# mkshing/e4t-diffusion

Hardware: AMD Instinct MI355X
Metric: E4T pretrain images/sec @512px bf16 (higher is better)
Workload: dtype bf16; 1 GPU; SD-1.4 UNet + ViT-H-14 E4T encoder pretrain step, 512px; per_gpu_batch=16, global_batch=16, parallelism=dp1, trainable=weight offsets + E4T head (ViT frozen), next_batch_prefetch=vit+vae

## Files before the change

e4t-diffusion_amd/csrc/attention.hip:

```cpp
#include "common.h"
#include "../../include/e4t_hip.h"
#include <math.h>
#include <type_traits>

namespace {

struct AttnArgs {
  const bf16_t *Q, *K, *V, *dO;
  const bf16_t* O;
  bf16_t *Out, *dQ, *dK, *dV;
  float* L;
  float* Delta;
  float* LD;
  int T, S, H;
  int ldq, ldk, ldv, ldo;
  long long bq, bk, bv, bo;
  float scale2;
  float scale;
  int causal;
  int xcd_raster;
  float* part;
  int tsplit, tchunk;
};

struct Blk { int x, h, b; };
__device__ __forceinline__ Blk xcd_block(int on) {
  Blk o{(int)blockIdx.x, (int)blockIdx.y, (int)blockIdx.z};
  if (!on) return o;
  const int gx = gridDim.x, gy = gridDim.y, nwg = gx * gy * gridDim.z;
  const int lin = (blockIdx.z * gy + blockIdx.y) * gx + blockIdx.x;
  const int q = nwg >> 3, r = nwg & 7, v = lin & 7;
  const int lin2 = (v < r ? v * (q + 1) : r * (q + 1) + (v - r) * q) + (lin >> 3);
  const int t = lin2 / gx;
  o.x = lin2 - t * gx; o.b = t / gy; o.h = t - o.b * gy;
  return o;
}

template <int DH>
struct Cfg {
  static constexpr int DK = (DH + 15) / 16 * 16;
  static constexpr int DV = (DH + 31) / 32 * 32;
  static constexpr int NKS = DK / 16;
  static constexpr int NDT = DV / 32;
  static constexpr int LDE = DH <= 128 ? 128 : 256;
  static constexpr int NCH = DH / 8;
  static constexpr int NIT = (32 * NCH + 255) / 256;
};

union Frag {
  bf16x8 v;
  uint4 q;
  uint2 h[2];
  uint32_t w[4];
};

__device__ __forceinline__ float xhalf_max(float v) {
  float a = v, b = v;
  asm volatile("s_nop 1\n\tv_permlane32_swap_b32 %0, %1\n\ts_nop 1\n\tv_max_f32 %0, %0, %1" : "+v"(a), "+v"(b));
  return a;
}
__device__ __forceinline__ float xhalf_sum(float v) {
  float a = v, b = v;
  asm volatile("s_nop 1\n\tv_permlane32_swap_b32 %0, %1\n\ts_nop 1\n\tv_add_f32 %0, %0, %1" : "+v"(a), "+v"(b));
  return a;
}

__device__ __forceinline__ f32x16 mfma32(bf16x8 a, bf16x8 b, f32x16 c) { return __builtin_amdgcn_mfma_f32_32x32x16_bf16(a, b, c, 0, 0, 0); }

__device__ __forceinline__ float fast_exp2(float x) { return __builtin_amdgcn_exp2f(x); }

typedef float f32x2 __attribute__((ext_vector_type(2)));
constexpr bool PK_REG = true;
constexpr bool PK_DMA = false;
template <bool PK>
__device__ __forceinline__ f32x2 pk_fma(f32x2 a, f32x2 b, f32x2 c) {
  if constexpr (PK) return __builtin_elementwise_fma(a, b, c);
  else return f32x2{__builtin_fmaf(a.x, b.x, c.x), __builtin_fmaf(a.y, b.y, c.y)};
}
template <bool PK>
__device__ __forceinline__ f32x2 pk_mul(f32x2 a, f32x2 b) {
  if constexpr (PK) return a * b;
  else return f32x2{a.x * b.x, a.y * b.y};
}


template <int LDE>
__device__ __forceinline__ int img_off(int r, int L) {
  return r * LDE + (((((L >> 2) ^ (r & 3)) << 2) | ((L & 3) ^ ((r >> 2) & 3))) << 3);
}

template <int DH>
struct TileRegs {
  using C = Cfg<DH>;
  uint4 v[C::NIT][2];
  unsigned vo[C::NIT];
  int ldb;
  __device__ __forceinline__ void init(int ld) {
    ldb = ld * 2;
#pragma unroll
    for (int it = 0; it < C::NIT; ++it) {
      const int item = threadIdx.x + it * 256;
      const int ch = item >> 5, kp = item & 31;
      vo[it] = item < 32 * C::NCH ? (unsigned)((2 * kp * ld + ch * 8) * 2) : 0xFFFF0000u;
    }
  }
  __device__ __forceinline__ void load(__amdgpu_buffer_rsrc_t rs, int r0) {
    const int soff = r0 * ldb;
#pragma unroll
    for (int it = 0; it < C::NIT; ++it) {
      v[it][0] = buf_load16(rs, vo[it], soff);
      v[it][1] = buf_load16(rs, vo[it], soff + ldb);
    }
  }
  __device__ __forceinline__ void store_rows(bf16_t* lds) const {
#pragma unroll
    for (int it = 0; it < C::NIT; ++it) {
      const int item = threadIdx.x + it * 256;
      const int ch = item >> 5, kp = item & 31;
      if (item < 32 * C::NCH) {
        *(uint4*)(lds + img_off<C::LDE>(2 * kp, ch)) = v[it][0];
        *(uint4*)(lds + img_off<C::LDE>(2 * kp + 1, ch)) = v[it][1];
      }
    }
  }
};

template <int DH>
__device__ __forceinline__ void zero_pad_cols(bf16_t* lds) {
  constexpr int PADC = (Cfg<DH>::DK - DH) / 8;
  if (PADC > 0)
    for (int i = threadIdx.x; i < 64 * PADC; i += 256)
      *(uint4*)(lds + img_off<Cfg<DH>::LDE>(i / PADC, Cfg<DH>::NCH + i % PADC)) = make_uint4(0, 0, 0, 0);
}

template <int DH>
__device__ __forceinline__ void load_row_frags(const bf16_t* g, int ld, int row, int R, int hi, bf16x8* f) {
#pragma unroll
  for (int ks = 0; ks < Cfg<DH>::NKS; ++ks) {
    Frag t;
    t.q = make_uint4(0, 0, 0, 0);
    const int d0 = ks * 16 + hi * 8;
    if (row < R && d0 < DH) t.q = *(const uint4*)(g + (long long)row * ld + d0);
    f[ks] = t.v;
  }
}

template <int DH>
struct FragOff {
  using C = Cfg<DH>;
  int row[C::NKS], tr_lo[C::NDT], tr_hi[C::NDT];
  __device__ __forceinline__ FragOff() {
    const int lane = threadIdx.x & 63, li = lane & 31, hi = lane >> 5, il = lane & 15, d16 = (lane >> 4) & 1;
#pragma unroll
    for (int ks = 0; ks < C::NKS; ++ks) row[ks] = img_off<C::LDE>(li, ks * 2 + hi);
#pragma unroll
    for (int dt = 0; dt < C::NDT; ++dt) {
      const int L = dt * 4 + 2 * d16 + ((il & 3) >> 1), r = 4 * hi + (il >> 2);
      tr_lo[dt] = img_off<C::LDE>(r, L) + 4 * (il & 1);
      tr_hi[dt] = img_off<C::LDE>(r + 8, L) + 4 * (il & 1);
    }
  }
};
template <int DH>
__device__ __forceinline__ bf16x8 load_row_frag(const bf16_t* img, const FragOff<DH>& f, int sub, int ks) {
  return *(const bf16x8*)(img + sub * 32 * Cfg<DH>::LDE + f.row[ks]);
}
template <int DH>
__device__ __forceinline__ bf16x8 load_T_frag(const bf16_t* img, const FragOff<DH>& f, int dt, int sub, int k2) {
  const bf16_t* b = img + (sub * 32 + k2 * 16) * Cfg<DH>::LDE;
  return tr_frag(b + f.tr_lo[dt], b + f.tr_hi[dt]);
}
__device__ __forceinline__ bf16x8 pack_acc(const float* p, int k2) {
  Frag t;
#pragma unroll
  for (int j = 0; j < 4; ++j) t.w[j] = pack2bf(p[8 * k2 + 2 * j], p[8 * k2 + 2 * j + 1]);
  return t.v;
}
__device__ __forceinline__ int acc_row(int r, int hi) { return (r & 3) + 8 * (r >> 2) + 4 * hi; }

template <int DH>
__device__ __forceinline__ void store_T_acc(const f32x16* acc, float mul, bf16_t* g, int ld, int row, int R, int hi) {
  if (row >= R) return;
#pragma unroll
  for (int dt = 0; dt < Cfg<DH>::NDT; ++dt)
#pragma unroll
    for (int rg = 0; rg < 4; ++rg) {
      const int d = dt * 32 + 8 * rg + 4 * hi;
      if (d < DH) {
        float f[4];
#pragma unroll
        for (int j = 0; j < 4; ++j) f[j] = acc[dt][rg * 4 + j] * mul;
        *(uint2*)(g + (long long)row * ld + d) = pack4(f);
      }
    }
}

template <int DH>
__device__ __forceinline__ void store_T_acc_f32(const f32x16* acc, float* g, int row, int R, int hi) {
  if (row >= R) return;
#pragma unroll
  for (int dt = 0; dt < Cfg<DH>::NDT; ++dt)
#pragma unroll
    for (int rg = 0; rg < 4; ++rg) {
      const int d = dt * 32 + 8 * rg + 4 * hi;
      if (d < DH) *(float4*)(g + (size_t)row * DH + d) = make_float4(acc[dt][rg * 4], acc[dt][rg * 4 + 1], acc[dt][rg * 4 + 2], acc[dt][rg * 4 + 3]);
    }
}

template <int DH>
__global__ __launch_bounds__(256, (DH <= 64 ? 4 : DH <= 80 ? 2 : 1)) void attn_fwd_kernel(AttnArgs p) {
  using C = Cfg<DH>;
  __shared__ __attribute__((aligned(16))) bf16_t Ks[64 * C::LDE];
  __shared__ __attribute__((aligned(16))) bf16_t Vs[64 * C::LDE];
  const FragOff<DH> fo;
  const Blk blk = xcd_block(p.xcd_raster);
  const int b = blk.b, h = blk.h;
  const int lane = threadIdx.x & 63, wave = threadIdx.x >> 6;
  const int li = lane & 31, hi = lane >> 5;
  const int q = blk.x * 128 + wave * 32 + li;
  const bf16_t* Qb = p.Q + b * p.bq + h * DH;
  const bf16_t* Kb = p.K + b * p.bk + h * DH;
  const bf16_t* Vb = p.V + b * p.bv + h * DH;

  bf16x8 qf[C::NKS];
  load_row_frags<DH>(Qb, p.ldq, q, p.T, hi, qf);

  f32x16 o[C::NDT];
#pragma unroll
  for (int dt = 0; dt < C::NDT; ++dt)
#pragma unroll
    for (int r = 0; r < 16; ++r) o[dt][r] = 0.f;
  float m = -INFINITY, l = 0.f;
  constexpr bool SUM_BY_MFMA = C::DV > DH && DH % 8 == 0;

  TileRegs<DH> kr, vr;
  const __amdgpu_buffer_rsrc_t rsK = make_rsrc(Kb, (unsigned)(((long long)(p.S - 1) * p.ldk + DH) * 2));
  const __amdgpu_buffer_rsrc_t rsV = make_rsrc(Vb, (unsigned)(((long long)(p.S - 1) * p.ldv + DH) * 2));
  kr.init(p.ldk); vr.init(p.ldv);
  kr.load(rsK, 0);
  vr.load(rsV, 0);
  zero_pad_cols<DH>(Ks);
  if (SUM_BY_MFMA) {
    if (threadIdx.x < 64) *(uint4*)(Vs + img_off<C::LDE>(threadIdx.x, C::NCH)) = make_uint4(0x3F80u, 0, 0, 0);
  }
  for (int kv0 = 0; kv0 < p.S; kv0 += 64) {
    __syncthreads();
    kr.store_rows(Ks);
    vr.store_rows(Vs);
    __syncthreads();
    if (kv0 + 64 < p.S) {
      kr.load(rsK, kv0 + 64);
      vr.load(rsV, kv0 + 64);
    }
    const int nsub = (p.S - kv0 > 32) ? 2 : 1;
#pragma unroll
    for (int sub = 0; sub < 2; ++sub) {
      if (sub >= nsub) break;
      f32x16 s;
#pragma unroll
      for (int r = 0; r < 16; ++r) s[r] = 0.f;
#pragma unroll
      for (int ks = 0; ks < C::NKS; ++ks) {
        s = mfma32(load_row_frag<DH>(Ks, fo, sub, ks), qf[ks], s);
      }
      float pr[16];
      float mx = -INFINITY;
      const bool tail = kv0 + 64 > p.S;
      if (tail || p.causal) {
#pragma unroll
        for (int r = 0; r < 16; ++r) {
          const int key = kv0 + sub * 32 + acc_row(r, hi);
          s[r] = (key < p.S && (!p.causal || key <= q)) ? s[r] : -INFINITY;
        }
      }
#pragma unroll
      for (int r = 0; r < 16; ++r) mx = fmaxf(mx, s[r]);
      mx = xhalf_max(mx) * p.scale2;
      if (__builtin_amdgcn_ballot_w64(mx > m + 8.f) != 0) {
        const float mn = fmaxf(m, mx);
        const float alpha = fast_exp2(m - mn);
        m = mn;
        if (!SUM_BY_MFMA) l *= alpha;
#pragma unroll
        for (int dt = 0; dt < C::NDT; ++dt)
#pragma unroll
          for (int r = 0; r < 16; ++r) o[dt][r] *= alpha;
      }
#pragma unroll
      for (int r = 0; r < 16; r += 2) {
        const f32x2 t = pk_fma<PK_REG>(f32x2{s[r], s[r + 1]}, f32x2{p.scale2, p.scale2}, f32x2{-m, -m});
        pr[r] = fast_exp2(t.x); pr[r + 1] = fast_exp2(t.y);
      }
      if (!SUM_BY_MFMA) {
        float rs = 0.f;
#pragma unroll
        for (int r = 0; r < 16; ++r) rs += pr[r];
        l += xhalf_sum(rs);
      }
      const bf16x8 pf0 = pack_acc(pr, 0), pf1 = pack_acc(pr, 1);
#pragma unroll
      for (int dt = 0; dt < C::NDT; ++dt) {
        o[dt] = mfma32(load_T_frag<DH>(Vs, fo, dt, sub, 0), pf0, o[dt]);
        o[dt] = mfma32(load_T_frag<DH>(Vs, fo, dt, sub, 1), pf1, o[dt]);
      }
    }
  }
  if (SUM_BY_MFMA) {
    constexpr int blk = DH / 32, reg = (DH % 32) / 8 * 4;
    static_assert((DH % 32) % 8 == 0 && ((DH % 32) / 8) * 8 + 0 == DH % 32, "spare row must be row 8k of its block");
    l = o[blk][reg];
    l = __shfl(l, li, 64);
  }
  const float inv = 1.f / l;
  store_T_acc<DH>(o, inv, p.Out + b * p.bo + h * DH, p.ldo, q, p.T, hi);
  if (p.L && hi == 0 && q < p.T) p.L[((long long)b * p.H + h) * p.T + q] = m + log2f(l);
}

constexpr int FWD64_OCC = 2, FWD64_MIN_S = 512;
__device__ __forceinline__ void a64_fence() { __builtin_amdgcn_sched_barrier(0); }

__device__ __forceinline__ f32x2 pk_fms(f32x2 s, f32x2 sc, f32x2 mm) {
  f32x2 d;
  asm("v_fma_f32 %0, %1, %2, -%3" : "=v"(d.x) : "v"(s.x), "s"(sc.x), "v"(mm.x));
  asm("v_fma_f32 %0, %1, %2, -%3" : "=v"(d.y) : "v"(s.y), "s"(sc.x), "v"(mm.x));
  return d;
}

__device__ __forceinline__ int img64_slot(int r, int L) { return ((((L >> 2) ^ ((r >> 1) & 1)) << 2) | ((L & 3) ^ ((r >> 2) & 3))); }
__device__ __forceinline__ int img64_off(int r, int L) { return r * 64 + img64_slot(r, L) * 8; }
template <int DH>
struct FragOff64 {
  using C = Cfg<DH>;
  static_assert(C::DV <= 64, "128-byte image rows hold 64 columns");
  int row[C::NKS], tr_lo[C::NDT], tr_hi[C::NDT];
  __device__ __forceinline__ FragOff64() {
    const int lane = threadIdx.x & 63, li = lane & 31, hi = lane >> 5, il = lane & 15, d16 = (lane >> 4) & 1;
#pragma unroll
    for (int ks = 0; ks < C::NKS; ++ks) row[ks] = img64_off(li, ks * 2 + hi);
#pragma unroll
    for (int dt = 0; dt < C::NDT; ++dt) {
      const int L = dt * 4 + 2 * d16 + ((il & 3) >> 1), r = 4 * hi + (il >> 2);
      tr_lo[dt] = img64_off(r, L) + 4 * (il & 1);
      tr_hi[dt] = img64_off(r + 8, L) + 4 * (il & 1);
    }
  }
};
typedef int i32x4_native __attribute__((ext_vector_type(4)));
struct DmaRsrc { i32x4_native w; };
__device__ __forceinline__ DmaRsrc make_dma_rsrc(const void* base, unsigned bytes) {
  const unsigned long long a = (unsigned long long)base;
  DmaRsrc r;
  r.w = i32x4_native{__builtin_amdgcn_readfirstlane((int)(unsigned)a), __builtin_amdgcn_readfirstlane((int)(unsigned)(a >> 32)),
                     __builtin_amdgcn_readfirstlane((int)bytes), 0x00020000};
  return r;
}
__device__ __forceinline__ unsigned lds_addr(const bf16_t* p) {
  return (unsigned)(unsigned long long)(__attribute__((address_space(3))) const void*)p;
}
__device__ __forceinline__ void dma16(const DmaRsrc& rs, unsigned voff, unsigned lds_wave_base_bytes) {
  asm volatile("s_mov_b32 m0, %0\n\ts_nop 0\n\tbuffer_load_dwordx4 %1, %2, 0 offen lds" ::"s"(lds_wave_base_bytes), "v"(voff), "s"(rs.w) : "memory");
}
__device__ __forceinline__ void dma4(const DmaRsrc& rs, unsigned voff, unsigned lds_wave_base_bytes) {
  asm volatile("s_mov_b32 m0, %0\n\ts_nop 0\n\tbuffer_load_dword %1, %2, 0 offen lds" ::"s"(lds_wave_base_bytes), "v"(voff), "s"(rs.w) : "memory");
}
template <int N>
__device__ __forceinline__ void attn_wait_vmcnt() { asm volatile("s_waitcnt vmcnt(%0)" ::"n"(N) : "memory"); }
template <int DH, int ROWS = 64>
struct TileDma {
  static constexpr int NP = ROWS / 32;
  unsigned vo[NP], step[NP];
  __device__ __forceinline__ void init(int ld) {
    const int lane = threadIdx.x & 63, wave = threadIdx.x >> 6;
#pragma unroll
    for (int i = 0; i < NP; ++i) {
      const int r = 8 * (NP * wave + i) + (lane >> 3), L = img64_slot(r, lane & 7);
      const bool on = L < Cfg<DH>::NCH;
      vo[i] = on ? (unsigned)((r * ld + L * 8) * 2) : 0x80000000u;
      step[i] = on ? (unsigned)(ROWS * ld * 2) : 0u;
    }
  }
  __device__ __forceinline__ void issue(const DmaRsrc& rs, bf16_t* img) {
    const unsigned base = __builtin_amdgcn_readfirstlane(lds_addr(img) + (threadIdx.x >> 6) * (NP * 1024));
#pragma unroll
    for (int i = 0; i < NP; ++i) {
      dma16(rs, vo[i], base + i * 1024);
      vo[i] += step[i];
    }
  }
};

template <int DH>
__device__ __forceinline__ void fwd64_write_pads(bf16_t* tile, int row0, int S) {
  constexpr int ROWS = 128, IMG = ROWS * 64, PER = ROWS / 4;
  const int lane = threadIdx.x & 63, wave = threadIdx.x >> 6;
  const int img = lane / PER, r = PER * wave + lane % PER;
  if (img < 2) {
    const unsigned w0 = img ? 0x3F80u : (row0 + r < S ? 0u : 0xC6EAu);
    *(uint4*)(tile + img * IMG + img64_off(r, Cfg<DH>::NCH)) = make_uint4(w0, 0u, 0u, 0u);
  }
}

template <int DH, bool LOADS, int VOFF, int KOFF, int PADS, int STAGE>
__device__ __forceinline__ void fwd64_phase(const f32x2 sc, const FragOff64<DH>& fo, bf16_t* lds,
                                            const f32x16& sx, f32x2& mm, Frag (&px)[2], f32x16 (&ox)[Cfg<DH>::NDT],
                                            f32x16& sy, const Frag (&py)[2], f32x16 (&oy)[Cfg<DH>::NDT], const bf16x8 (&qfy)[Cfg<DH>::NKS],
                                            bf16x8 (&vfr)[Cfg<DH>::NDT][2], bf16x8 (&kfr)[Cfg<DH>::NKS],
                                            TileDma<DH, 128>& kd, TileDma<DH, 128>& vd, const DmaRsrc& rsK, const DmaRsrc& rsV, const int pad_row0,
                                            const int S) {
  using C = Cfg<DH>;
  constexpr int NPV = 2 * C::NDT, NM = NPV + C::NKS, IMG = 128 * 64;
  f32x2 t = pk_fms(f32x2{sx[0], sx[1]}, sc, mm);
  float pe0 = 0.f, pe1 = 0.f;
#pragma unroll
  for (int c = 0; c < 8; ++c) {
#pragma unroll
    for (int i = (c * NM + 7) / 8; i < ((c + 1) * NM + 7) / 8; ++i) {
      if (i < NPV) {
        const int k2 = i / C::NDT, dt = i % C::NDT;
        oy[dt] = mfma32(vfr[dt][k2], py[k2].v, oy[dt]);
      } else {
        const int ks = i - NPV;
        f32x16 z;
#pragma unroll
        for (int r = 0; r < 16; ++r) z[r] = 0.f;
        sy = mfma32(kfr[ks], qfy[ks], ks == 0 ? z : sy);
      }
      a64_fence();
      if (LOADS && i == NPV - 1) {
#pragma unroll
        for (int k2 = 0; k2 < 2; ++k2)
#pragma unroll
          for (int dt = 0; dt < C::NDT; ++dt) {
            const bf16_t* vb = lds + VOFF + k2 * 16 * 64;
            vfr[dt][k2] = tr_frag(vb + fo.tr_lo[dt], vb + fo.tr_hi[dt]);
          }
        a64_fence();
      }
      if (LOADS && i == NM - 1 && PADS >= 0) {
        attn_wait_vmcnt<0>();
        fwd64_write_pads<DH>(lds + PADS, pad_row0, S);
        __syncthreads();
      }
      if (LOADS && i == NM - 1) {
#pragma unroll
        for (int ks = 0; ks < C::NKS; ++ks) kfr[ks] = *(const bf16x8*)(lds + KOFF + fo.row[ks]);
        a64_fence();
      }
    }
    const float e0 = fast_exp2(t.x), e1 = fast_exp2(t.y);
    if (c < 7) t = pk_fms(f32x2{sx[2 * c + 2], sx[2 * c + 3]}, sc, mm);
    if (c > 0) px[(c - 1) >> 2].w[(c - 1) & 3] = pack2bf(pe0, pe1);
    pe0 = e0; pe1 = e1;
    a64_fence();
    if (STAGE >= 0) {
      if (c == 0) { kd.issue(rsK, lds + STAGE); a64_fence(); }
      if (c == 1) { vd.issue(rsV, lds + STAGE + IMG); a64_fence(); }
    }
  }
  px[1].w[3] = pack2bf(pe0, pe1);
  const uint32_t orv = (px[0].w[0] | px[0].w[1] | px[0].w[2]) | (px[0].w[3] | px[1].w[0] | px[1].w[1]) | (px[1].w[2] | px[1].w[3]);
  if (__builtin_amdgcn_ballot_w64((orv & 0x40004000u) != 0u) != 0) {
    float mv = sx[0];
#pragma unroll
    for (int r = 1; r < 16; ++r) mv = fmaxf(mv, sx[r]);
    mv = xhalf_max(mv) * sc.x;
    const float mn = fmaxf(mm.x, mv);
    const float alpha = fast_exp2(mm.x - mn);
    mm = f32x2{mn, mn};
#pragma unroll
    for (int dt = 0; dt < C::NDT; ++dt)
#pragma unroll
      for (int r = 0; r < 16; ++r) ox[dt][r] *= alpha;
#pragma unroll
    for (int c = 0; c < 8; ++c) {
      const f32x2 u = pk_fma<PK_DMA>(f32x2{sx[2 * c], sx[2 * c + 1]}, sc, -mm);
      px[c >> 2].w[c & 3] = pack2bf(fast_exp2(u.x), fast_exp2(u.y));
    }
  }
}

template <int DH>
__global__ __launch_bounds__(256, FWD64_OCC) void attn_fwd64_kernel(AttnArgs p) {
  using C = Cfg<DH>;
  static_assert(DH % 16 == 8 && C::DV > DH && C::DV <= 64, "needs a spare contraction slot (key mask), a spare O^T row (row sum), 128-byte image rows");
  constexpr int ROWS = 128, IMG = ROWS * 64, TILE = 2 * IMG, NBUF = 2;
  __shared__ __attribute__((aligned(1024))) bf16_t lds[NBUF * TILE];
  const FragOff64<DH> fo;
  const Blk blk = xcd_block(p.xcd_raster);
  const int b = blk.b, h = blk.h;
  const int lane = threadIdx.x & 63, wave = threadIdx.x >> 6;
  const int li = lane & 31, hi = lane >> 5;
  const int q0 = blk.x * 256 + wave * 64 + li;
  const bf16_t* Qb = p.Q + b * p.bq + h * DH;
  const bf16_t* Kb = p.K + b * p.bk + h * DH;
  const bf16_t* Vb = p.V + b * p.bv + h * DH;
  const f32x2 sc = {p.scale2, p.scale2};

  TileDma<DH, ROWS> kd, vd;
  const DmaRsrc rsK = make_dma_rsrc(Kb, (unsigned)(((long long)(p.S - 1) * p.ldk + DH) * 2));
  const DmaRsrc rsV = make_dma_rsrc(Vb, (unsigned)(((long long)(p.S - 1) * p.ldv + DH) * 2));
  kd.init(p.ldk); vd.init(p.ldv);
#pragma unroll
  for (int tb = 0; tb < NBUF; ++tb) { kd.issue(rsK, lds + tb * TILE); vd.issue(rsV, lds + tb * TILE + IMG); }

  bf16x8 qf[2][C::NKS];
  load_row_frags<DH>(Qb, p.ldq, q0, p.T, hi, qf[0]);
  load_row_frags<DH>(Qb, p.ldq, q0 + 32, p.T, hi, qf[1]);
  if (hi == 1) {
    Frag t;
    t.q = make_uint4(0x3F80u, 0u, 0u, 0u);
    qf[0][DH / 16] = t.v; qf[1][DH / 16] = t.v;
  }

  f32x16 oa[C::NDT], ob[C::NDT], sa, sb;
  Frag pa[2], pb[2];
  bf16x8 vfr[C::NDT][2], kfr[C::NKS];
#pragma unroll
  for (int dt = 0; dt < C::NDT; ++dt)
#pragma unroll
    for (int r = 0; r < 16; ++r) { oa[dt][r] = 0.f; ob[dt][r] = 0.f; }
  {
    Frag z;
    z.q = make_uint4(0u, 0u, 0u, 0u);
    pa[0] = z; pa[1] = z; pb[0] = z; pb[1] = z;
#pragma unroll
    for (int dt = 0; dt < C::NDT; ++dt) { vfr[dt][0] = z.v; vfr[dt][1] = z.v; }
  }
  f32x2 ma = {-1e30f, -1e30f}, mb = ma;
  attn_wait_vmcnt<0>();
  fwd64_write_pads<DH>(lds, 0, p.S);
  __syncthreads();
#pragma unroll
  for (int ks = 0; ks < C::NKS; ++ks) kfr[ks] = *(const bf16x8*)(lds + fo.row[ks]);
#pragma unroll
  for (int r = 0; r < 16; ++r) sa[r] = 0.f;
#pragma unroll
  for (int ks = 0; ks < C::NKS; ++ks) sa = mfma32(kfr[ks], qf[0][ks], sa);

  const int ntiles = (p.S + ROWS - 1) / ROWS;
  auto tile = [&](auto tb_, int t) __attribute__((always_inline)) {
    constexpr int TB = decltype(tb_)::value;
    constexpr int KI = TB * TILE, VI = KI + IMG, KN = ((TB + 1) % NBUF) * TILE;
#define F64_Y sa, ma, pa, oa, sb, pb, ob, qf[1], vfr, kfr, kd, vd, rsK, rsV
#define F64_X sb, mb, pb, ob, sa, pa, oa, qf[0], vfr, kfr, kd, vd, rsK, rsV
    fwd64_phase<DH, true, VI, KI + 32 * 64, -1, -1>(sc, fo, lds, F64_Y, 0, p.S);
    fwd64_phase<DH, false, 0, 0, -1, -1>(sc, fo, lds, F64_X, 0, p.S);
    fwd64_phase<DH, true, VI + 32 * 64, KI + 64 * 64, -1, -1>(sc, fo, lds, F64_Y, 0, p.S);
    fwd64_phase<DH, false, 0, 0, -1, -1>(sc, fo, lds, F64_X, 0, p.S);
    fwd64_phase<DH, true, VI + 64 * 64, KI + 96 * 64, -1, -1>(sc, fo, lds, F64_Y, 0, p.S);
    fwd64_phase<DH, false, 0, 0, -1, -1>(sc, fo, lds, F64_X, 0, p.S);
    fwd64_phase<DH, true, VI + 96 * 64, KN, KN, -1>(sc, fo, lds, F64_Y, (t + 1) * ROWS, p.S);
    fwd64_phase<DH, false, 0, 0, -1, KI>(sc, fo, lds, F64_X, 0, p.S);
#undef F64_Y
#undef F64_X
  };
  for (int t = 0; t < ntiles; t += NBUF) {
    tile(std::integral_constant<int, 0>{}, t);
    if (t + 1 < ntiles) tile(std::integral_constant<int, 1>{}, t + 1);
  }
  attn_wait_vmcnt<0>();
#pragma unroll
  for (int k2 = 0; k2 < 2; ++k2)
#pragma unroll
    for (int dt = 0; dt < C::NDT; ++dt) ob[dt] = mfma32(vfr[dt][k2], pb[k2].v, ob[dt]);

  constexpr int sblk = DH / 32, sreg = (DH % 32) / 8 * 4;
  float la = __shfl(oa[sblk][sreg], li, 64), lb = __shfl(ob[sblk][sreg], li, 64);
  bf16_t* Ob = p.Out + b * p.bo + h * DH;
  int qrow = q0;
  asm volatile("" : "+v"(qrow));
  store_T_acc<DH>(oa, 1.f / la, Ob, p.ldo, qrow, p.T, hi);
  store_T_acc<DH>(ob, 1.f / lb, Ob, p.ldo, qrow + 32, p.T, hi);
  if (p.L && hi == 0) {
    float* Lb = p.L + ((long long)b * p.H + h) * p.T;
    if (qrow < p.T) Lb[qrow] = ma.x + log2f(la);
    if (qrow + 32 < p.T) Lb[qrow + 32] = mb.x + log2f(lb);
  }
}

template <int DH>
__device__ __forceinline__ float row_delta(const bf16_t* o_base, int ldo, int row, int R, int hi, const bf16x8* dof) {
  bf16x8 of[Cfg<DH>::NKS];
  load_row_frags<DH>(o_base, ldo, row, R, hi, of);
  float s = 0.f;
#pragma unroll
  for (int ks = 0; ks < Cfg<DH>::NKS; ++ks) {
    Frag a, g;
    a.v = of[ks]; g.v = dof[ks];
    float x[8], y[8];
    unpack8(a.q, x);
    unpack8(g.q, y);
#pragma unroll
    for (int k = 0; k < 8; ++k) s = fmaf(x[k], y[k], s);
  }
  return s + __shfl_xor(s, 32, 64);
}

template <int DH>
__global__ __launch_bounds__(256, (DH <= 64 ? 3 : DH <= 80 ? 2 : 1)) void attn_bwd_dq_kernel(AttnArgs p) {
  using C = Cfg<DH>;
  __shared__ __attribute__((aligned(16))) bf16_t Ks[64 * C::LDE];
  __shared__ __attribute__((aligned(16))) bf16_t Vs[64 * C::LDE];
  const FragOff<DH> fo;
  const Blk blk = xcd_block(p.xcd_raster);
  const int b = blk.b, h = blk.h;
  const int lane = threadIdx.x & 63, wave = threadIdx.x >> 6;
  const int li = lane & 31, hi = lane >> 5;
  const int q = blk.x * 128 + wave * 32 + li;
  const bf16_t* Kb = p.K + b * p.bk + h * DH;
  const bf16_t* Vb = p.V + b * p.bv + h * DH;

  bf16x8 qf[C::NKS], dof[C::NKS];
  load_row_frags<DH>(p.Q + b * p.bq + h * DH, p.ldq, q, p.T, hi, qf);
  load_row_frags<DH>(p.dO + b * p.bo + h * DH, p.ldo, q, p.T, hi, dof);
  float Lq = 0.f;
  const float Dq = row_delta<DH>(p.O + b * p.bo + h * DH, p.ldo, q, p.T, hi, dof);
  if (q < p.T) {
    Lq = p.L[((long long)b * p.H + h) * p.T + q];
    if (hi == 0) {
      p.Delta[((long long)b * p.H + h) * p.T + q] = Dq;
      if (p.LD) *(float2*)(p.LD + 2 * (((long long)b * p.H + h) * p.T + q)) = make_float2(Lq, Dq);
    }
  }

  f32x16 acc[C::NDT];
#pragma unroll
  for (int dt = 0; dt < C::NDT; ++dt)
#pragma unroll
    for (int r = 0; r < 16; ++r) acc[dt][r] = 0.f;

  TileRegs<DH> kr, vr;
  const __amdgpu_buffer_rsrc_t rsK = make_rsrc(Kb, (unsigned)(((long long)(p.S - 1) * p.ldk + DH) * 2));
  const __amdgpu_buffer_rsrc_t rsV = make_rsrc(Vb, (unsigned)(((long long)(p.S - 1) * p.ldv + DH) * 2));
  kr.init(p.ldk); vr.init(p.ldv);
  kr.load(rsK, 0);
  vr.load(rsV, 0);
  zero_pad_cols<DH>(Ks);
  zero_pad_cols<DH>(Vs);
  for (int kv0 = 0; kv0 < p.S; kv0 += 64) {
    __syncthreads();
    kr.store_rows(Ks);
    vr.store_rows(Vs);
    __syncthreads();
    if (kv0 + 64 < p.S) {
      kr.load(rsK, kv0 + 64);
      vr.load(rsV, kv0 + 64);
    }
    const int nsub = (p.S - kv0 > 32) ? 2 : 1;
    auto sub_tile = [&](auto sub_) __attribute__((always_inline)) {
      const int sub = sub_;
      f32x16 s, dp;
#pragma unroll
      for (int r = 0; r < 16; ++r) { s[r] = 0.f; dp[r] = 0.f; }
#pragma unroll
      for (int ks = 0; ks < C::NKS; ++ks) {
        s = mfma32(load_row_frag<DH>(Ks, fo, sub, ks), qf[ks], s);
        dp = mfma32(load_row_frag<DH>(Vs, fo, sub, ks), dof[ks], dp);
      }
      float ds[16];
      if (kv0 + 64 > p.S || p.causal) {
#pragma unroll
        for (int r = 0; r < 16; ++r) {
          const int key = kv0 + sub * 32 + acc_row(r, hi);
          const float pv = (key < p.S && (!p.causal || key <= q)) ? fast_exp2(s[r] * p.scale2 - Lq) : 0.f;
          ds[r] = pv * (dp[r] - Dq);
        }
      } else {
#pragma unroll
        for (int r = 0; r < 16; r += 2) {
          if (DH <= 48) {
            const f32x2 t = pk_fma<PK_REG>(f32x2{s[r], s[r + 1]}, f32x2{p.scale2, p.scale2}, f32x2{-Lq, -Lq});
            const f32x2 d = pk_fma<PK_REG>(f32x2{Dq, Dq}, f32x2{-1.f, -1.f}, f32x2{dp[r], dp[r + 1]});
            const f32x2 o2 = pk_mul<PK_REG>(f32x2{fast_exp2(t.x), fast_exp2(t.y)}, d);
            ds[r] = o2.x; ds[r + 1] = o2.y;
          } else {
            ds[r] = fast_exp2(s[r] * p.scale2 - Lq) * (dp[r] - Dq);
            ds[r + 1] = fast_exp2(s[r + 1] * p.scale2 - Lq) * (dp[r + 1] - Dq);
          }
        }
      }
      const bf16x8 f0 = pack_acc(ds, 0), f1 = pack_acc(ds, 1);
#pragma unroll
      for (int dt = 0; dt < C::NDT; ++dt) {
        acc[dt] = mfma32(load_T_frag<DH>(Ks, fo, dt, sub, 0), f0, acc[dt]);
        acc[dt] = mfma32(load_T_frag<DH>(Ks, fo, dt, sub, 1), f1, acc[dt]);
      }
    };
    if constexpr (DH <= 48) {
      sub_tile(std::integral_constant<int, 0>{});
      if (nsub > 1) sub_tile(std::integral_constant<int, 1>{});
    } else {
#pragma unroll 1
      for (int sub = 0; sub < nsub; ++sub) sub_tile(sub);
    }
  }
  int qrow = q;
  asm volatile("" : "+v"(qrow));
  store_T_acc<DH>(acc, p.scale, p.dQ + b * p.bq + h * DH, p.ldq, qrow, p.T, hi);
}

template <int DH>
__global__ __launch_bounds__(256, 3) void attn_bwd_dq_dma_kernel(AttnArgs p) {
  using C = Cfg<DH>;
  static_assert(C::DV <= 64, "compact images hold 64 columns");
  constexpr int IMG = 64 * 64, TILE = 2 * IMG, NB = 3;
  __shared__ __attribute__((aligned(1024))) bf16_t lds[NB * TILE];
  const FragOff64<DH> fo;
  const Blk blk = xcd_block(p.xcd_raster);
  const int b = blk.b, h = blk.h;
  const int lane = threadIdx.x & 63, wave = threadIdx.x >> 6;
  const int li = lane & 31, hi = lane >> 5;
  const int q = blk.x * 128 + wave * 32 + li;
  const bf16_t* Kb = p.K + b * p.bk + h * DH;
  const bf16_t* Vb = p.V + b * p.bv + h * DH;

  TileDma<DH> kd, vd;
  const DmaRsrc rsK = make_dma_rsrc(Kb, (unsigned)(((long long)(p.S - 1) * p.ldk + DH) * 2));
  const DmaRsrc rsV = make_dma_rsrc(Vb, (unsigned)(((long long)(p.S - 1) * p.ldv + DH) * 2));
  kd.init(p.ldk); vd.init(p.ldv);
  kd.issue(rsK, lds); vd.issue(rsV, lds + IMG);
  kd.issue(rsK, lds + TILE); vd.issue(rsV, lds + TILE + IMG);

  bf16x8 qf[C::NKS], dof[C::NKS];
  load_row_frags<DH>(p.Q + b * p.bq + h * DH, p.ldq, q, p.T, hi, qf);
  load_row_frags<DH>(p.dO + b * p.bo + h * DH, p.ldo, q, p.T, hi, dof);
  float Lq = 0.f;
  const float Dq = row_delta<DH>(p.O + b * p.bo + h * DH, p.ldo, q, p.T, hi, dof);
  if (q < p.T) {
    Lq = p.L[((long long)b * p.H + h) * p.T + q];
    if (hi == 0) {
      p.Delta[((long long)b * p.H + h) * p.T + q] = Dq;
      if (p.LD) *(float2*)(p.LD + 2 * (((long long)b * p.H + h) * p.T + q)) = make_float2(Lq, Dq);
    }
  }
  f32x16 acc[C::NDT];
#pragma unroll
  for (int dt = 0; dt < C::NDT; ++dt)
#pragma unroll
    for (int r = 0; r < 16; ++r) acc[dt][r] = 0.f;
  const int ntiles = (p.S + 63) >> 6;

  auto tile = [&](auto tb_, int t) __attribute__((always_inline)) {
    constexpr int TB = decltype(tb_)::value;
    constexpr int KI = TB * TILE, VI = KI + IMG, NXT = ((TB + 2) % NB) * TILE;
    attn_wait_vmcnt<4>();
    __syncthreads();
    kd.issue(rsK, lds + NXT); vd.issue(rsV, lds + NXT + IMG);
    const int kv0 = t * 64;
    auto sub_tile = [&](auto sub_) __attribute__((always_inline)) {
      constexpr int sub = decltype(sub_)::value, SO = sub * 32 * 64;
      f32x16 s, dp;
#pragma unroll
      for (int r = 0; r < 16; ++r) { s[r] = 0.f; dp[r] = 0.f; }
#pragma unroll
      for (int ks = 0; ks < C::NKS; ++ks) {
        s = mfma32(*(const bf16x8*)(lds + KI + SO + fo.row[ks]), qf[ks], s);
        dp = mfma32(*(const bf16x8*)(lds + VI + SO + fo.row[ks]), dof[ks], dp);
      }
      float ds[16];
      if (kv0 + 64 > p.S) {
#pragma unroll
        for (int r = 0; r < 16; ++r) {
          const int key = kv0 + sub * 32 + acc_row(r, hi);
          const float pv = key < p.S ? fast_exp2(s[r] * p.scale2 - Lq) : 0.f;
          ds[r] = pv * (dp[r] - Dq);
        }
      } else {
#pragma unroll
        for (int r = 0; r < 16; r += 2) {
          const f32x2 t2 = pk_fma<PK_DMA>(f32x2{s[r], s[r + 1]}, f32x2{p.scale2, p.scale2}, f32x2{-Lq, -Lq});
          const f32x2 d = pk_fma<PK_DMA>(f32x2{Dq, Dq}, f32x2{-1.f, -1.f}, f32x2{dp[r], dp[r + 1]});
          const f32x2 o2 = pk_mul<PK_DMA>(f32x2{fast_exp2(t2.x), fast_exp2(t2.y)}, d);
          ds[r] = o2.x; ds[r + 1] = o2.y;
        }
      }
      const bf16x8 f0 = pack_acc(ds, 0), f1 = pack_acc(ds, 1);
#pragma unroll
      for (int dt = 0; dt < C::NDT; ++dt) {
        const bf16_t* k0 = lds + KI + SO, *k1 = k0 + 16 * 64;
        acc[dt] = mfma32(tr_frag(k0 + fo.tr_lo[dt], k0 + fo.tr_hi[dt]), f0, acc[dt]);
        acc[dt] = mfma32(tr_frag(k1 + fo.tr_lo[dt], k1 + fo.tr_hi[dt]), f1, acc[dt]);
      }
    };
    sub_tile(std::integral_constant<int, 0>{});
    if (p.S - kv0 > 32) sub_tile(std::integral_constant<int, 1>{});
  };
  for (int t = 0; t < ntiles; t += 3) {
    tile(std::integral_constant<int, 0>{}, t);
    if (t + 1 < ntiles) tile(std::integral_constant<int, 1>{}, t + 1);
    if (t + 2 < ntiles) tile(std::integral_constant<int, 2>{}, t + 2);
  }
  attn_wait_vmcnt<0>();
  int qrow = q;
  asm volatile("" : "+v"(qrow));
  store_T_acc<DH>(acc, p.scale, p.dQ + b * p.bq + h * DH, p.ldq, qrow, p.T, hi);
}

__device__ __forceinline__ uint4 split3_bf16(float x) {
  const bf16_t h0 = f2bf(x);
  const float r1 = x - bf2f(h0);
  const bf16_t h1 = f2bf(r1);
  const bf16_t h2 = f2bf(r1 - bf2f(h1));
  return make_uint4((uint32_t)h0 | ((uint32_t)h1 << 16), (uint32_t)h2, 0u, 0u);
}

template <int DH, int OCC>
__global__ __launch_bounds__(256, OCC) void attn_bwd_dkv_kernel(AttnArgs p) {
  using C = Cfg<DH>;
  __shared__ __attribute__((aligned(16))) bf16_t Qs[64 * C::LDE];
  __shared__ __attribute__((aligned(16))) bf16_t dOs[64 * C::LDE];
  const FragOff<DH> fo;
  __shared__ __attribute__((aligned(16))) float Ls[64], Dls[64];
  const Blk blk = xcd_block(p.xcd_raster);
  const int b = blk.b, h = blk.h;
  const int lane = threadIdx.x & 63, wave = threadIdx.x >> 6;
  const int li = lane & 31, hi = lane >> 5;
  const int nkb = (p.S + 127) >> 7;
  const int ts = p.tsplit > 1 ? blk.x / nkb : 0;
  const int key = (blk.x - ts * nkb) * 128 + wave * 32 + li;
  const int t_begin = ts * p.tchunk, t_end = p.tsplit > 1 ? min(p.T, t_begin + p.tchunk) : p.T;
  const bf16_t* Qb = p.Q + b * p.bq + h * DH;
  const bf16_t* dOb = p.dO + b * p.bo + h * DH;

  bf16x8 kf[C::NKS], vf[C::NKS];
  load_row_frags<DH>(p.K + b * p.bk + h * DH, p.ldk, key, p.S, hi, kf);
  load_row_frags<DH>(p.V + b * p.bv + h * DH, p.ldv, key, p.S, hi, vf);
  constexpr bool FOLD = C::DK - DH >= 3 && DH % 8 == 0;
  if (FOLD && hi == (DH % 16) / 8) {
    Frag t;
    t.v = kf[DH / 16]; t.w[0] = 0x3F803F80u; t.w[1] = 0x00003F80u; kf[DH / 16] = t.v;
    t.v = vf[DH / 16]; t.w[0] = 0x3F803F80u; t.w[1] = 0x00003F80u; vf[DH / 16] = t.v;
  }

  f32x16 dvt[C::NDT], dkt[C::NDT];
#pragma unroll
  for (int dt = 0; dt < C::NDT; ++dt)
#pragma unroll
    for (int r = 0; r < 16; ++r) { dvt[dt][r] = 0.f; dkt[dt][r] = 0.f; }

  TileRegs<DH> qr, dor;
  float l_next = 0.f, d_next = 0.f;
  auto load_stats = [&](int q0) {
    if (threadIdx.x < 64) {
      const int qq = q0 + threadIdx.x;
      l_next = qq < p.T ? p.L[((long long)b * p.H + h) * p.T + qq] : INFINITY;
      d_next = qq < p.T ? p.Delta[((long long)b * p.H + h) * p.T + qq] : 0.f;
    }
  };
  constexpr bool PF = DH <= 80 && OCC < 3;
  const __amdgpu_buffer_rsrc_t rsQ = make_rsrc(Qb, (unsigned)(((long long)(p.T - 1) * p.ldq + DH) * 2));
  const __amdgpu_buffer_rsrc_t rsdO = make_rsrc(dOb, (unsigned)(((long long)(p.T - 1) * p.ldo + DH) * 2));
  qr.init(p.ldq); dor.init(p.ldo);
  if (PF) {
    qr.load(rsQ, t_begin);
    dor.load(rsdO, t_begin);
    load_stats(t_begin);
  }
  zero_pad_cols<DH>(Qs);
  zero_pad_cols<DH>(dOs);
  const float inv_scale2 = 1.f / p.scale2;
  for (int q0 = t_begin; q0 < t_end; q0 += 64) {
    if (!PF) {
      qr.load(rsQ, q0);
      dor.load(rsdO, q0);
      load_stats(q0);
    }
    __syncthreads();
    qr.store_rows(Qs);
    dor.store_rows(dOs);
    if (threadIdx.x < 64) {
      if (FOLD) {
        *(uint4*)(Qs + img_off<C::LDE>(threadIdx.x, C::NCH)) = split3_bf16(fmaxf(-l_next * inv_scale2, -1e30f));
        *(uint4*)(dOs + img_off<C::LDE>(threadIdx.x, C::NCH)) = split3_bf16(-d_next);
      } else {
        Ls[threadIdx.x] = l_next; Dls[threadIdx.x] = d_next;
      }
    }
    __syncthreads();
    if (PF && q0 + 64 < t_end) {
      qr.load(rsQ, q0 + 64);
      dor.load(rsdO, q0 + 64);
      load_stats(q0 + 64);
    }
    const int nsub = (t_end - q0 > 32) ? 2 : 1;
    auto sub_tile = [&](auto sub_) __attribute__((always_inline)) {
      const int sub = sub_;
      f32x16 s, dp;
#pragma unroll
      for (int r = 0; r < 16; ++r) { s[r] = 0.f; dp[r] = 0.f; }
#pragma unroll
      for (int ks = 0; ks < C::NKS; ++ks) {
        s = mfma32(load_row_frag<DH>(Qs, fo, sub, ks), kf[ks], s);
        dp = mfma32(load_row_frag<DH>(dOs, fo, sub, ks), vf[ks], dp);
      }
      float pr[16], ds[16];
      if (FOLD) {
#pragma unroll
        for (int r = 0; r < 16; r += 2) {
          const f32x2 t = pk_mul<PK_REG>(f32x2{s[r], s[r + 1]}, f32x2{p.scale2, p.scale2});
          const f32x2 e2 = f32x2{fast_exp2(t.x), fast_exp2(t.y)};
          const f32x2 o2 = pk_mul<PK_REG>(e2, f32x2{dp[r], dp[r + 1]});
          pr[r] = e2.x; pr[r + 1] = e2.y; ds[r] = o2.x; ds[r + 1] = o2.y;
        }
      } else
#pragma unroll
      for (int g = 0; g < 4; ++g) {
        const float4 l4 = *(const float4*)(Ls + sub * 32 + 8 * g + 4 * hi);
        const float4 d4 = *(const float4*)(Dls + sub * 32 + 8 * g + 4 * hi);
        const float lq[4] = {l4.x, l4.y, l4.z, l4.w}, dq[4] = {d4.x, d4.y, d4.z, d4.w};
#pragma unroll
        for (int j = 0; j < 4; j += 2) {
          const int r = 4 * g + j;
          const f32x2 t = pk_fma<PK_REG>(f32x2{s[r], s[r + 1]}, f32x2{p.scale2, p.scale2}, f32x2{-lq[j], -lq[j + 1]});
          const f32x2 d = pk_fma<PK_REG>(f32x2{dq[j], dq[j + 1]}, f32x2{-1.f, -1.f}, f32x2{dp[r], dp[r + 1]});
          const f32x2 e2 = f32x2{fast_exp2(t.x), fast_exp2(t.y)};
          const f32x2 o2 = pk_mul<PK_REG>(e2, d);
          pr[r] = e2.x; pr[r + 1] = e2.y; ds[r] = o2.x; ds[r + 1] = o2.y;
        }
      }
      if (p.causal) {
#pragma unroll
        for (int r = 0; r < 16; ++r)
          if (q0 + sub * 32 + acc_row(r, hi) < key) { pr[r] = 0.f; ds[r] = 0.f; }
      }
      const bf16x8 pf0 = pack_acc(pr, 0), pf1 = pack_acc(pr, 1);
      const bf16x8 sf0 = pack_acc(ds, 0), sf1 = pack_acc(ds, 1);
#pragma unroll
      for (int dt = 0; dt < C::NDT; ++dt) {
        dvt[dt] = mfma32(load_T_frag<DH>(dOs, fo, dt, sub, 0), pf0, dvt[dt]);
        dvt[dt] = mfma32(load_T_frag<DH>(dOs, fo, dt, sub, 1), pf1, dvt[dt]);
        dkt[dt] = mfma32(load_T_frag<DH>(Qs, fo, dt, sub, 0), sf0, dkt[dt]);
        dkt[dt] = mfma32(load_T_frag<DH>(Qs, fo, dt, sub, 1), sf1, dkt[dt]);
      }
    };
    if constexpr (DH <= 48) {
      sub_tile(std::integral_constant<int, 0>{});
      if (nsub > 1) sub_tile(std::integral_constant<int, 1>{});
    } else {
#pragma unroll 1
      for (int sub = 0; sub < nsub; ++sub) sub_tile(sub);
    }
  }
  int krow = key;
  asm volatile("" : "+v"(krow));
  if (p.tsplit > 1) {
    float* base = p.part + ((((size_t)ts * gridDim.z + b) * p.H + h) * 2) * (size_t)p.S * DH;
    store_T_acc_f32<DH>(dvt, base, krow, p.S, hi);
    store_T_acc_f32<DH>(dkt, base + (size_t)p.S * DH, krow, p.S, hi);
    return;
  }
  store_T_acc<DH>(dvt, 1.f, p.dV + b * p.bv + h * DH, p.ldv, krow, p.S, hi);
  store_T_acc<DH>(dkt, p.scale, p.dK + b * p.bk + h * DH, p.ldk, krow, p.S, hi);
}

template <int DH>
__global__ __launch_bounds__(256, 3) void attn_bwd_dkv_dma_kernel(AttnArgs p) {
  using C = Cfg<DH>;
  static_assert(DH % 16 == 8 && C::DK - DH >= 3 && C::DV <= 64, "folded statistics need three spare contraction slots; compact images 64 columns");
  constexpr int IMG = 64 * 64, STAT = 512, TILE = 2 * IMG + STAT, NB = 3;
  __shared__ __attribute__((aligned(1024))) bf16_t lds[NB * TILE];
  const FragOff64<DH> fo;
  const Blk blk = xcd_block(p.xcd_raster);
  const int b = blk.b, h = blk.h;
  const int lane = threadIdx.x & 63, wave = __builtin_amdgcn_readfirstlane(threadIdx.x >> 6);
  const int li = lane & 31, hi = lane >> 5;
  const int key = blk.x * 128 + wave * 32 + li;
  const bf16_t* Qb = p.Q + b * p.bq + h * DH;
  const bf16_t* dOb = p.dO + b * p.bo + h * DH;
  const float* LDb = p.LD + 2 * ((long long)b * p.H + h) * p.T;

  bf16x8 kf[C::NKS], vf[C::NKS];
  load_row_frags<DH>(p.K + b * p.bk + h * DH, p.ldk, key, p.S, hi, kf);
  load_row_frags<DH>(p.V + b * p.bv + h * DH, p.ldv, key, p.S, hi, vf);
  if (hi == 1) {
    Frag t;
    t.q = make_uint4(0x3F803F80u, 0x00003F80u, 0u, 0u);
    kf[DH / 16] = t.v; vf[DH / 16] = t.v;
  }
  f32x16 dvt[C::NDT], dkt[C::NDT];
#pragma unroll
  for (int dt = 0; dt < C::NDT; ++dt)
#pragma unroll
    for (int r = 0; r < 16; ++r) { dvt[dt][r] = 0.f; dkt[dt][r] = 0.f; }

  TileDma<DH> qd, dod;
  const DmaRsrc rsQ = make_dma_rsrc(Qb, (unsigned)(((long long)(p.T - 1) * p.ldq + DH) * 2));
  const DmaRsrc rsdO = make_dma_rsrc(dOb, (unsigned)(((long long)(p.T - 1) * p.ldo + DH) * 2));
  const DmaRsrc rsLD = make_dma_rsrc(LDb, (unsigned)(p.T * 8));
  qd.init(p.ldq); dod.init(p.ldo);
  unsigned svo = lane < 32 ? (unsigned)((32 * wave + lane) * 4) : 0x80000000u;
  const unsigned sstep = lane < 32 ? 512u : 0u;
  auto issue_tile = [&](bf16_t* slot) {
    qd.issue(rsQ, slot); dod.issue(rsdO, slot + IMG);
    dma4(rsLD, svo, __builtin_amdgcn_readfirstlane(lds_addr(slot + 2 * IMG) + wave * 256));
    svo += sstep;
  };
  issue_tile(lds);
  issue_tile(lds + TILE);
  const float inv_scale2 = 1.f / p.scale2;
  const int ntiles = (p.T + 63) >> 6;

  auto tile = [&](auto tb_, int t) __attribute__((always_inline)) {
    constexpr int TB = decltype(tb_)::value;
    constexpr int QI = TB * TILE, DI = QI + IMG, SI = QI + 2 * IMG, NXT = ((TB + 2) % NB) * TILE;
    attn_wait_vmcnt<5>();
    if (lane < 32) {
      const int r = 16 * wave + (lane & 15);
      const float2 ld = *(const float2*)((const float*)(lds + SI) + 64 * wave + 2 * (lane & 15));
      const int q = t * 64 + r;
      const float x = lane < 16 ? fmaxf(-(q < p.T ? ld.x : INFINITY) * inv_scale2, -1e30f) : (q < p.T ? -ld.y : 0.f);
      *(uint4*)(lds + (lane < 16 ? QI : DI) + img64_off(r, C::NCH)) = split3_bf16(x);
    }
    __syncthreads();
    issue_tile(lds + NXT);
    auto sub_tile = [&](auto sub_) __attribute__((always_inline)) {
      constexpr int SO = decltype(sub_)::value * 32 * 64;
      f32x16 s, dp;
#pragma unroll
      for (int r = 0; r < 16; ++r) { s[r] = 0.f; dp[r] = 0.f; }
#pragma unroll
      for (int ks = 0; ks < C::NKS; ++ks) {
        s = mfma32(*(const bf16x8*)(lds + QI + SO + fo.row[ks]), kf[ks], s);
        dp = mfma32(*(const bf16x8*)(lds + DI + SO + fo.row[ks]), vf[ks], dp);
      }
      float pr[16], ds[16];
#pragma unroll
      for (int r = 0; r < 16; r += 2) {
        const f32x2 t2 = pk_mul<PK_DMA>(f32x2{s[r], s[r + 1]}, f32x2{p.scale2, p.scale2});
        const f32x2 e2 = f32x2{fast_exp2(t2.x), fast_exp2(t2.y)};
        const f32x2 o2 = pk_mul<PK_DMA>(e2, f32x2{dp[r], dp[r + 1]});
        pr[r] = e2.x; pr[r + 1] = e2.y; ds[r] = o2.x; ds[r + 1] = o2.y;
      }
      const bf16x8 pf0 = pack_acc(pr, 0), pf1 = pack_acc(pr, 1);
      const bf16x8 sf0 = pack_acc(ds, 0), sf1 = pack_acc(ds, 1);
#pragma unroll
      for (int dt = 0; dt < C::NDT; ++dt) {
        const bf16_t* q0 = lds + QI + SO, *q1 = q0 + 16 * 64, *o0 = lds + DI + SO, *o1 = o0 + 16 * 64;
        dvt[dt] = mfma32(tr_frag(o0 + fo.tr_lo[dt], o0 + fo.tr_hi[dt]), pf0, dvt[dt]);
        dvt[dt] = mfma32(tr_frag(o1 + fo.tr_lo[dt], o1 + fo.tr_hi[dt]), pf1, dvt[dt]);
        dkt[dt] = mfma32(tr_frag(q0 + fo.tr_lo[dt], q0 + fo.tr_hi[dt]), sf0, dkt[dt]);
        dkt[dt] = mfma32(tr_frag(q1 + fo.tr_lo[dt], q1 + fo.tr_hi[dt]), sf1, dkt[dt]);
      }
    };
    sub_tile(std::integral_constant<int, 0>{});
    if (p.T - t * 64 > 32) sub_tile(std::integral_constant<int, 1>{});
  };
  for (int t = 0; t < ntiles; t += 3) {
    tile(std::integral_constant<int, 0>{}, t);
    if (t + 1 < ntiles) tile(std::integral_constant<int, 1>{}, t + 1);
    if (t + 2 < ntiles) tile(std::integral_constant<int, 2>{}, t + 2);
  }
  attn_wait_vmcnt<0>();
  int krow = key;
  asm volatile("" : "+v"(krow));
  store_T_acc<DH>(dvt, 1.f, p.dV + b * p.bv + h * DH, p.ldv, krow, p.S, hi);
  store_T_acc<DH>(dkt, p.scale, p.dK + b * p.bk + h * DH, p.ldk, krow, p.S, hi);
}

template <int DH>
__global__ __launch_bounds__(256) void attn_dkv_reduce_kernel(AttnArgs p, int Bn) {
  constexpr int D4 = DH / 4;
  const long long per = (long long)p.S * D4, total = (long long)Bn * p.H * 2 * per;
  const size_t slab = (size_t)Bn * p.H * 2 * p.S * DH;
  for (long long i = (long long)blockIdx.x * 256 + threadIdx.x; i < total; i += (long long)gridDim.x * 256) {
    const long long bh2 = i / per;
    const int rem = (int)(i - bh2 * per), key = rem / D4, d = (rem - key * D4) * 4;
    const int which = (int)(bh2 & 1), h = (int)((bh2 >> 1) % p.H), b = (int)((bh2 >> 1) / p.H);
    const float* src = p.part + (size_t)bh2 * p.S * DH + (size_t)key * DH + d;
    float4 a = *(const float4*)src;
    for (int t = 1; t < p.tsplit; ++t) {
      const float4 v = *(const float4*)(src + (size_t)t * slab);
      a.x += v.x; a.y += v.y; a.z += v.z; a.w += v.w;
    }
    const float mul = which ? p.scale : 1.f;
    const float f[4] = {a.x * mul, a.y * mul, a.z * mul, a.w * mul};
    bf16_t* dst = which ? p.dK + b * p.bk + (long long)key * p.ldk + h * DH + d : p.dV + b * p.bv + (long long)key * p.ldv + h * DH + d;
    *(uint2*)dst = pack4(f);
  }
}

struct AttnKernel { void (*fn)(AttnArgs); const char* text; int rows; };
#define ATTN_KERNEL(rows, name, ...) {&name<__VA_ARGS__>, #name "<" #__VA_ARGS__ ">", rows}
#define NO_KERNEL {nullptr, nullptr, 0}
struct AttnKernels {
  int dh;
  AttnKernel fwd, fwd64;
  AttnKernel dq, dq_dma;
  AttnKernel dkv, dkv3, dkv_dma;
  void (*reduce)(AttnArgs, int);
};
const AttnKernels kKernels[] = {
    {32, ATTN_KERNEL(128, attn_fwd_kernel, 32), NO_KERNEL, ATTN_KERNEL(128, attn_bwd_dq_kernel, 32), ATTN_KERNEL(128, attn_bwd_dq_dma_kernel, 32),
     ATTN_KERNEL(128, attn_bwd_dkv_kernel, 32, 2), ATTN_KERNEL(128, attn_bwd_dkv_kernel, 32, 3), NO_KERNEL, &attn_dkv_reduce_kernel<32>},
    {40, ATTN_KERNEL(128, attn_fwd_kernel, 40), ATTN_KERNEL(256, attn_fwd64_kernel, 40), ATTN_KERNEL(128, attn_bwd_dq_kernel, 40),
     ATTN_KERNEL(128, attn_bwd_dq_dma_kernel, 40), ATTN_KERNEL(128, attn_bwd_dkv_kernel, 40, 2), ATTN_KERNEL(128, attn_bwd_dkv_kernel, 40, 3),
     ATTN_KERNEL(128, attn_bwd_dkv_dma_kernel, 40), &attn_dkv_reduce_kernel<40>},
    {64, ATTN_KERNEL(128, attn_fwd_kernel, 64), NO_KERNEL, ATTN_KERNEL(128, attn_bwd_dq_kernel, 64), ATTN_KERNEL(128, attn_bwd_dq_dma_kernel, 64),
     ATTN_KERNEL(128, attn_bwd_dkv_kernel, 64, 2), NO_KERNEL, NO_KERNEL, &attn_dkv_reduce_kernel<64>},
    {80, ATTN_KERNEL(128, attn_fwd_kernel, 80), NO_KERNEL, ATTN_KERNEL(128, attn_bwd_dq_kernel, 80), NO_KERNEL,
     ATTN_KERNEL(128, attn_bwd_dkv_kernel, 80, 1), NO_KERNEL, NO_KERNEL, &attn_dkv_reduce_kernel<80>},
    {160, ATTN_KERNEL(128, attn_fwd_kernel, 160), NO_KERNEL, ATTN_KERNEL(128, attn_bwd_dq_kernel, 160), NO_KERNEL,
     ATTN_KERNEL(128, attn_bwd_dkv_kernel, 160, 1), NO_KERNEL, NO_KERNEL, &attn_dkv_reduce_kernel<160>},
};
#undef ATTN_KERNEL
#undef NO_KERNEL
const AttnKernels* kernels_for(int DH) {
  for (const AttnKernels& k : kKernels)
    if (k.dh == DH) return &k;
  return nullptr;
}

inline void dkv_tsplit(int Bn, int H, int T, int S, int* tsplit, int* tchunk) {
  const long long wgs = (long long)cdiv(S, 128) * H * Bn;
  int n = 1;
  if (wgs < 512 && T >= 512) {
    n = (int)((1024 + wgs - 1) / wgs);
    if (n > T / 256) n = T / 256;
    if (n < 1) n = 1;
  }
  const int chunk = cdiv(cdiv(T, n), 64) * 64;
  *tchunk = chunk;
  *tsplit = cdiv(T, chunk);
}

struct BwdWorkspace {
  int tsplit, tchunk;
  size_t ld, part;
  size_t total;
};
BwdWorkspace plan_workspace(int Bn, int H, int T, int S, int DH, size_t ws_floats) {
  BwdWorkspace w{};
  dkv_tsplit(Bn, H, T, S, &w.tsplit, &w.tchunk);
  const size_t delta = (size_t)Bn * H * T, behind = (delta + 3) & ~(size_t)3;
  if (w.tsplit > 1) {
    const size_t partials = (size_t)w.tsplit * Bn * H * 2 * S * DH;
    w.total = delta + 4 + partials;
    if (ws_floats >= delta + 3 + partials) w.part = behind;
    else w.tsplit = 1;
  } else {
    w.total = 3 * delta + 4;
    if (ws_floats >= w.total) w.ld = behind;
  }
  return w;
}

const AttnKernel& plan_fwd(const AttnKernels& k, int S, int causal) {
  return k.dh == 40 && !causal && S >= FWD64_MIN_S ? k.fwd64 : k.fwd;
}

struct BwdPlan {
  BwdWorkspace ws;
  const AttnKernel *dq, *dkv;
  int dkv_occ;
  bool reduce;
};
BwdPlan plan_bwd(const AttnKernels& k, int Bn, int H, int T, int S, int causal, size_t ws_floats) {
  const int DH = k.dh;
  BwdPlan pl;
  pl.ws = plan_workspace(Bn, H, T, S, DH, ws_floats);
  const bool dq_dma = DH <= 64 && !causal && S >= 192;
  const bool dkv_dma = DH == 40 && !causal && pl.ws.tsplit == 1 && T >= 192 && pl.ws.ld != 0 && (long long)T * 8 < 0x7fffffffLL;
  pl.dkv_occ = dkv_dma ? 3 : DH > 64 ? 1 : (S >= 2048 && DH < 64) ? 3 : 2;
  pl.dq = dq_dma ? &k.dq_dma : &k.dq;
  pl.dkv = dkv_dma ? &k.dkv_dma : pl.dkv_occ == 3 ? &k.dkv3 : &k.dkv;
  pl.reduce = pl.ws.tsplit > 1;
  return pl;
}

int launch(const AttnKernel& k, dim3 grid, const AttnArgs& p, hipStream_t st) {
  E4T_REQUIRE(k.fn, "attention: the planned kernel is not built for this head dim");
  hipLaunchKernelGGL(k.fn, grid, dim3(256), 0, st, p);
  E4T_CHECK_LAUNCH(k.text);
  return 0;
}

int launch_fwd(const AttnKernels& k, const AttnArgs& p, int Bn, hipStream_t st) {
  const int DH = k.dh;
  const AttnKernel& f = plan_fwd(k, p.S, p.causal);
  E4T_LOG_LAUNCH("%s|B%d H%d T%d S%d causal%d|%.0f|%.0f", f.text, Bn, p.H, p.T, p.S, p.causal,
                 2.0 * Bn * p.H * DH * (2.0 * p.T + 2.0 * p.S) + 4.0 * Bn * p.H * p.T, 4.0 * Bn * p.H * (double)p.T * p.S * DH);
  return launch(f, dim3(cdiv(p.T, f.rows), p.H, Bn), p, st);
}

int launch_bwd(const AttnKernels& k, AttnArgs p, int Bn, size_t ws_floats, hipStream_t st) {
  const int DH = k.dh;
  const BwdPlan pl = plan_bwd(k, Bn, p.H, p.T, p.S, p.causal, ws_floats);
  p.tsplit = pl.ws.tsplit; p.tchunk = pl.ws.tchunk;
  if (pl.ws.ld) p.LD = p.Delta + pl.ws.ld;
  if (pl.ws.part) p.part = p.Delta + pl.ws.part;
  if (e4t_launch_log_enabled()) {
    const double el = (double)Bn * p.H * DH;
    E4T_LOG_LAUNCH("%s|B%d H%d T%d S%d causal%d|%.0f|%.0f", pl.dq->text, Bn, p.H, p.T, p.S, p.causal,
                   2.0 * el * (4.0 * p.T + 2.0 * p.S) + 8.0 * Bn * p.H * p.T, 6.0 * Bn * p.H * (double)p.T * p.S * DH);
    E4T_LOG_LAUNCH("%s|B%d H%d T%d S%d causal%d|%.0f|%.0f", pl.dkv->text, Bn, p.H, p.T, p.S, p.causal,
                   2.0 * el * (2.0 * p.T + 4.0 * p.S) + 8.0 * Bn * p.H * p.T, 8.0 * Bn * p.H * (double)p.T * p.S * DH);
  }
  if (int e = launch(*pl.dq, dim3(cdiv(p.T, pl.dq->rows), p.H, Bn), p, st)) return e;
  if (int e = launch(*pl.dkv, dim3(cdiv(p.S, pl.dkv->rows) * p.tsplit, p.H, Bn), p, st)) return e;
  if (pl.reduce) {
    const long long items = (long long)Bn * p.H * 2 * p.S * (DH / 4);
    int rb = (int)((items + 255) / 256);
    if (rb > 2048) rb = 2048;
    hipLaunchKernelGGL(k.reduce, dim3(rb), dim3(256), 0, st, p, Bn);
    E4T_CHECK_LAUNCH("attn_dkv_reduce_kernel");
  }
  return 0;
}

int check_common(int Bn, int H, int T, int S, int DH, int ldq, int ldk, int ldv, int ldo) {
  E4T_REQUIRE(Bn > 0 && H > 0 && T > 0 && S > 0, "attention: bad shape B=%d H=%d T=%d S=%d", Bn, H, T, S);
  E4T_REQUIRE(kernels_for(DH), "attention: head dim %d not built (32/40/64/80/160)", DH);
  E4T_REQUIRE(ldq % 8 == 0 && ldk % 8 == 0 && ldv % 8 == 0 && ldo % 8 == 0, "attention: row strides must be multiples of 8");
  return 0;
}

AttnArgs common_args(const void* Q, const void* K, const void* V, int H, int T, int S, int ldq, int ldk, int ldv, int ldo, long long bq, long long bk,
                     long long bv, long long bo, float scale, int causal) {
  AttnArgs p;
  memset(&p, 0, sizeof(p));
  p.Q = (const bf16_t*)Q; p.K = (const bf16_t*)K; p.V = (const bf16_t*)V;
  p.T = T; p.S = S; p.H = H; p.ldq = ldq; p.ldk = ldk; p.ldv = ldv; p.ldo = ldo; p.bq = bq; p.bk = bk; p.bv = bv; p.bo = bo;
  p.scale = scale; p.scale2 = scale * 1.4426950408889634f; p.causal = causal;
  p.xcd_raster = 1;
  return p;
}

}

extern "C" int e4t_attention_fwd(const void* Q, const void* K, const void* V, void* O, float* lse, int Bn, int H, int T, int S,
                                 int DH, int ldq, int ldk, int ldv, int ldo, long long bq, long long bk, long long bv,
                                 long long bo, float scale, int causal, e4t_stream stream) {
  if (int e = check_common(Bn, H, T, S, DH, ldq, ldk, ldv, ldo)) return e;
  E4T_REQUIRE(Q && K && V && O, "attention_fwd: null operand");
  AttnArgs p = common_args(Q, K, V, H, T, S, ldq, ldk, ldv, ldo, bq, bk, bv, bo, scale, causal);
  p.Out = (bf16_t*)O; p.L = lse;
  return launch_fwd(*kernels_for(DH), p, Bn, (hipStream_t)stream);
}

extern "C" size_t e4t_attention_bwd_workspace_floats(int Bn, int H, int T, int S, int DH) {
  if (Bn <= 0 || H <= 0 || T <= 0 || S <= 0 || DH <= 0) return 0;
  return plan_workspace(Bn, H, T, S, DH, 0).total;
}

extern "C" int e4t_attention_plan(int Bn, int H, int T, int S, int DH, int causal, size_t ws_floats, e4t_attention_plan_t* out) {
  if (int e = check_common(Bn, H, T, S, DH, 0, 0, 0, 0)) return e;
  E4T_REQUIRE(out, "attention_plan: null output");
  const AttnKernels& k = *kernels_for(DH);
  const BwdPlan pl = plan_bwd(k, Bn, H, T, S, causal, ws_floats);
  out->fwd = plan_fwd(k, S, causal).text; out->dq = pl.dq->text; out->dkv = pl.dkv->text;
  out->tsplit = pl.ws.tsplit; out->tchunk = pl.ws.tchunk; out->dkv_occ = pl.dkv_occ;
  out->workspace_floats = pl.ws.total;
  return 0;
}

extern "C" int e4t_attention_bwd(const void* Q, const void* K, const void* V, const void* O, const void* dO, const float* lse,
                                 float* delta_ws, void* dQ, void* dK, void* dV, int Bn, int H, int T, int S, int DH, int ldq,
                                 int ldk, int ldv, int ldo, long long bq, long long bk, long long bv, long long bo, float scale,
                                 int causal, e4t_stream stream) {
  return e4t_attention_bwd_ws(Q, K, V, O, dO, lse, delta_ws, (size_t)(Bn > 0 && H > 0 && T > 0 ? (size_t)Bn * H * T : 0), dQ, dK, dV, Bn, H, T, S, DH,
                              ldq, ldk, ldv, ldo, bq, bk, bv, bo, scale, causal, stream);
}

extern "C" int e4t_attention_bwd_ws(const void* Q, const void* K, const void* V, const void* O, const void* dO, const float* lse,
                                    float* delta_ws, size_t ws_floats, void* dQ, void* dK, void* dV, int Bn, int H, int T, int S, int DH,
                                    int ldq, int ldk, int ldv, int ldo, long long bq, long long bk, long long bv, long long bo, float scale,
                                    int causal, e4t_stream stream) {
  if (int e = check_common(Bn, H, T, S, DH, ldq, ldk, ldv, ldo)) return e;
  E4T_REQUIRE(Q && K && V && O && dO && lse && delta_ws && dQ && dK && dV, "attention_bwd: null operand");
  E4T_REQUIRE(ws_floats >= (size_t)Bn * H * T, "attention_bwd: workspace of %zu floats is smaller than B*H*T", ws_floats);
  E4T_REQUIRE(((uintptr_t)delta_ws & 15) == 0, "attention_bwd: workspace must be 16-byte aligned");
  AttnArgs p = common_args(Q, K, V, H, T, S, ldq, ldk, ldv, ldo, bq, bk, bv, bo, scale, causal);
  p.O = (const bf16_t*)O; p.dO = (const bf16_t*)dO; p.L = (float*)lse; p.Delta = delta_ws;
  p.dQ = (bf16_t*)dQ; p.dK = (bf16_t*)dK; p.dV = (bf16_t*)dV;
  return launch_bwd(*kernels_for(DH), p, Bn, ws_floats, (hipStream_t)stream);
}
```

e4t-diffusion_amd/e4t/_C.py:

```python
from __future__ import annotations

import ctypes as C
import os

_HERE = os.path.dirname(os.path.abspath(__file__))
LIB_PATH = os.environ.get("E4T_LIB") or os.path.join(_HERE, "libe4t_hip.so")

vp, i32, i64, f32, sz = C.c_void_p, C.c_int, C.c_longlong, C.c_float, C.c_size_t


class GemmDesc(C.Structure):
    _fields_ = [
        ("A", vp), ("A2", vp), ("B", vp), ("C", vp), ("bias", vp), ("residual", vp), ("rowbias", vp),
        ("workspace", vp), ("workspace_bytes", sz),
        ("M", i32), ("N", i32), ("K", i32), ("K1", i32),
        ("lda", i32), ("lda2", i32), ("ldb", i32), ("ldc", i32), ("ldr", i32),
        ("rows_per_batch", i32), ("flags", i32), ("tile", i32), ("splitk", i32), ("batch", i32),
        ("strideA", i64), ("strideB", i64), ("strideC", i64), ("strideBias", i64),
        ("alpha", f32), ("ldrb", i32), ("colstats", vp),
        ("panel_rows", i32), ("panel_stride", i32), ("panel_off", i32),
        ("aux", vp), ("ldaux", i32),
    ]


class ConvDesc(C.Structure):
    _fields_ = [
        ("X", vp), ("W", vp), ("Y", vp), ("bias", vp), ("residual", vp), ("rowbias", vp),
        ("workspace", vp), ("workspace_bytes", sz),
        ("B", i32), ("Hin", i32), ("Win", i32), ("Cin", i32), ("Hout", i32), ("Wout", i32), ("Cout", i32),
        ("mode", i32), ("flags", i32), ("tile", i32), ("splitk", i32), ("ldrb", i32), ("colstats", vp),
    ]


class GemmPlan(C.Structure):
    _fields_ = [("tile", i32), ("tile_m", i32), ("tile_n", i32), ("splitk", i32), ("workspace_bytes", sz), ("tail_rows", i32), ("stages", i32)]


class GemmKernel(C.Structure):
    _fields_ = [("symbol", C.c_char_p), ("reduce", C.c_char_p), ("splitk", i32), ("tail_rows", i32), ("store", i32), ("colstats", i32)]


class AttentionPlan(C.Structure):
    _fields_ = [("fwd", C.c_char_p), ("dq", C.c_char_p), ("dkv", C.c_char_p), ("tsplit", i32), ("tchunk", i32), ("dkv_occ", i32), ("workspace_floats", sz)]


class WODesc(C.Structure):
    _fields_ = (
        [(n, vp) for n in ("v", "w1", "b1", "w2", "b2", "wc", "bc", "wr", "br", "W", "vecs", "partial", "weff", "weffT", "dweff")]
        + [(n, vp) for n in ("g_v", "g_w1", "g_b1", "g_w2", "g_b2", "g_wc", "g_bc", "g_wr", "g_br", "g_W")]
        + [(n, i32) for n in ("row", "col", "ld_weff", "ld_weffT", "ld_dweff", "mode")]
    )


SIGNATURES = {
    "e4t_version": (i32, []),
    "e4t_last_error": (C.c_char_p, []),
    "e4t_device_info": (i32, [C.c_char_p, i32, C.POINTER(i32)]),
    "e4t_set_launch_log": (i32, [C.c_char_p]),
    "e4t_gemm_nt": (i32, [C.POINTER(GemmDesc), vp]),
    "e4t_gemm_tn": (i32, [C.POINTER(GemmDesc), vp]),
    "e4t_conv3x3": (i32, [C.POINTER(ConvDesc), vp]),
    "e4t_gemm_plan": (i32, [C.POINTER(GemmDesc), C.POINTER(GemmPlan)]),
    "e4t_gemm_tn_plan": (i32, [C.POINTER(GemmDesc), C.POINTER(GemmPlan)]),
    "e4t_conv3x3_plan": (i32, [C.POINTER(ConvDesc), C.POINTER(GemmPlan)]),
    "e4t_conv3x3_kernel": (i32, [C.POINTER(ConvDesc), C.POINTER(C.c_char_p), C.POINTER(i32)]),
    "e4t_gemm_kernel": (i32, [C.POINTER(GemmDesc), C.POINTER(GemmKernel)]),
    "e4t_gemm_tn_kernel": (i32, [C.POINTER(GemmDesc), C.POINTER(GemmKernel)]),
    "e4t_attention_fwd": (i32, [vp, vp, vp, vp, vp, i32, i32, i32, i32, i32, i32, i32, i32, i32, i64, i64, i64, i64, f32, i32, vp]),
    "e4t_attention_bwd": (i32, [vp] * 10 + [i32] * 9 + [i64] * 4 + [f32, i32, vp]),
    "e4t_attention_bwd_workspace_floats": (sz, [i32] * 5),
    "e4t_attention_bwd_ws": (i32, [vp] * 7 + [sz] + [vp] * 3 + [i32] * 9 + [i64] * 4 + [f32, i32, vp]),
    "e4t_attention_plan": (i32, [i32] * 6 + [sz, C.POINTER(AttentionPlan)]),
    "e4t_groupnorm_num_chunks": (i32, [i32, i32]),
    "e4t_groupnorm_workspace_bytes": (sz, [i32, i32, i32, i32, i32]),
    "e4t_groupnorm_stats": (i32, [vp, i32, vp, i32, i32, i32, i32, f32, vp, vp, sz, vp]),
    "e4t_groupnorm_apply": (i32, [vp, i32, vp, i32, vp, vp, vp, vp, i32, i32, i32, i32, vp]),
    "e4t_groupnorm_fwd": (i32, [vp, i32, vp, i32, vp, vp, vp, vp, i32, i32, i32, f32, i32, vp, sz, vp]),
    "e4t_groupnorm_fwd_cs": (i32, [vp, i32, vp, vp, i32, vp, vp, vp, vp, vp, i32, i32, i32, f32, i32, vp, sz, vp]),
    "e4t_groupnorm_bwd": (i32, [vp, i32, vp, i32, vp, vp, vp, vp, vp, vp, vp, vp, vp, i32, i32, i32, i32, vp, sz, vp]),
    "e4t_layernorm_fwd": (i32, [vp, vp, vp, vp, vp, i32, i32, f32, vp]),
    "e4t_layernorm_fwd_f32": (i32, [vp, vp, vp, vp, vp, i32, i32, f32, vp]),
    "e4t_layernorm_bwd": (i32, [vp, vp, vp, vp, vp, vp, i32, i32, vp]),
    "e4t_colreduce_splits": (i32, [i32]),
    "e4t_colsum": (i32, [vp, i32, i32, i32, vp, i32, vp, sz, vp]),
    "e4t_layernorm_param_grad": (i32, [vp, vp, vp, i32, i32, vp, vp, i32, vp, sz, vp]),
    "e4t_wo_vecs_floats": (sz, [i32, i32]),
    "e4t_wo_partial_floats": (sz, [i32, i32]),
    "e4t_wo_forward": (i32, [vp, i32, i32, i32, vp]),
    "e4t_wo_backward": (i32, [vp, i32, i32, i32, i32, vp]),
    "e4t_weight_prepare": (i32, [vp, i32, i32, i32, vp]),
    "e4t_conv_weight_prepare": (i32, [vp, vp, vp, i32, i32, i32, i32, vp]),
    "e4t_geglu_fwd": (i32, [vp, vp, i64, i32, vp]),
    "e4t_geglu_bwd": (i32, [vp, vp, vp, i64, i32, vp]),
    "e4t_unary": (i32, [vp, vp, vp, i64, i32, vp]),
    "e4t_add": (i32, [vp, vp, vp, i64, vp]),
    "e4t_transpose": (i32, [vp, vp, i32, i32, i32, i32, i32, i64, i64, vp]),
    "e4t_sumpool2": (i32, [vp, vp, i32, i32, i32, i32, vp]),
    "e4t_spatial_mean": (i32, [vp, vp, i32, i32, i32, i32, i32, vp]),
    "e4t_spatial_mean_bwd": (i32, [vp, vp, vp, i32, i32, i32, i32, i32, vp]),
    "e4t_timestep_embedding": (i32, [vp, vp, i32, i32, vp]),
    "e4t_clip_preprocess": (i32, [vp, vp, i32, i32, i32, i32, i32, i32, vp]),
    "e4t_guided_step": (i32, [vp, vp, vp, vp, vp, i32, i32, i32, i32, i32, vp]),
    "e4t_sampler_step": (i32, [vp, vp, vp, vp, vp, vp, vp, vp, i32, i32, i32, i32, i32, i32, i32, vp]),
    "e4t_sampler_step_edit": (i32, [vp, vp, vp, vp, vp, vp, vp, vp, vp, vp, vp, i32, i32, i32, i32, i32, i32, i32, i32, i32, vp]),
    "e4t_image_prep": (i32, [vp, vp, vp, i32, i32, vp]),
    "e4t_mask_prep": (i32, [vp, vp, vp, vp, i32, i32, vp]),
    "e4t_masked_mse_fwd": (i32, [vp, vp, vp, vp, vp, i32, i32, i32, i32, vp]),
    "e4t_masked_mse_bwd": (i32, [vp, vp, vp, vp, i64, vp]),
    "e4t_weighted_mse_fwd": (i32, [vp, vp, vp, vp, vp, vp, i32, i32, i32, i32, vp]),
    "e4t_robust_loss_fwd": (i32, [vp, vp, vp, vp, vp, vp, vp, vp, i32, i32, i32, i32, i32, i32, vp]),
    "e4t_diffuse": (i32, [vp, vp, vp, vp, vp, vp, vp, vp, i32, i32, i32, i32, f32, i32, vp]),
    "e4t_softmax_rows": (i32, [vp, i64, i32, i32, vp]),
    "e4t_im2col3_rgb": (i32, [vp, vp, i32, i32, i32, vp]),
    "e4t_im2col_T": (i32, [vp, vp, i32, i32, i32, i32, i32, i32, i32, i32, vp]),
    "e4t_im2col": (i32, [vp, vp, i32, i32, i32, i32, i32, i32, i32, vp]),
    "e4t_adamw": (i32, [vp, vp, vp, vp, i64, f32, f32, f32, f32, f32, i32, f32, vp]),
    "e4t_adamw_hyper": (i32, [vp, vp, vp, vp, i64, vp, f32, f32, f32, f32, vp]),
    "e4t_adamw_rank": (i32, [vp, vp, vp, vp, vp, i32, i32, i32, i32, i32, i64, f32, f32, f32, f32, f32, i32, f32, vp, vp]),
    "e4t_adamw_ema": (i32, [vp, vp, vp, vp, vp, i64, f32, f32, f32, f32, f32, i32, f32, f32, vp, vp]),
    "e4t_adamw_rank_ema": (i32, [vp, vp, vp, vp, vp, vp, i32, i32, i32, i32, i32, i64, f32, f32, f32, f32, f32, i32, f32, f32, vp, vp]),
    "e4t_ema_update": (i32, [vp, vp, i64, f32, vp, vp]),
    "e4t_adamw8": (i32, [vp, vp, vp, vp, vp, vp, vp, i64, vp, vp, f32, f32, f32, f32, f32, i32, f32, f32, vp, vp]),
    "e4t_sumsq_partial": (i32, [vp, i64, vp, i32, vp]),
    "e4t_tome_plan_ints": (sz, [i32, i32]),
    "e4t_tome_match": (i32, [vp, i32, i32, i32, i32, i32, i32, vp, vp, vp]),
    "e4t_tome_merge": (i32, [vp, i32, vp, vp, i32, i32, i32, i32, i32, i32, vp]),
    "e4t_tome_unmerge": (i32, [vp, i32, vp, vp, vp, i32, i32, i32, i32, i32, i32, vp]),
    "e4t_probe_mfma_layout": (i32, [vp, vp, vp]),
    "e4t_comm_unique_id": (i32, [vp]),
    "e4t_comm_init": (i32, [C.POINTER(vp), vp, i32, i32]),
    "e4t_comm_allreduce": (i32, [vp, vp, i64, i32, i32, vp]),
    "e4t_comm_allgather": (i32, [vp, vp, vp, i64, i32, vp]),
    "e4t_comm_wait": (i32, [vp, vp]),
    "e4t_comm_info": (i32, [vp, C.POINTER(i32), C.POINTER(i32), C.POINTER(vp)]),
    "e4t_comm_destroy": (i32, [vp]),
}

OUT_F32, RES_F32, ACT_GELU, ACCUM, REDUCE_BATCH = 1, 2, 4, 8, 16
EPI_GEGLU, EPI_GEGLU_BWD = 32, 64
ERR_NO_FUSED = -95
STORE_NAMES = ("bf16-staged", "f32-direct", "scalar", "splitk-partial")
CONV_S1, CONV_S2, CONV_UP2, CONV_S2T, CONV_S2A = 1, 2, 3, 4, 5
WO_STORE_F32, WO_OFFSETS_ONLY = 1, 2
SAMPLER_MAX_HIST, SAMPLER_ROW = 4, 16
MASKED_MSE_STATS = 2050
LOSS_HUBER, LOSS_SMOOTH_L1 = 1, 2
COMM_F32, COMM_BF16 = 0, 1
COMM_SUM, COMM_AVG, COMM_MIN, COMM_MAX = 0, 1, 2, 3
OP_SILU, OP_SILU_BWD, OP_GELU, OP_GELU_BWD, OP_LRELU, OP_LRELU_BWD, OP_QGELU, OP_QGELU_BWD = range(8)

_lib = None


class E4TError(RuntimeError):
    pass


def load():
    global _lib
    if _lib is not None:
        return _lib
    if not os.path.exists(LIB_PATH):
        raise E4TError(
            f"{LIB_PATH} not found: build the HIP extension first (python -c 'import __graft_entry__ as g; g.build()'). "
            "There is no CPU / PyTorch fallback for the E4T hot path."
        )
    lib = C.CDLL(LIB_PATH)
    for name, (res, args) in SIGNATURES.items():
        fn = getattr(lib, name)
        fn.restype = res
        fn.argtypes = args
    _lib = lib
    return lib


def check(code: int, what: str) -> int:
    if code >= 0:
        return code
    msg = load().e4t_last_error()
    raise E4TError(f"{what} failed ({code}): {msg.decode() if msg else '?'}")
```

e4t-diffusion_amd/e4t/functional.py:

```python
from __future__ import annotations


import torch

from . import _C, ops

f32 = torch.float32


def act_dtype():
    return ops.ACT


class PreparedLinear:

    def __init__(self, weight: torch.nn.Parameter, colstats: bool = False):
        self.weight = weight
        self.key = None
        self.w = self.wT = None
        self._table = None
        self.colstats = colstats

    def get(self):
        wt = self.weight
# ... 140 lines not shown
    if ctx_needs_w:
        N, kw = weight.shape[0], weight[0].numel()
        g = _grad_slot(weight)
        if g is not None and x.shape[1] == kw:
            _weight_grad(dyb, x, out=g.view(N, kw))
        else:
            dw = _weight_grad(dyb, x)
            if dw.shape[1] != kw:
                dw = dw[:, :kw].contiguous()
            dw = dw.reshape(weight.shape)
    if ctx_needs_b:
        g = _grad_slot(bias) if (bias.requires_grad and bias.is_leaf) else None
        if g is not None:
            ops.backend().colsum(dyb, out=g, accumulate=True)
        else:
            db = ops.backend().colsum(dyb)
    return dw, db


class FeedForwardFn(torch.autograd.Function):

    @staticmethod
    def forward(ctx, x, w1, b1, w2, b2, residual, prep1: PreparedLinear, prep2: PreparedLinear):
        be = ops.backend()
        w1c, _ = prep1.get()
        w2c, _ = prep2.get()
        K, H = x.shape[1], w2.shape[1]
        w1v = w1c[:, :K] if w1c.shape[1] != K else w1c
        w2v = w2c[:, :H] if w2c.shape[1] != H else w2c
        uh = be.gemm_geglu(x, w1v, b1) if hasattr(be, "gemm_geglu") and not prep1.colstats else None
        if uh is None:
            u = be.gemm(x, w1v, bias=b1, out_dtype=act_dtype(), colstats=prep1.colstats)
            uh = (u, be.geglu_fwd(u))
        u, h = uh
        y = be.gemm(h, w2v, bias=b2, residual=residual, out_dtype=act_dtype(), colstats=prep2.colstats)
        ctx.prep1, ctx.prep2 = prep1, prep2
        ctx.params = (w1, b1, w2, b2)
        ctx.res_dtype = residual.dtype if residual is not None else None
        ctx.save_for_backward(x if w1.requires_grad else None, u, h if w2.requires_grad else None)
        return y

    @staticmethod
    def backward(ctx, dy):
        be = ops.backend()
        x, u, h = ctx.saved_tensors
        w1, b1, w2, b2 = ctx.params
        need = ctx.needs_input_grad
        dyb = (dy if dy.dtype == act_dtype() else dy.to(act_dtype())).contiguous()
        dx = dw1 = db1 = dw2 = db2 = dres = None
        if need[0] or need[1] or (b1 is not None and need[2]):
            _, w2T = ctx.prep2.get()
            N2, H = w2.shape
            w2Tn = w2T[:, :N2] if w2T.shape[1] != N2 else w2T
            du = be.gemm_geglu_bwd(dyb, w2Tn, u) if hasattr(be, "gemm_geglu_bwd") else None
            if du is None:
                du = be.geglu_bwd(u, be.gemm(dyb, w2Tn))
            if need[0]:
                _, w1T = ctx.prep1.get()
                N1 = w1.shape[0]
                dx = be.gemm(du, w1T[:, :N1] if w1T.shape[1] != N1 else w1T)
            dw1, db1 = _linear_param_grads(need[1], b1 is not None and need[2], w1, b1, du, x)
        dw2, db2 = _linear_param_grads(need[3], b2 is not None and need[4], w2, b2, dyb, h)
        if ctx.res_dtype is not None and need[5]:
            dres = dy if dy.dtype == ctx.res_dtype else dy.to(ctx.res_dtype)
        return dx, dw1, db1, dw2, db2, dres, None, None


def feed_forward(x, w1, b1, prep1, w2, b2, prep2, residual=None):
    return FeedForwardFn.apply(x, w1, b1, w2, b2, residual, prep1, prep2)


class WOSlot:

    def __init__(self, weff, weffT, dweff):
        self.weff, self.weffT, self.dweff = weff, weffT, dweff
        self.dweff_valid = False


class WOLinearFn(torch.autograd.Function):

    @staticmethod
    def forward(ctx, x, token, slot: WOSlot):
        y = ops.backend().gemm(x, slot.weff)
        ctx.slot = slot
        ctx.save_for_backward(x)
        return y

    @staticmethod
    def backward(ctx, dy):
        be = ops.backend()
        (x,) = ctx.saved_tensors
        slot = ctx.slot
        dy = dy.contiguous()
        dx = be.gemm(dy, slot.weffT) if ctx.needs_input_grad[0] else None
        be.gemm_tn(dy, x, out=slot.dweff, accum=slot.dweff_valid)
        slot.dweff_valid = True
        return dx, None, None


class WOBankFn(torch.autograd.Function):

    @staticmethod
    def forward(ctx, root, bank):
        bank._run_forward()
        ctx.bank = bank
        ctx.set_materialize_grads(False)
        tok = getattr(bank, "_token_value", None)
        if tok is None or tok.device != root.device:
            tok = bank._token_value = torch.zeros(1, dtype=f32, device=root.device)
        return tok.view_as(tok)

    @staticmethod
    def backward(ctx, g):
        ctx.bank._run_backward()
        return None, None


class ConvFn(torch.autograd.Function):
    @staticmethod
    def forward(ctx, x, weight, bias, rowbias, residual, prep: PreparedConv, geom, mode: int, out_f32: bool):
        B, Hin, Win, Hout, Wout = geom
        wf, _ = prep.get()
        y = ops.backend().conv3x3(x, wf, B, Hin, Win, Hout, Wout, mode, bias=bias, rowbias=rowbias, residual=residual,
                                  out_dtype=f32 if out_f32 else act_dtype(), colstats=not out_f32)
        ctx.prep, ctx.geom, ctx.mode = prep, geom, mode
        ctx.cin = x.shape[1]
        ctx.has = (bias is not None, rowbias is not None, residual is not None)
        ctx.bias_param = bias if (bias is not None and bias.requires_grad and bias.is_leaf) else None
        ctx.res_dtype = residual.dtype if residual is not None else None
        ctx.save_for_backward(x if weight.requires_grad else None)
        return y

    @staticmethod
    def backward(ctx, dy):
        be = ops.backend()
        B, Hin, Win, Hout, Wout = ctx.geom
        has_bias, has_rb, has_res = ctx.has
        dyb = dy if dy.dtype == act_dtype() else dy.to(act_dtype())
        dyb = dyb.contiguous()
        cout = dyb.shape[1]
        dx = db = drb = dres = None
        if ctx.needs_input_grad[0]:
            _, wd = ctx.prep.get()
            opad = wd.shape[1] // 9
            if opad != cout:
                t = torch.zeros((dyb.shape[0], opad), dtype=dyb.dtype, device=dyb.device)
                t[:, :cout] = dyb
                dyb_p = t
            else:
                dyb_p = dyb
            if ctx.mode == _C.CONV_S1:
                dx = be.conv3x3(dyb_p, wd, B, Hout, Wout, Hin, Win, _C.CONV_S1)
            elif ctx.mode == _C.CONV_S2:
                dx = be.conv3x3(dyb_p, wd, B, Hout, Wout, Hin, Win, _C.CONV_S2T)
            else:
                up = be.conv3x3(dyb_p, wd, B, Hout, Wout, Hout, Wout, _C.CONV_S1)
                dx = be.sumpool2(up, B, Hin, Win)
            if dx.shape[1] != ctx.cin:
                dx = dx[:, : ctx.cin].contiguous()
        dw = None
        if ctx.needs_input_grad[1]:
            (x,) = ctx.saved_tensors
            wshape = ctx.prep.weight.shape
            if cout % 8 == 0 and x.shape[1] % 8 == 0:
                dwk = be.gemm_tn(dyb, be.im2col(x, B, Hin, Win, Hout, Wout, ctx.mode), out_dtype=f32)
            else:
                xcolT = be.im2col_T(x, B, Hin, Win, Hout, Wout, ctx.mode)
                dwk = be.gemm(be.transpose(dyb, pad_to=xcolT.shape[1]), xcolT, out_dtype=f32)
            dw = dwk.view(wshape[0], 9, ctx.cin)[:, :, : wshape[1]].permute(0, 2, 1).reshape(wshape).contiguous()
        if has_bias and ctx.needs_input_grad[2]:
            g = _grad_slot(ctx.bias_param) if ctx.bias_param is not None else None
            if g is not None:
                ops.backend().colsum(dyb, out=g, accumulate=True)
            else:
                db = ops.backend().colsum(dyb)
        if has_rb and ctx.needs_input_grad[3]:
            drb = torch.zeros((B, cout), dtype=f32, device=dy.device)
            be.spatial_mean(dyb, B, Hout * Wout, drb, 0)
            drb = drb * float(Hout * Wout)
        if has_res and ctx.needs_input_grad[4]:
            dres = dy if dy.dtype == ctx.res_dtype else dy.to(ctx.res_dtype)
        return dx, dw, db, drb, dres, None, None, None, None


def conv3x3(x, weight, bias, prep, geom, mode=_C.CONV_S1, rowbias=None, residual=None, out_f32=False):
    return ConvFn.apply(x, weight, bias, rowbias, residual, prep, geom, mode, out_f32)


class TimeEmbProjAllFn(torch.autograd.Function):

    @staticmethod
    def forward(ctx, temb_act, wcat, wcat_t, bcat, splits):
        y = ops.backend().gemm(temb_act, wcat, bias=bcat, out_dtype=f32)
        ctx.save_for_backward(wcat_t)
        ctx.splits, ctx.act = splits, temb_act.dtype
        return tuple(y[:, o:o + c] for o, c in splits)

    @staticmethod
    def backward(ctx, *grads):
        (wcat_t,) = ctx.saved_tensors
        ref = next(g for g in grads if g is not None)
        parts = [g if g is not None else ref.new_zeros((ref.shape[0], c)) for g, (o, c) in zip(grads, ctx.splits)]
        dy = torch.cat(parts, dim=1).to(ctx.act)
        return ops.backend().gemm(dy, wcat_t), None, None, None, None


class GroupNormFn(torch.autograd.Function):
    @staticmethod
    def forward(ctx, x1, x2, gamma, beta, B, HW, G, eps, silu):
        y, stats = ops.backend().groupnorm_fwd(x1, x2, gamma, beta, B, HW, G, eps, silu)
        ctx.save_for_backward(x1, x2, stats, gamma, beta)
        ctx.cfg = (B, HW, G, silu)
        return y

    @staticmethod
    def backward(ctx, dy):
        x1, x2, stats, gamma, beta = ctx.saved_tensors
        B, HW, G, silu = ctx.cfg
        wp = ctx.needs_input_grad[2] or ctx.needs_input_grad[3]
        dx1, dx2, dg, db = ops.backend().groupnorm_bwd(x1, x2, dy.contiguous(), stats, gamma, beta, None, B, HW, G, silu, want_param_grads=wp)
        return dx1, dx2, dg, db, None, None, None, None, None


def group_norm(x1, x2, gamma, beta, B, HW, G, eps, silu):
    return GroupNormFn.apply(x1, x2, gamma, beta, B, HW, G, eps, silu)


class GroupNormSkipFn(torch.autograd.Function):

    @staticmethod
    def forward(ctx, x1, x2, gamma, beta, B, HW, G, eps, silu):
        y, stats = ops.backend().groupnorm_fwd(x1, x2, gamma, beta, B, HW, G, eps, silu)
        ctx.save_for_backward(x1, x2, stats, gamma, beta)
        ctx.cfg = (B, HW, G, silu)
        if x2 is None:
            return y, x1.view_as(x1)
        return y, x1.view_as(x1), x2.view_as(x2)

    @staticmethod
    def backward(ctx, dy, d1, d2=None):
        x1, x2, stats, gamma, beta = ctx.saved_tensors
        B, HW, G, silu = ctx.cfg
        wp = ctx.needs_input_grad[2] or ctx.needs_input_grad[3]
        if dy is None:
            return d1, d2, None, None, None, None, None, None, None
        a1 = None if d1 is None else d1.to(x1.dtype).contiguous()
        a2 = None if d2 is None else d2.to(x2.dtype).contiguous()
        dx1, dx2, dg, db = ops.backend().groupnorm_bwd(x1, x2, dy.contiguous(), stats, gamma, beta, a1, B, HW, G, silu,
                                                       want_param_grads=wp, add2=a2)
        return dx1, dx2, dg, db, None, None, None, None, None


def group_norm_skip(x1, x2, gamma, beta, B, HW, G, eps, silu):
    if not (torch.is_grad_enabled() and (x1.requires_grad or (x2 is not None and x2.requires_grad))):
        return GroupNormFn.apply(x1, x2, gamma, beta, B, HW, G, eps, silu), x1, x2
    out = GroupNormSkipFn.apply(x1, x2, gamma, beta, B, HW, G, eps, silu)
    return (out[0], out[1], None) if x2 is None else out


class LayerNormFn(torch.autograd.Function):
    @staticmethod
    def forward(ctx, x, gamma, beta, eps):
        y, stats = ops.backend().layernorm_fwd(x, gamma, beta, eps)
        ctx.save_for_backward(x, stats, gamma)
        return y

    @staticmethod
    def backward(ctx, dy):
        x, stats, gamma = ctx.saved_tensors
        wp = ctx.needs_input_grad[1] or ctx.needs_input_grad[2]
        dx, dg, db = ops.backend().layernorm_bwd(x, dy.contiguous(), gamma, stats, want_param_grads=wp)
        return dx, dg, db, None


def layer_norm(x, gamma, beta, eps=1e-5):
    return LayerNormFn.apply(x, gamma, beta, eps)


class LayerNormSkipFn(torch.autograd.Function):

    @staticmethod
    def forward(ctx, x, gamma, beta, eps):
        y, stats = ops.backend().layernorm_fwd(x, gamma, beta, eps)
        ctx.save_for_backward(x, stats, gamma)
        return y, x.view_as(x)

    @staticmethod
    def backward(ctx, dy, dskip):
        x, stats, gamma = ctx.saved_tensors
        wp = ctx.needs_input_grad[1] or ctx.needs_input_grad[2]
        if dy is None:
            return dskip, None, None, None
        add = None if dskip is None else dskip.to(x.dtype).contiguous()
        dx, dg, db = ops.backend().layernorm_bwd(x, dy.contiguous(), gamma, stats, want_param_grads=wp, add=add)
        return dx, dg, db, None


def layer_norm_skip(x, gamma, beta, eps=1e-5):
    if not (torch.is_grad_enabled() and x.requires_grad):
        return LayerNormFn.apply(x, gamma, beta, eps), x
    return LayerNormSkipFn.apply(x, gamma, beta, eps)


class AttentionFn(torch.autograd.Function):

    @staticmethod
    def forward(ctx, qkv, kv, B, H, T, S, DH, scale, causal=False):
        d = H * DH
        if kv is None:
            q, k, v = qkv[:, :d], qkv[:, d:2 * d], qkv[:, 2 * d:]
        else:
            q, k, v = qkv, kv[:, :d], kv[:, d:]
        o, lse = ops.backend().attention_fwd(q, k, v, B, H, T, S, DH, scale, causal=causal)
        ctx.save_for_backward(qkv, kv, o, lse)
        ctx.cfg = (B, H, T, S, DH, scale, causal)
        return o

    @staticmethod
    def backward(ctx, do):
        qkv, kv, o, lse = ctx.saved_tensors
        B, H, T, S, DH, scale, causal = ctx.cfg
        d = H * DH
        dqkv = torch.empty_like(qkv)
        dkv = torch.empty_like(kv) if kv is not None else None
        if kv is None:
            q, k, v = qkv[:, :d], qkv[:, d:2 * d], qkv[:, 2 * d:]
            dq, dk, dv = dqkv[:, :d], dqkv[:, d:2 * d], dqkv[:, 2 * d:]
        else:
            q, k, v = qkv, kv[:, :d], kv[:, d:]
            dq, dk, dv = dqkv, dkv[:, :d], dkv[:, d:]
        ops.backend().attention_bwd(q, k, v, o, do.contiguous(), lse, dq, dk, dv, B, H, T, S, DH, scale, causal=causal)
        return dqkv, dkv, None, None, None, None, None, None, None


def attention(qkv, kv, B, H, T, S, DH, scale, causal=False):
    return AttentionFn.apply(qkv, kv, B, H, T, S, DH, scale, causal)


class TomeMergeFn(torch.autograd.Function):

    @staticmethod
    def forward(ctx, x, plan):
        ctx.plan = plan
        return ops.backend().tome_merge(x, plan, mean=True)

    @staticmethod
    def backward(ctx, dy):
        return ops.backend().tome_unmerge(dy.contiguous(), ctx.plan, scale=True), None


class TomeUnmergeFn(torch.autograd.Function):

    @staticmethod
    def forward(ctx, y, residual, plan):
        ctx.plan = plan
        ctx.res_dtype = residual.dtype if residual is not None else None
        return ops.backend().tome_unmerge(y, plan, residual=residual)

    @staticmethod
    def backward(ctx, dout):
        dy = ops.backend().tome_merge(dout.contiguous(), ctx.plan, mean=False) if ctx.needs_input_grad[0] else None
        dres = None
        if ctx.res_dtype is not None and ctx.needs_input_grad[1]:
            dres = dout if dout.dtype == ctx.res_dtype else dout.to(ctx.res_dtype)
        return dy, dres, None


def tome_merge(x, plan):
    return TomeMergeFn.apply(x, plan)


def tome_unmerge(y, plan, residual=None):
    return TomeUnmergeFn.apply(y, residual, plan)


class GegluFn(torch.autograd.Function):
    @staticmethod
    def forward(ctx, u):
        ctx.save_for_backward(u)
        return ops.backend().geglu_fwd(u)

    @staticmethod
    def backward(ctx, dh):
        (u,) = ctx.saved_tensors
        return ops.backend().geglu_bwd(u, dh.contiguous())


def geglu(u):
    return GegluFn.apply(u)


class UnaryFn(torch.autograd.Function):
    @staticmethod
    def forward(ctx, x, op):
        ctx.save_for_backward(x)
        ctx.op = op
        return ops.backend().unary(x, op)

    @staticmethod
    def backward(ctx, dy):
        (x,) = ctx.saved_tensors
        return ops.backend().unary(x, ctx.op + 1, dy.contiguous()), None


def silu(x):
    return UnaryFn.apply(x, _C.OP_SILU)


def leaky_relu(x):
    return UnaryFn.apply(x, _C.OP_LRELU)


def gelu(x):
    return UnaryFn.apply(x, _C.OP_GELU)


def quick_gelu(x):
    return UnaryFn.apply(x, _C.OP_QGELU)


class MaskedMSEFn(torch.autograd.Function):

    @staticmethod
    def forward(ctx, pred, target, w):
        loss, wd, stats = ops.backend().masked_mse(pred, target, w, save=ctx.needs_input_grad[0])
        ctx.save_for_backward(wd, stats)
        return loss

    @staticmethod
    def backward(ctx, g):
        wd, stats = ctx.saved_tensors
        return ops.backend().masked_mse_bwd(wd, stats, g.contiguous().float()), None, None


def masked_mse(pred, target, w):
    be = ops.backend()
    if hasattr(be, "masked_mse"):
        return MaskedMSEFn.apply(pred.float(), target.float(), w.float())
    d = pred.float() - target.float()
    w = w.float()
    den = pred.shape[1] * torch.clamp(w.sum(), min=1.0)
    return (w.unsqueeze(1) * d * d).sum() / den


class WeightedMSEFn(torch.autograd.Function):

    @staticmethod
    def forward(ctx, pred, target, lam, w):
        loss, wd, stats = ops.backend().weighted_mse(pred, target, lam, w, save=ctx.needs_input_grad[0])
        ctx.save_for_backward(wd, stats)
        return loss

    @staticmethod
    def backward(ctx, g):
        wd, stats = ctx.saved_tensors
        return ops.backend().weighted_mse_bwd(wd, stats, g.contiguous().float()), None, None, None


def weighted_mse(pred, target, lam=None, w=None):
    be = ops.backend()
    if hasattr(be, "weighted_mse"):
        return WeightedMSEFn.apply(pred.float(), target.float(), None if lam is None else lam.detach().float(), None if w is None else w.float())
    d = pred.float() - target.float()
    B, C = pred.shape[0], pred.shape[1]
    if w is None:
        den = float(pred.numel())
        wl = torch.ones((B, 1, 1, 1), dtype=f32, device=pred.device) if lam is None else lam.detach().float().view(B, 1, 1, 1)
    else:
        w = w.float()
        den = C * torch.clamp(w.sum(), min=1.0)
        wl = w.unsqueeze(1) if lam is None else lam.detach().float().view(B, 1, 1, 1) * w.unsqueeze(1)
    return (wl * d * d).sum() / den


class RobustLossFn(torch.autograd.Function):

    @staticmethod
    def forward(ctx, pred, target, ctab, timesteps, kind, lam, w):
        loss, wd, stats = ops.backend().robust_loss(pred, target, ctab, timesteps, kind, lam, w, save=ctx.needs_input_grad[0])
        ctx.save_for_backward(wd, stats)
        return loss

    @staticmethod
    def backward(ctx, g):
        wd, stats = ctx.saved_tensors
        return ops.backend().robust_loss_bwd(wd, stats, g.contiguous().float()), None, None, None, None, None, None


ROBUST_KINDS = ("huber", "smooth_l1")


def robust_loss(pred, target, ctab, timesteps, kind="huber", lam=None, w=None):
    if kind not in ROBUST_KINDS:
        raise ValueError(f"robust_loss: kind={kind!r} must be one of {ROBUST_KINDS}")
    be = ops.backend()
    if hasattr(be, "robust_loss"):
        return RobustLossFn.apply(pred.float(), target.float(), ctab.float(), timesteps, kind, None if lam is None else lam.detach().float(),
                                  None if w is None else w.float())
    d = pred.float() - target.float()
    B, C = pred.shape[0], pred.shape[1]
    ctab = ctab.detach().float()
    c = (ctab[:1].expand(B) if timesteps is None else ctab[timesteps.clamp(0, ctab.shape[0] - 1)]).view(B, 1, 1, 1)
    d2 = d * d
    h = d2 / (torch.sqrt(d2 + c * c) + c)
    wl = 2.0 * c if kind == "huber" else torch.full_like(c, 2.0)
    if lam is not None:
        wl = lam.detach().float().view(B, 1, 1, 1) * wl
    if w is None:
        den = float(pred.numel())
    else:
        w = w.float()
        den = C * torch.clamp(w.sum(), min=1.0)
        wl = w.unsqueeze(1) * wl
    return (wl * h).sum() / den


def diffusion_objective(x0, noise, timesteps, coef, z=None, offset=0.0, v_prediction=False):
    if offset and z is None:
        raise ValueError("diffusion_objective: a noise offset needs its draw z [B, C]")
    if offset < 0:
        raise ValueError(f"diffusion_objective: offset={offset!r} must be >= 0")
    be = ops.backend()
    if hasattr(be, "diffuse"):
        return be.diffuse(x0.float(), noise.float(), timesteps, coef, z=None if not offset else z.float(), offset=float(offset),
                          v_prediction=v_prediction)
    x0, noise = x0.float(), noise.float()
    B = x0.shape[0]
    c = coef[timesteps.clamp(0, coef.shape[0] - 1)]
    a, s, lam = c[:, 0].view(B, 1, 1, 1), c[:, 1].view(B, 1, 1, 1), c[:, 2].contiguous()
    n1 = noise + (offset * z.float()).view(B, -1, 1, 1) if offset else noise
    noisy = a * x0 + s * n1
    target = a * n1 - s * x0 if v_prediction else n1
    return noisy, target, lam


class SpatialMeanFn(torch.autograd.Function):

    @staticmethod
    def forward(ctx, B, *maps):
        be = ops.backend()
        total = sum(m.shape[1] for m in maps)
        out = torch.empty((B, total), dtype=f32, device=maps[0].device)
        off, meta = 0, []
        for m in maps:
            hw = m.shape[0] // B
            be.spatial_mean(m, B, hw, out, off)
            meta.append((hw, m.shape[1], off))
            off += m.shape[1]
        ctx.meta, ctx.B = meta, B
        return out

    @staticmethod
    def backward(ctx, g):
        be = ops.backend()
        g = g.contiguous().float()
        outs = []
        for i, (hw, c, off) in enumerate(ctx.meta):
            outs.append(be.spatial_mean_bwd(g, None, ctx.B, hw, c, off) if ctx.needs_input_grad[1 + i] else None)
        return (None, *outs)


def spatial_mean_cat(B, maps):
    return SpatialMeanFn.apply(B, *maps)
```

e4t-diffusion_amd/e4t/ops.py:

```python
from __future__ import annotations

import contextlib
import ctypes as C
import gc
import os
import threading
from dataclasses import dataclass, field
from typing import List, Optional

import torch

from . import _C

bf16 = torch.bfloat16
f32 = torch.float32

ACT = bf16

_WEIGHTS_EPOCH = 0

capture_lock = threading.RLock()


@contextlib.contextmanager
def capture_guard():
    was_on = gc.isenabled()
    gc.collect()
    gc.disable()
    try:
        with capture_lock:
            yield
    finally:
        if was_on:
            gc.enable()


def weights_epoch() -> int:
    return _WEIGHTS_EPOCH


def bump_weights_epoch():
    global _WEIGHTS_EPOCH
    _WEIGHTS_EPOCH += 1


def _ptr(t: Optional[torch.Tensor]):
    return None if t is None else t.data_ptr()


_DEV_INDEX = None


def _stream():
    global _DEV_INDEX
    if _DEV_INDEX is None:
        _DEV_INDEX = torch.cuda.current_device()
    return torch._C._cuda_getCurrentRawStream(_DEV_INDEX)


def _rowmajor(t: torch.Tensor, name: str):
    if t.dim() < 2 or t.stride(-1) != 1:
        raise ValueError(f"{name}: expected a row-major matrix with unit inner stride, got strides {t.stride()}")



@dataclass
class WOEntry:
    row: int
    col: int
    W: torch.Tensor
    params: Optional[dict] = None
    weff: Optional[torch.Tensor] = None
    weffT: Optional[torch.Tensor] = None
    dweff: Optional[torch.Tensor] = None
    grads: Optional[dict] = None
    g_W: Optional[torch.Tensor] = None
    vecs: Optional[torch.Tensor] = None
    partial: Optional[torch.Tensor] = None
    mode: int = 0


@dataclass
class WOTable:
    entries: List[WOEntry]
    dev: Optional[torch.Tensor] = None
    _sig: tuple = field(default_factory=tuple)

    @property
    def max_row(self):
        return max(e.row for e in self.entries)

    @property
    def max_col(self):
        return max(e.col for e in self.entries)


class TomePlan:

    def __init__(self, buf: torch.Tensor, B: int, T: int, r: int):
        assert buf.dtype == torch.int32 and buf.dim() == 1 and buf.is_contiguous()
        assert T % 4 == 0 and 1 <= r <= T - T // 4 and buf.numel() >= B * (2 * T + T // 4 + 1)
        self.buf, self.B, self.T, self.r = buf, B, T, r
        self.nd, self.Tm = T // 4, T - r

    def _field(self, off, rows):
        return self.buf[off:off + self.B * rows].view(self.B, rows)

    @property
    def map(self):
        return self._field(0, self.T)

    @property
    def row_tok(self):
        return self._field(self.B * self.T, self.Tm)

    @property
    def seg_off(self):
        return self._field(self.B * (self.T + self.Tm), self.nd + 1)

    @property
    def seg_src(self):
        return self._field(self.B * (self.T + self.Tm + self.nd + 1), self.r)

    def fields(self):
        return {"map": self.map, "row_tok": self.row_tok, "seg_off": self.seg_off, "seg_src": self.seg_src}

    @classmethod
    def from_fields(cls, map, row_tok, seg_off, seg_src):
        B, T = map.shape
        r = seg_src.shape[1]
        buf = torch.cat([t.reshape(-1).to(torch.int32) for t in (map, row_tok, seg_off, seg_src)]).contiguous()
        return cls(buf, B, T, r)

    def to(self, device):
        n = self.B * (2 * self.T + self.nd + 1)
        return TomePlan(self.buf[:n].to(device), self.B, self.T, self.r)


class HipBackend:

    name = "hip"

    def __init__(self):
        self.lib = _C.load()
        self._ws = {}
        self.prof = None

    def _timed(self, key, flops, fn, nbytes=0.0):
        if self.prof is None:
            return fn()
        e0, e1 = torch.cuda.Event(enable_timing=True), torch.cuda.Event(enable_timing=True)
        e0.record()
        r = fn()
        e1.record()
        self.prof.append((key, flops, float(nbytes() if callable(nbytes) else nbytes), e0, e1))
        return r

    def _plan(self, fn, d, what):
        pl = _C.GemmPlan()
        _C.check(fn(C.byref(d), C.byref(pl)), what)
        return pl

    def workspace(self, nbytes: int, device) -> torch.Tensor:
        key = (device.type, device.index, _stream() if device.type == "cuda" else 0)
        ws = self._ws.get(key)
        if ws is None or ws.numel() < nbytes:
            ws = torch.empty(max(nbytes, 64 << 20), dtype=torch.uint8, device=device)
            self._ws[key] = ws
        return ws

    @staticmethod
    def _colstats_buf(out, M, N, wanted):
        if not wanted or out.dtype != bf16 or M % 32 or not out.is_contiguous():
            return None
        return torch.empty((M // 32, N, 2), dtype=f32, device=out.device)

    def gemm(self, a, b, *, a2=None, bias=None, residual=None, rowbias=None, rows_per_batch=0, out=None,
             out_dtype=bf16, gelu=False, accum=False, alpha=1.0, reduce_batch=False, tile=0, splitk=0, colstats=False, panels=None):
        batched = a.dim() == 3
        _rowmajor(a, "gemm A"); _rowmajor(b, "gemm B")
        if batched:
            nb, M, K = a.shape
            N = b.shape[1]
            sA, sB = a.stride(0), b.stride(0)
        else:
            nb, (M, K), N, sA, sB = 1, a.shape, b.shape[0], 0, 0
        if panels is not None:
            pr, ps, po, pc = panels
            assert not batched and out is not None and a.shape[0] >= (pc - 1) * ps + po + pr and out.shape[0] == a.shape[0], "gemm: bad row panels"
            assert residual is None or residual.shape[0] == a.shape[0]
            M = pr * pc
        K1 = K
        if a2 is not None:
            _rowmajor(a2, "gemm A2")
            K = K1 + a2.shape[-1]
        assert b.shape[-1] == K, f"gemm: B has K={b.shape[-1]}, A has K={K}"
        if out is None:
            shape = (M, N) if (not batched or reduce_batch) else (nb, M, N)
            out = torch.empty(shape, dtype=out_dtype, device=a.device)
        _rowmajor(out, "gemm C")
        d = _C.GemmDesc()
        d.A, d.A2, d.B, d.C = _ptr(a), _ptr(a2), _ptr(b), _ptr(out)
        d.bias, d.residual, d.rowbias = _ptr(bias), _ptr(residual), _ptr(rowbias)
        d.M, d.N, d.K, d.K1 = M, N, K, K1
        d.lda, d.lda2, d.ldb, d.ldc = a.stride(-2), (a2.stride(-2) if a2 is not None else 0), b.stride(-2), out.stride(-2)
        d.ldr = residual.stride(-2) if residual is not None else 0
        d.rows_per_batch = rows_per_batch
        d.ldrb = rowbias.stride(0) if rowbias is not None else 0
        flags = 0
        if out.dtype == f32:
            flags |= _C.OUT_F32
        if residual is not None and residual.dtype == f32:
            flags |= _C.RES_F32
        if gelu:
            flags |= _C.ACT_GELU
        if accum:
            flags |= _C.ACCUM
        if reduce_batch:
            flags |= _C.REDUCE_BATCH
        d.flags, d.tile, d.splitk, d.batch, d.alpha = flags, tile, splitk, nb, alpha
        d.strideA, d.strideB = sA, sB
        d.strideC = out.stride(0) if (batched and not reduce_batch) else 0
        d.strideBias = bias.stride(0) if (bias is not None and bias.dim() == 2) else 0
        if panels is not None:
            d.panel_rows, d.panel_stride, d.panel_off = panels[0], panels[1], panels[2]
        cs = self._colstats_buf(out, M, N, colstats and not batched)
        d.colstats = _ptr(cs)
        pl = self._plan(self.lib.e4t_gemm_plan, d, "e4t_gemm_plan")
        ws = self.workspace(pl.workspace_bytes, a.device) if pl.workspace_bytes else None
        d.workspace, d.workspace_bytes = _ptr(ws), (ws.numel() if ws is not None else 0)
        st = _stream()
        nbytes = lambda: (2.0 * nb * M * K + 2.0 * N * K * (nb if sB else 1) + out.element_size() * M * N * (1 if reduce_batch else nb) * (2 if accum else 1)
                          + (residual.element_size() * M * N if residual is not None else 0))
        rc = self._timed(f"gemm{pl.tile}" + (f"s{pl.stages}" if pl.stages else ""), 2.0 * M * N * K * nb,
                         lambda: _C.check(self.lib.e4t_gemm_nt(C.byref(d), st), "e4t_gemm_nt"), nbytes)
        if cs is not None and rc == 1:
            out._e4t_colstats = cs
        return out

    def _gemm_fused_geglu(self, key, flag, a, b, bias, M, N, K, flops, nbytes, aux=None):
        fwd = flag == _C.EPI_GEGLU
        for t, name in ((a, "A"), (b, "B")) + (() if fwd else ((aux, "aux"),)):
            _rowmajor(t, f"{key} {name}")
        d = _C.GemmDesc()
        d.A, d.B, d.bias = _ptr(a), _ptr(b), _ptr(bias)
        d.M, d.N, d.K, d.K1 = M, N, K, K
        d.lda, d.ldb = a.stride(0), b.stride(0)
        d.ldc, d.ldaux = (N, N // 2) if fwd else (2 * N, aux.stride(0))
        d.flags, d.batch, d.alpha = flag, 1, 1.0
        pl = _C.GemmPlan()
        rc = self.lib.e4t_gemm_plan(C.byref(d), C.byref(pl))
        if rc == _C.ERR_NO_FUSED:
            return None
        _C.check(rc, "e4t_gemm_plan")
        out = torch.empty((M, N if fwd else 2 * N), dtype=bf16, device=a.device)
        if fwd:
            aux = torch.empty((M, N // 2), dtype=bf16, device=a.device)
        d.C, d.aux = _ptr(out), _ptr(aux)
        st = _stream()
        self._timed(f"{key}{pl.tile}" + (f"s{pl.stages}" if pl.stages else ""), flops,
                    lambda: _C.check(self.lib.e4t_gemm_nt(C.byref(d), st), "e4t_gemm_nt"), nbytes)
        return (out, aux) if fwd else out

    def gemm_geglu(self, x, w, bias):
        (M, K), N = x.shape, w.shape[0]
        if x.dtype != bf16 or w.dtype != bf16 or N % 2 or w.shape[1] != K:
            return None
        return self._gemm_fused_geglu("gemm_geglu", _C.EPI_GEGLU, x, w, bias, M, N, K, 2.0 * M * N * K,
                                      2.0 * M * K + 2.0 * N * K + (4.0 * N if bias is not None else 0.0) + 3.0 * M * N)

    def gemm_geglu_bwd(self, dy, w2T, u):
        (M, K), H = dy.shape, w2T.shape[0]
        if dy.dtype != bf16 or w2T.dtype != bf16 or u.dtype != bf16 or u.shape != (M, 2 * H) or w2T.shape[1] != K:
            return None
        return self._gemm_fused_geglu("gemm_geglu_bwd", _C.EPI_GEGLU_BWD, dy, w2T, None, M, H, K, 2.0 * M * H * K,
                                      2.0 * M * K + 2.0 * H * K + 8.0 * M * H, aux=u)

    def gemm_tn(self, a, b, *, out=None, out_dtype=f32, accum=False, alpha=1.0, splitk=0):
        _rowmajor(a, "gemm_tn A"); _rowmajor(b, "gemm_tn B")
        K, M = a.shape
        N = b.shape[1]
        assert b.shape[0] == K
        if out is None:
            out = torch.empty((M, N), dtype=out_dtype, device=a.device)
        _rowmajor(out, "gemm_tn C")
        d = _C.GemmDesc()
        d.A, d.B, d.C = _ptr(a), _ptr(b), _ptr(out)
        d.M, d.N, d.K, d.K1 = M, N, K, K
        d.lda, d.ldb, d.ldc = a.stride(0), b.stride(0), out.stride(0)
        flags = (_C.OUT_F32 if out.dtype == f32 else 0) | (_C.ACCUM if accum else 0)
        d.flags, d.splitk, d.batch, d.alpha = flags, splitk, 1, alpha
        pl = self._plan(self.lib.e4t_gemm_tn_plan, d, "e4t_gemm_tn_plan")
        ws = self.workspace(pl.workspace_bytes, a.device) if pl.workspace_bytes else None
        d.workspace, d.workspace_bytes = _ptr(ws), (ws.numel() if ws is not None else 0)
        st = _stream()
        self._timed("gemm_tn", 2.0 * M * N * K, lambda: _C.check(self.lib.e4t_gemm_tn(C.byref(d), st), "e4t_gemm_tn"),
                    2.0 * K * (M + N) + out.element_size() * M * N * (2 if accum else 1))
        return out

    def conv3x3(self, x, w, B, Hin, Win, Hout, Wout, mode, *, colstats=False, bias=None, residual=None, rowbias=None, out=None,
                out_dtype=bf16, accum=False, tile=0, splitk=0):
        Cin, Cout = x.shape[-1], w.shape[0]
        assert x.is_contiguous() and w.is_contiguous() and w.shape[1] == 9 * Cin
        M = B * Hout * Wout
        if out is None:
            out = torch.empty((M, Cout), dtype=out_dtype, device=x.device)
        d = _C.ConvDesc()
        d.X, d.W, d.Y, d.bias, d.residual, d.rowbias = _ptr(x), _ptr(w), _ptr(out), _ptr(bias), _ptr(residual), _ptr(rowbias)
        d.B, d.Hin, d.Win, d.Cin, d.Hout, d.Wout, d.Cout = B, Hin, Win, Cin, Hout, Wout, Cout
        flags = 0
        if out.dtype == f32:
            flags |= _C.OUT_F32
        if residual is not None and residual.dtype == f32:
            flags |= _C.RES_F32
        if accum:
            flags |= _C.ACCUM
        d.mode, d.flags, d.tile, d.splitk = mode, flags, tile, splitk
        d.ldrb = rowbias.stride(0) if rowbias is not None else 0
        cs = self._colstats_buf(out, M, Cout, colstats)
        d.colstats = _ptr(cs)
        pl = self._plan(self.lib.e4t_conv3x3_plan, d, "e4t_conv3x3_plan")
        ws = self.workspace(pl.workspace_bytes, x.device) if pl.workspace_bytes else None
        d.workspace, d.workspace_bytes = _ptr(ws), (ws.numel() if ws is not None else 0)
        st = _stream()
        nbytes = 2.0 * B * Hin * Win * Cin + 2.0 * Cout * 9 * Cin + out.element_size() * M * Cout * (2 if accum else 1) + \
            (residual.element_size() * M * Cout if residual is not None else 0)
        rc = self._timed(f"conv{pl.tile}" + (f"s{pl.stages}" if pl.stages else ""), 2.0 * M * Cout * 9 * Cin,
                         lambda: _C.check(self.lib.e4t_conv3x3(C.byref(d), st), "e4t_conv3x3"), nbytes)
        if cs is not None and rc == 1:
            out._e4t_colstats = cs
        return out

    def conv_weight_prepare(self, w_oihw, Ipad=None, Opad=None, want_fwd=True, want_dgrad=True):
        O, I = w_oihw.shape[:2]
        Ipad = Ipad or (I + 63) // 64 * 64
        Opad = Opad or (O + 63) // 64 * 64
        w = w_oihw.detach().contiguous().float()
        wf = torch.empty((O, 9 * Ipad), dtype=bf16, device=w.device) if want_fwd else None
        wd = torch.empty((I, 9 * Opad), dtype=bf16, device=w.device) if want_dgrad else None
        _C.check(self.lib.e4t_conv_weight_prepare(_ptr(w), _ptr(wf), _ptr(wd), O, I, Ipad, Opad, _stream()), "e4t_conv_weight_prepare")
        return wf, wd

    def attention_fwd(self, q, k, v, B, H, T, S, DH, scale, out=None, need_lse=True, causal=False):
        for t in (q, k, v):
            _rowmajor(t, "attention operand")
        if out is None:
            out = torch.empty((B * T, H * DH), dtype=bf16, device=q.device)
        lse = torch.empty((B, H, T), dtype=f32, device=q.device) if need_lse else None
        ldq, ldk, ldv, ldo = q.stride(0), k.stride(0), v.stride(0), out.stride(0)
        st = _stream()
        self._timed(f"attn_fwd{DH}", 4.0 * B * H * T * S * DH, lambda: _C.check(self.lib.e4t_attention_fwd(
            _ptr(q), _ptr(k), _ptr(v), _ptr(out), _ptr(lse), B, H, T, S, DH, ldq, ldk, ldv, ldo,
            T * ldq, S * ldk, S * ldv, T * ldo, float(scale), int(causal), st), "e4t_attention_fwd"),
            2.0 * B * H * DH * (2 * T + 2 * S) + 4.0 * B * H * T)
        return out, lse

    def attention_bwd(self, q, k, v, o, do, lse, dq, dk, dv, B, H, T, S, DH, scale, causal=False):
        ldq, ldk, ldv, ldo = q.stride(0), k.stride(0), v.stride(0), o.stride(0)
        assert dq.stride(0) == ldq and dk.stride(0) == ldk and dv.stride(0) == ldv and do.stride(0) == ldo
        nws = self.lib.e4t_attention_bwd_workspace_floats(B, H, T, S, DH)
        ws = torch.empty(nws, dtype=f32, device=q.device)
        st = _stream()
        self._timed(f"attn_bwd{DH}", 10.0 * B * H * T * S * DH, lambda: _C.check(self.lib.e4t_attention_bwd_ws(
            _ptr(q), _ptr(k), _ptr(v), _ptr(o), _ptr(do), _ptr(lse), _ptr(ws), nws, _ptr(dq), _ptr(dk),
            _ptr(dv), B, H, T, S, DH, ldq, ldk, ldv, ldo, T * ldq, S * ldk, S * ldv, T * ldo,
            float(scale), int(causal), st), "e4t_attention_bwd_ws"), 2.0 * B * H * DH * (4 * T + 4 * S) + 8.0 * B * H * T)

    def groupnorm_fwd(self, x1, x2, gamma, beta, B, HW, G, eps, silu):
        C1, C2 = x1.shape[-1], (x2.shape[-1] if x2 is not None else 0)
        Cn = C1 + C2
        assert x1.is_contiguous() and (x2 is None or x2.is_contiguous())
        stats = torch.empty((B, G, 2), dtype=f32, device=x1.device)
        nb = self.lib.e4t_groupnorm_workspace_bytes(B, HW, Cn, G, 0)
        ws = self.workspace(nb, x1.device)
        y = torch.empty((B * HW, Cn), dtype=bf16, device=x1.device)
        cs1 = getattr(x1, "_e4t_colstats", None)
        cs2 = getattr(x2, "_e4t_colstats", None) if x2 is not None else None
        nblk, nch = HW // 32, self.lib.e4t_groupnorm_num_chunks(B, HW)
        if cs1 is not None and (x2 is None or cs2 is not None) and HW % 32 == 0 and nblk % min(nch, nblk) == 0:
            self._timed("gn_fwd_colstats", 0.0, lambda: _C.check(self.lib.e4t_groupnorm_fwd_cs(
                _ptr(x1), C1, _ptr(cs1), _ptr(x2), C2, _ptr(cs2), _ptr(gamma), _ptr(beta), _ptr(y), _ptr(stats),
                B, HW, G, float(eps), int(silu), _ptr(ws), ws.numel(), _stream()), "e4t_groupnorm_fwd_cs"), 4.0 * B * HW * Cn)
            return y, stats
        self._timed("gn_fwd_2pass", 0.0, lambda: _C.check(self.lib.e4t_groupnorm_fwd(
            _ptr(x1), C1, _ptr(x2), C2, _ptr(gamma), _ptr(beta), _ptr(y), _ptr(stats), B, HW, G, float(eps),
            int(silu), _ptr(ws), ws.numel(), _stream()), "e4t_groupnorm_fwd"), 6.0 * B * HW * Cn)
        return y, stats

    def groupnorm_fwd_unfused(self, x1, x2, gamma, beta, B, HW, G, eps, silu):
        C1, C2 = x1.shape[-1], (x2.shape[-1] if x2 is not None else 0)
        Cn = C1 + C2
        stats = torch.empty((B, G, 2), dtype=f32, device=x1.device)
        ws = self.workspace(self.lib.e4t_groupnorm_workspace_bytes(B, HW, Cn, G, 0), x1.device)
        _C.check(self.lib.e4t_groupnorm_stats(_ptr(x1), C1, _ptr(x2), C2, B, HW, G, float(eps), _ptr(stats), _ptr(ws), ws.numel(), _stream()),
                 "e4t_groupnorm_stats")
        y = torch.empty((B * HW, Cn), dtype=bf16, device=x1.device)
        _C.check(self.lib.e4t_groupnorm_apply(_ptr(x1), C1, _ptr(x2), C2, _ptr(stats), _ptr(gamma), _ptr(beta), _ptr(y), B, HW, G, int(silu), _stream()),
                 "e4t_groupnorm_apply")
        return y, stats

    def groupnorm_bwd(self, x1, x2, dy, stats, gamma, beta, add, B, HW, G, silu, want_param_grads=False, add2=None):
        C1, C2 = x1.shape[-1], (x2.shape[-1] if x2 is not None else 0)
        Cn = C1 + C2
        assert dy.is_contiguous() and (add is None or (add.is_contiguous() and add.shape == x1.shape and add.dtype == x1.dtype))
        assert add2 is None or (x2 is not None and add2.is_contiguous() and add2.shape == x2.shape and add2.dtype == x2.dtype)
        dx1 = torch.empty_like(x1)
        dx2 = torch.empty_like(x2) if x2 is not None else None
        ch = self.lib.e4t_groupnorm_num_chunks(B, HW)
        cpart = torch.empty((B * ch, Cn, 2), dtype=f32, device=x1.device) if want_param_grads else None
        nb = self.lib.e4t_groupnorm_workspace_bytes(B, HW, Cn, G, 0) + B * G * 8
        ws = self.workspace(nb, x1.device)
        self._timed("gn_bwd", 0.0, lambda: _C.check(self.lib.e4t_groupnorm_bwd(
            _ptr(x1), C1, _ptr(x2), C2, _ptr(dy), _ptr(stats), _ptr(gamma), _ptr(beta), _ptr(add), _ptr(add2), _ptr(dx1),
            _ptr(dx2), _ptr(cpart), B, HW, G, int(silu), _ptr(ws), ws.numel(), _stream()), "e4t_groupnorm_bwd"),
            2.0 * B * HW * (5 * Cn + (C1 if add is not None else 0) + (C2 if add2 is not None else 0)))
        dgamma = dbeta = None
        if want_param_grads:
            s = cpart.sum(dim=0)
            dbeta, dgamma = s[:, 0].contiguous(), s[:, 1].contiguous()
        return dx1, dx2, dgamma, dbeta

    def layernorm_fwd(self, x, gamma, beta, eps, need_stats=True):
        M, D = x.shape
        assert x.is_contiguous()
        y = torch.empty((M, D), dtype=bf16, device=x.device)
        stats = torch.empty((M, 2), dtype=f32, device=x.device) if need_stats else None
        fn, what = (self.lib.e4t_layernorm_fwd_f32, "e4t_layernorm_fwd_f32") if x.dtype == f32 else (self.lib.e4t_layernorm_fwd, "e4t_layernorm_fwd")
        self._timed("ln_fwd", 0.0, lambda: _C.check(fn(_ptr(x), _ptr(gamma), _ptr(beta), _ptr(y), _ptr(stats), M, D, float(eps), _stream()), what),
                    (x.element_size() + 2.0) * M * D)
        return y, stats

    def layernorm_bwd(self, x, dy, gamma, stats, want_param_grads=False, add=None):
        M, D = x.shape
        assert dy.is_contiguous() and (add is None or (add.is_contiguous() and add.shape == x.shape and add.dtype == x.dtype))
        dx = torch.empty_like(x)
        self._timed("ln_bwd", 0.0, lambda: _C.check(self.lib.e4t_layernorm_bwd(_ptr(x), _ptr(dy), _ptr(gamma), _ptr(stats), _ptr(add), _ptr(dx), M, D,
                                                                           _stream()), "e4t_layernorm_bwd"), 2.0 * M * D * (4 if add is not None else 3))
        dgamma = dbeta = None
        if want_param_grads:
            dgamma, dbeta = torch.empty(D, dtype=f32, device=x.device), torch.empty(D, dtype=f32, device=x.device)
            ws = self.workspace(2 * self.lib.e4t_colreduce_splits(M) * D * 4, x.device)
            _C.check(self.lib.e4t_layernorm_param_grad(_ptr(x), _ptr(dy), _ptr(stats), M, D, _ptr(dgamma), _ptr(dbeta), 0, _ptr(ws), ws.numel(),
                                                       _stream()), "e4t_layernorm_param_grad")
        return dx, dgamma, dbeta

    def colsum(self, x, out=None, accumulate=False):
        M, Cn = x.shape
        assert x.stride(1) == 1 and x.dtype == bf16
        if Cn % 8 or x.stride(0) % 8 or x.data_ptr() % 16:
            r = x.float().sum(0)
            return r if out is None else (out.add_(r) if accumulate else out.copy_(r))
        if out is None:
            out, accumulate = torch.empty(Cn, dtype=f32, device=x.device), False
        assert out.dtype == f32 and out.is_contiguous() and out.numel() == Cn
        ws = self.workspace(self.lib.e4t_colreduce_splits(M) * Cn * 4, x.device)
        _C.check(self.lib.e4t_colsum(_ptr(x), x.stride(0), M, Cn, _ptr(out), int(accumulate), _ptr(ws), ws.numel(), _stream()), "e4t_colsum")
        return out

    def geglu_fwd(self, u):
        M, H2 = u.shape
        h = torch.empty((M, H2 // 2), dtype=bf16, device=u.device)
        self._timed("geglu_fwd", 0.0, lambda: _C.check(self.lib.e4t_geglu_fwd(_ptr(u), _ptr(h), M, H2 // 2, _stream()), "e4t_geglu_fwd"), 3.0 * M * H2)
        return h

    def geglu_bwd(self, u, dh):
        du = torch.empty_like(u)
        self._timed("geglu_bwd", 0.0, lambda: _C.check(self.lib.e4t_geglu_bwd(_ptr(u), _ptr(dh), _ptr(du), u.shape[0], u.shape[1] // 2, _stream()),
                                                       "e4t_geglu_bwd"), 5.0 * u.shape[0] * u.shape[1])
        return du

    def unary(self, x, op, dy=None):
        assert x.is_contiguous() and (dy is None or dy.is_contiguous())
        y = torch.empty_like(x)
        _C.check(self.lib.e4t_unary(_ptr(x), _ptr(dy), _ptr(y), x.numel(), op, _stream()), "e4t_unary")
        return y

    def add(self, a, b):
        assert a.is_contiguous() and b.is_contiguous() and a.shape == b.shape
        y = torch.empty_like(a)
        _C.check(self.lib.e4t_add(_ptr(a), _ptr(b), _ptr(y), a.numel(), _stream()), "e4t_add")
        return y

    def transpose(self, x, pad_to=0):
        _rowmajor(x, "transpose input")
        R, Cn = x.shape
        ldo = max(R, pad_to)
        out = torch.zeros((Cn, ldo), dtype=bf16, device=x.device) if ldo > R else torch.empty((Cn, ldo), dtype=bf16, device=x.device)
        _C.check(self.lib.e4t_transpose(_ptr(x), _ptr(out), 1, R, Cn, x.stride(0), ldo, 0, 0, _stream()), "e4t_transpose")
        return out

    def sumpool2(self, x, B, H, W):
        Cn = x.shape[-1]
        out = torch.empty((B * H * W, Cn), dtype=bf16, device=x.device)
        _C.check(self.lib.e4t_sumpool2(_ptr(x), _ptr(out), B, H, W, Cn, _stream()), "e4t_sumpool2")
        return out

    def spatial_mean(self, x, B, HW, out, coff):
        _C.check(self.lib.e4t_spatial_mean(_ptr(x), _ptr(out), B, HW, x.shape[-1], out.stride(0), coff, _stream()), "e4t_spatial_mean")

    def spatial_mean_bwd(self, g, base, B, HW, Cn, coff):
        dx = torch.empty((B * HW, Cn), dtype=bf16, device=g.device)
        _C.check(self.lib.e4t_spatial_mean_bwd(_ptr(g), _ptr(base), _ptr(dx), B, HW, Cn, g.stride(0), coff, _stream()), "e4t_spatial_mean_bwd")
        return dx

    def timestep_embedding(self, t, dim):
        t = t.to(torch.int64).contiguous()
        out = torch.empty((t.shape[0], dim), dtype=bf16, device=t.device)
        _C.check(self.lib.e4t_timestep_embedding(_ptr(t), _ptr(out), t.shape[0], dim, _stream()), "e4t_timestep_embedding")
        return out

    def clip_preprocess(self, pixels, S, P, Kpad):
        pixels = pixels.float().contiguous()
        B, _, Hin, Win = pixels.shape
        g = S // P
        out = torch.zeros((B * g * g, Kpad), dtype=bf16, device=pixels.device)
        _C.check(self.lib.e4t_clip_preprocess(_ptr(pixels), _ptr(out), B, Hin, Win, S, P, Kpad, _stream()), "e4t_clip_preprocess")
        return out

    def guided_step(self, pred, sample, coef, noise=None, cfg=True, pred_nhwc=False, out=None):
        B, Cn = sample.shape[0], sample.shape[1]
        HW = sample.numel() // (B * Cn)
        assert pred.dtype == f32 and sample.dtype == f32 and coef.dtype == f32 and coef.numel() == 4
        assert pred.is_contiguous() and sample.is_contiguous() and pred.numel() == sample.numel() * (2 if cfg else 1)
        assert noise is None or (noise.dtype == f32 and noise.is_contiguous() and noise.shape == sample.shape)
        if out is None:
            out = torch.empty_like(sample)
        _C.check(self.lib.e4t_guided_step(_ptr(pred), _ptr(sample), _ptr(noise), _ptr(out), _ptr(coef), B, Cn, HW, int(cfg), int(pred_nhwc), _stream()),
                 "e4t_guided_step")
        return out

    def sampler_step(self, pred, x, row, hist=None, saved=None, noise=None, x_in=None, cfg=True, pred_nhwc=False, out=None, edit=None):
        B, Cn = x.shape[0], x.shape[1]
        HW = x.numel() // (B * Cn)
        assert pred.dtype == f32 and x.dtype == f32 and row.dtype == f32 and row.numel() == _C.SAMPLER_ROW and row.is_contiguous()
        assert pred.is_contiguous() and x.is_contiguous() and pred.numel() == x.numel() * (2 if cfg else 1)
        for t in (saved, noise):
            assert t is None or (t.dtype == f32 and t.is_contiguous() and t.shape == x.shape)
        K = 0
        if hist is not None:
            K = hist.shape[0]
            assert hist.dtype == f32 and hist.is_contiguous() and tuple(hist.shape[1:]) == tuple(x.shape) and K <= _C.SAMPLER_MAX_HIST
        copies = 0
        if x_in is not None:
            assert x_in.dtype == f32 and x_in.is_contiguous() and x_in.numel() % x.numel() == 0
            copies = x_in.numel() // x.numel()
        if out is None:
            out = torch.empty_like(x)
        assert out.dtype == f32 and out.is_contiguous() and out.shape == x.shape
        if edit is not None:
            keep, x0, n0 = edit
            for t in edit:
                assert t.dtype == f32 and t.is_contiguous() and t.device == x.device
            assert keep.numel() in (HW, B * HW) and x0.numel() in (Cn * HW, B * Cn * HW) and n0.shape == x.shape
            _C.check(self.lib.e4t_sampler_step_edit(_ptr(pred), _ptr(x), _ptr(out), _ptr(hist), _ptr(saved), _ptr(noise), _ptr(x_in), _ptr(row),
                                                    _ptr(keep), _ptr(x0), _ptr(n0), B, Cn, HW, K, int(cfg), int(pred_nhwc), copies,
                                                    int(B > 1 and keep.numel() == B * HW), int(B > 1 and x0.numel() == B * Cn * HW), _stream()),
                     "e4t_sampler_step_edit")
            return out
        _C.check(self.lib.e4t_sampler_step(_ptr(pred), _ptr(x), _ptr(out), _ptr(hist), _ptr(saved), _ptr(noise), _ptr(x_in), _ptr(row),
                                           B, Cn, HW, K, int(cfg), int(pred_nhwc), copies, _stream()), "e4t_sampler_step")
        return out

    def sampler_step_edit(self, pred, x, row, keep, x0, n0, **kw):
        return self.sampler_step(pred, x, row, edit=(keep, x0, n0), **kw)

    def image_prep(self, pool, table, B, S, out=None):
        assert pool.dtype == torch.uint8 and table.dtype == torch.int64 and table.shape == (B, 8) and table.is_contiguous()
        if out is None:
            out = torch.empty((B, 3, S, S), dtype=torch.float32, device=pool.device)
        _C.check(self.lib.e4t_image_prep(_ptr(pool), _ptr(table), _ptr(out), B, S, _stream()), "e4t_image_prep")
        return out

    def mask_prep(self, pool, table, mask_off, B, S, out=None):
        assert pool.dtype == torch.uint8 and table.dtype == torch.int64 and table.shape == (B, 8) and table.is_contiguous()
        assert mask_off.dtype == torch.int64 and mask_off.shape == (B,) and mask_off.is_contiguous() and S % 8 == 0
        if out is None:
            out = torch.empty((B, S // 8, S // 8), dtype=torch.float32, device=pool.device)
        _C.check(self.lib.e4t_mask_prep(_ptr(pool), _ptr(table), _ptr(mask_off), _ptr(out), B, S, _stream()), "e4t_mask_prep")
        return out

    def masked_mse(self, pred, target, w, save=True):
        B, Cn = pred.shape[0], pred.shape[1]
        HW = pred.numel() // (B * Cn)
        assert pred.dtype == f32 and target.dtype == f32 and w.dtype == f32 and pred.dim() == 4
        assert target.shape == pred.shape and w.numel() == B * HW
        nhwc = not pred.is_contiguous() and pred.permute(0, 2, 3, 1).is_contiguous()
        if not nhwc:
            pred = pred.contiguous()
        target, w = target.contiguous(), w.contiguous()
        wd = torch.empty_like(pred) if save else None
        stats = torch.empty(_C.MASKED_MSE_STATS, dtype=f32, device=pred.device)
        _C.check(self.lib.e4t_masked_mse_fwd(_ptr(pred), _ptr(target), _ptr(w), _ptr(wd), _ptr(stats), B, Cn, HW, int(nhwc), _stream()),
                 "e4t_masked_mse_fwd")
        return stats[0], wd, stats

    def masked_mse_bwd(self, wd, stats, g):
        assert g.dtype == f32 and g.numel() == 1 and wd.dtype == f32
        dpred = torch.empty_like(wd)
        _C.check(self.lib.e4t_masked_mse_bwd(_ptr(wd), _ptr(stats), _ptr(g), _ptr(dpred), wd.numel(), _stream()), "e4t_masked_mse_bwd")
        return dpred

    def weighted_mse(self, pred, target, lam=None, w=None, save=True):
        B, Cn = pred.shape[0], pred.shape[1]
        HW = pred.numel() // (B * Cn)
        assert pred.dtype == f32 and target.dtype == f32 and pred.dim() == 4 and target.shape == pred.shape
        assert w is None or (w.dtype == f32 and w.numel() == B * HW)
        assert lam is None or (lam.dtype == f32 and lam.numel() == B)
        nhwc = not pred.is_contiguous() and pred.permute(0, 2, 3, 1).is_contiguous()
        if not nhwc:
            pred = pred.contiguous()
        target = target.contiguous()
        w = None if w is None else w.contiguous()
        lam = None if lam is None else lam.contiguous()
        wd = torch.empty_like(pred) if save else None
        stats = torch.empty(_C.MASKED_MSE_STATS, dtype=f32, device=pred.device)
        _C.check(self.lib.e4t_weighted_mse_fwd(_ptr(pred), _ptr(target), _ptr(w), _ptr(lam), _ptr(wd), _ptr(stats), B, Cn, HW, int(nhwc), _stream()),
                 "e4t_weighted_mse_fwd")
        return stats[0], wd, stats

    def weighted_mse_bwd(self, wd, stats, g):
        return self.masked_mse_bwd(wd, stats, g)

    def robust_loss(self, pred, target, ctab, timesteps, kind, lam=None, w=None, save=True):
        B, Cn = pred.shape[0], pred.shape[1]
        HW = pred.numel() // (B * Cn)
        kind = {"huber": _C.LOSS_HUBER, "smooth_l1": _C.LOSS_SMOOTH_L1}.get(kind, kind)
        assert pred.dtype == f32 and target.dtype == f32 and pred.dim() == 4 and target.shape == pred.shape
        assert ctab.dtype == f32 and ctab.dim() == 1 and ctab.device == pred.device
        assert timesteps is None or (timesteps.dtype == torch.int64 and timesteps.numel() == B and timesteps.device == pred.device)
        assert w is None or (w.dtype == f32 and w.numel() == B * HW)
        assert lam is None or (lam.dtype == f32 and lam.numel() == B)
        nhwc = not pred.is_contiguous() and pred.permute(0, 2, 3, 1).is_contiguous()
        if not nhwc:
            pred = pred.contiguous()
        target, ctab = target.contiguous(), ctab.contiguous()
        timesteps = None if timesteps is None else timesteps.contiguous()
        w = None if w is None else w.contiguous()
        lam = None if lam is None else lam.contiguous()
        wd = torch.empty_like(pred) if save else None
        stats = torch.empty(_C.MASKED_MSE_STATS, dtype=f32, device=pred.device)
        _C.check(self.lib.e4t_robust_loss_fwd(_ptr(pred), _ptr(target), _ptr(w), _ptr(lam), _ptr(ctab), _ptr(timesteps), _ptr(wd), _ptr(stats), B, Cn, HW,
                                              ctab.numel(), int(kind), int(nhwc), _stream()), "e4t_robust_loss_fwd")
        return stats[0], wd, stats

    def robust_loss_bwd(self, wd, stats, g):
        return self.masked_mse_bwd(wd, stats, g)

    def diffuse(self, x0, noise, timesteps, coef, z=None, offset=0.0, v_prediction=False):
        B, Cn = x0.shape[0], x0.shape[1]
        HW = x0.numel() // (B * Cn)
        assert x0.dtype == f32 and noise.dtype == f32 and x0.dim() == 4 and noise.shape == x0.shape
        assert timesteps.dtype == torch.int64 and timesteps.numel() == B and coef.dtype == f32 and coef.dim() == 2 and coef.shape[1] == 3
        assert z is None or (z.dtype == f32 and z.numel() == B * Cn)
        x0, noise, timesteps, coef = x0.contiguous(), noise.contiguous(), timesteps.contiguous(), coef.contiguous()
        z = None if z is None else z.contiguous()
        noisy, target = torch.empty_like(x0), torch.empty_like(x0)
        lam = torch.empty(B, dtype=f32, device=x0.device)
        _C.check(self.lib.e4t_diffuse(_ptr(x0), _ptr(noise), _ptr(z), _ptr(timesteps), _ptr(coef), _ptr(noisy), _ptr(target), _ptr(lam), B, Cn, HW,
                                      coef.shape[0], float(offset), int(bool(v_prediction)), _stream()), "e4t_diffuse")
        return noisy, target, lam

    def adamw(self, p, g, m, v, lr, beta1, beta2, eps, wd, step, grad_scale=1.0):
        self._timed("adamw", 0.0, lambda: _C.check(self.lib.e4t_adamw(_ptr(p), _ptr(g), _ptr(m), _ptr(v), p.numel(), lr, beta1, beta2, eps, wd, step,
                                                                      grad_scale, _stream()), "e4t_adamw"), 28.0 * p.numel())

    def adamw_hyper(self, p, g, m, v, hyper, beta1, beta2, eps, wd):
        self._timed("adamw", 0.0, lambda: _C.check(self.lib.e4t_adamw_hyper(_ptr(p), _ptr(g), _ptr(m), _ptr(v), p.numel(), _ptr(hyper), beta1, beta2, eps, wd,
                                                                            _stream()), "e4t_adamw_hyper"), 28.0 * p.numel())

    def adamw_rank(self, p, m, v, G, Z, lr, beta1, beta2, eps, wd, step, grad_scale=1.0, hyper=None):
# ... 173 lines not shown
```

include/e4t_hip.h:

```cpp
#ifndef E4T_HIP_H
#define E4T_HIP_H
#include <stddef.h>
#include <stdint.h>

#ifdef __cplusplus
extern "C" {
#endif

typedef void* e4t_stream;

int e4t_version(void);
const char* e4t_last_error(void);
int e4t_device_info(char* arch, int arch_len, int* cu_count);
int e4t_set_launch_log(const char* path);

#define E4T_OUT_F32 1
#define E4T_RES_F32 2
#define E4T_ACT_GELU 4
#define E4T_ACCUM 8
#define E4T_REDUCE_BATCH 16
#define E4T_EPI_GEGLU 32
#define E4T_EPI_GEGLU_BWD 64
#define E4T_ERR_NO_FUSED (-95)

typedef struct {
  const void* A;
  const void* A2;
  const void* B;
  void* C;
  const float* bias;
  const void* residual;
  const float* rowbias;
  void* workspace;
  size_t workspace_bytes;
  int M, N, K, K1;
  int lda, lda2, ldb, ldc, ldr;
  int rows_per_batch;
  int flags;
  int tile;
  int splitk;
  int batch;
  long long strideA, strideB, strideC, strideBias;
  float alpha;
  int ldrb;
  float* colstats;
  int panel_rows;
  int panel_stride;
  int panel_off;
  void* aux;
  int ldaux;
} e4t_gemm_desc;
int e4t_gemm_nt(const e4t_gemm_desc* d, e4t_stream stream);
int e4t_gemm_tn(const e4t_gemm_desc* d, e4t_stream stream);

#define E4T_CONV_S1 1
#define E4T_CONV_S2 2
#define E4T_CONV_UP2 3
#define E4T_CONV_S2T 4
#define E4T_CONV_S2A 5
typedef struct {
  const void* X;
  const void* W;
  void* Y;
  const float* bias;
  const void* residual;
  const float* rowbias;
  void* workspace;
  size_t workspace_bytes;
  int B, Hin, Win, Cin, Hout, Wout, Cout;
  int mode, flags, tile, splitk;
  int ldrb;
  float* colstats;
} e4t_conv_desc;
int e4t_conv3x3(const e4t_conv_desc* d, e4t_stream stream);

typedef struct {
  int tile, tile_m, tile_n;
  int splitk;
  size_t workspace_bytes;
  int tail_rows;
  int stages;
} e4t_gemm_plan_t;
int e4t_gemm_plan(const e4t_gemm_desc* d, e4t_gemm_plan_t* out);
int e4t_gemm_tn_plan(const e4t_gemm_desc* d, e4t_gemm_plan_t* out);
int e4t_conv3x3_plan(const e4t_conv_desc* d, e4t_gemm_plan_t* out);
int e4t_conv3x3_kernel(const e4t_conv_desc* d, const char** symbol, int* splitk);
#define E4T_STORE_BF16_STAGED 0
#define E4T_STORE_F32_DIRECT 1
#define E4T_STORE_SCALAR 2
#define E4T_STORE_SPLITK_PARTIAL 3
typedef struct {
  const char* symbol;
  const char* reduce;
  int splitk;
  int tail_rows;
  int store;
  int colstats;
} e4t_gemm_kernel_t;
int e4t_gemm_kernel(const e4t_gemm_desc* d, e4t_gemm_kernel_t* out);
int e4t_gemm_tn_kernel(const e4t_gemm_desc* d, e4t_gemm_kernel_t* out);

int e4t_attention_fwd(const void* Q, const void* K, const void* V, void* O, float* lse, int B, int H, int T, int S, int DH,
                      int ldq, int ldk, int ldv, int ldo, long long bq, long long bk, long long bv, long long bo,
                      float scale, int causal , e4t_stream stream);
int e4t_attention_bwd(const void* Q, const void* K, const void* V, const void* O, const void* dO, const float* lse,
                      float* delta_ws, void* dQ, void* dK, void* dV, int B, int H, int T, int S, int DH, int ldq, int ldk,
                      int ldv, int ldo, long long bq, long long bk, long long bv, long long bo, float scale, int causal,
                      e4t_stream stream);
size_t e4t_attention_bwd_workspace_floats(int B, int H, int T, int S, int DH);
int e4t_attention_bwd_ws(const void* Q, const void* K, const void* V, const void* O, const void* dO, const float* lse,
                         float* ws, size_t ws_floats, void* dQ, void* dK, void* dV, int B, int H, int T, int S, int DH, int ldq,
                         int ldk, int ldv, int ldo, long long bq, long long bk, long long bv, long long bo, float scale,
                         int causal, e4t_stream stream);
typedef struct {
  const char* fwd;
  const char* dq;
  const char* dkv;
  int tsplit, tchunk, dkv_occ;
  size_t workspace_floats;
} e4t_attention_plan_t;
int e4t_attention_plan(int B, int H, int T, int S, int DH, int causal, size_t ws_floats, e4t_attention_plan_t* out);

int e4t_groupnorm_num_chunks(int B, int HW);
size_t e4t_groupnorm_workspace_bytes(int B, int HW, int C, int G, int with_param_grads);
int e4t_groupnorm_stats(const void* x1, int C1, const void* x2, int C2, int B, int HW, int G, float eps,
                        float* mean_rstd , void* workspace, size_t ws_bytes, e4t_stream stream);
int e4t_groupnorm_apply(const void* x1, int C1, const void* x2, int C2, const float* mean_rstd, const float* gamma,
                        const float* beta, void* y , int B, int HW, int G, int silu,
                        e4t_stream stream);
int e4t_groupnorm_fwd(const void* x1, int C1, const void* x2, int C2, const float* gamma, const float* beta, void* y,
                      float* mean_rstd , int B, int HW, int G, float eps, int silu, void* workspace,
                      size_t ws_bytes, e4t_stream stream);
int e4t_groupnorm_fwd_cs(const void* x1, int C1, const float* cs1, const void* x2, int C2, const float* cs2, const float* gamma,
                         const float* beta, void* y, float* mean_rstd, int B, int HW, int G, float eps, int silu, void* workspace,
                         size_t ws_bytes , e4t_stream stream);
int e4t_groupnorm_bwd(const void* x1, int C1, const void* x2, int C2, const void* dy, const float* mean_rstd,
                      const float* gamma, const float* beta, const void* add1, const void* add2, void* dx1, void* dx2,
                      float* dgamma_dbeta_partial, int B, int HW, int G, int silu, void* workspace, size_t ws_bytes,
                      e4t_stream stream);
int e4t_layernorm_fwd(const void* x, const float* gamma, const float* beta, void* y, float* mean_rstd ,
                      int M, int D, float eps, e4t_stream stream);
int e4t_layernorm_fwd_f32(const float* x, const float* gamma, const float* beta, void* y, float* mean_rstd, int M, int D, float eps,
                          e4t_stream stream);
int e4t_layernorm_bwd(const void* x, const void* dy, const float* gamma, const float* mean_rstd, const void* add, void* dx,
                      int M, int D, e4t_stream stream);
int e4t_colreduce_splits(int M);
int e4t_colsum(const void* x, int ldx, int M, int C, float* out, int accumulate, void* workspace, size_t ws_bytes, e4t_stream stream);
int e4t_layernorm_param_grad(const void* x, const void* dy, const float* mean_rstd, int M, int D, float* dgamma, float* dbeta,
                             int accumulate, void* workspace, size_t ws_bytes, e4t_stream stream);

#define E4T_WO_STORE_F32 1
#define E4T_WO_OFFSETS_ONLY 2
typedef struct {
  const float *v, *w1, *b1, *w2, *b2, *wc, *bc, *wr, *br;
  const float* W;
  float* vecs;
  float* partial;
  void* weff;
  void* weffT;
  const float* dweff;
  float *g_v, *g_w1, *g_b1, *g_w2, *g_b2, *g_wc, *g_bc, *g_wr, *g_br;
  float* g_W;
  int row, col, ld_weff, ld_weffT, ld_dweff;
  int mode;
} e4t_wo_desc;
size_t e4t_wo_vecs_floats(int row, int col);
size_t e4t_wo_partial_floats(int row, int col);
int e4t_wo_forward(const e4t_wo_desc* descs_dev, int n, int max_row, int max_col, e4t_stream stream);
int e4t_wo_backward(const e4t_wo_desc* descs_dev, int n, int max_row, int max_col, int accumulate, e4t_stream stream);
int e4t_weight_prepare(const e4t_wo_desc* descs_dev, int n, int max_row, int max_col, e4t_stream stream);
int e4t_conv_weight_prepare(const float* w_oihw, void* w_fwd, void* w_dgrad, int O, int I, int Ipad, int Opad, e4t_stream stream);

int e4t_geglu_fwd(const void* u , void* h , long long M, int H, e4t_stream stream);
int e4t_geglu_bwd(const void* u, const void* dh, void* du, long long M, int H, e4t_stream stream);
#define E4T_OP_SILU 0
#define E4T_OP_SILU_BWD 1
#define E4T_OP_GELU 2
#define E4T_OP_GELU_BWD 3
#define E4T_OP_LRELU 4
#define E4T_OP_LRELU_BWD 5
#define E4T_OP_QGELU 6
#define E4T_OP_QGELU_BWD 7
int e4t_unary(const void* x, const void* dy, void* y, long long n, int op, e4t_stream stream);
int e4t_add(const void* a, const void* b, void* y, long long n, e4t_stream stream);
int e4t_transpose(const void* in, void* out, int batch, int R, int C, int ldi, int ldo, long long bsi, long long bso, e4t_stream stream);
int e4t_sumpool2(const void* in , void* out , int B, int H, int W, int C, e4t_stream stream);
int e4t_spatial_mean(const void* x, float* out, int B, int HW, int C, int ldo, int coff, e4t_stream stream);
int e4t_spatial_mean_bwd(const float* g, const void* base, void* dx, int B, int HW, int C, int ldg, int coff, e4t_stream stream);
int e4t_timestep_embedding(const long long* t, void* out , int B, int dim, e4t_stream stream);
int e4t_clip_preprocess(const float* pixels_nchw, void* patches , int B, int Hin, int Win, int S, int P, int Kpad, e4t_stream stream);
int e4t_guided_step(const float* pred, const float* sample, const float* noise, float* out, const float* coef,
                    int B, int C, int HW, int cfg, int pred_nhwc, e4t_stream stream);
#define E4T_SAMPLER_MAX_HIST 4
#define E4T_SAMPLER_ROW 16
int e4t_sampler_step(const float* pred, const float* x, float* out, float* hist, float* saved, const float* noise, float* x_in,
                     const float* row, int B, int C, int HW, int K, int cfg, int pred_nhwc, int x_in_copies, e4t_stream stream);
int e4t_sampler_step_edit(const float* pred, const float* x, float* out, float* hist, float* saved, const float* noise, float* x_in,
                          const float* row, const float* keep, const float* x0, const float* n0, int B, int C, int HW, int K, int cfg,
                          int pred_nhwc, int x_in_copies, int keep_per_image, int x0_per_image, e4t_stream stream);
int e4t_image_prep(const void* pool, const long long* table, float* out, int B, int S, e4t_stream stream);
int e4t_mask_prep(const void* pool, const long long* table, const long long* mask_off, float* out , int B, int S, e4t_stream stream);
#define E4T_MASKED_MSE_STATS 2050
int e4t_masked_mse_fwd(const float* pred, const float* target, const float* w, float* wd, float* stats, int B, int C, int HW, int pred_nhwc,
                       e4t_stream stream);
int e4t_masked_mse_bwd(const float* wd, const float* stats, const float* g, float* dpred, long long n, e4t_stream stream);
int e4t_weighted_mse_fwd(const float* pred, const float* target, const float* w, const float* lam, float* wd, float* stats, int B, int C, int HW,
                         int pred_nhwc, e4t_stream stream);
#define E4T_LOSS_HUBER 1
#define E4T_LOSS_SMOOTH_L1 2
int e4t_robust_loss_fwd(const float* pred, const float* target, const float* w, const float* lam, const float* ctab, const long long* timesteps,
                        float* wd, float* stats, int B, int C, int HW, int T, int kind, int pred_nhwc, e4t_stream stream);
int e4t_diffuse(const float* x0, const float* noise, const float* z, const long long* timesteps, const float* coef, float* noisy, float* target,
                float* lam, int B, int C, int HW, int T, float s, int v_prediction, e4t_stream stream);
int e4t_softmax_rows(void* x, long long rows, int L, int ld, e4t_stream stream);
int e4t_im2col3_rgb(const float* pixels_nchw, void* out, int B, int H, int W, e4t_stream stream);
int e4t_im2col_T(const void* x, void* out, int B, int Hin, int Win, int C, int Hout, int Wout, int ldo, int mode, e4t_stream stream);
int e4t_im2col(const void* x, void* out, int B, int Hin, int Win, int C, int Hout, int Wout, int mode, e4t_stream stream);
int e4t_adamw(float* p, const float* g, float* m, float* v, long long n, float lr, float beta1, float beta2, float eps,
              float weight_decay, int step, float grad_scale, e4t_stream stream);
int e4t_adamw_hyper(float* p, const float* g, float* m, float* v, long long n, const float* hyper_dev, float beta1, float beta2, float eps,
                    float weight_decay, e4t_stream stream);
int e4t_adamw_rank(float* p, float* m, float* v, const void* G, const void* Z, int n, int rows, int cols, int K, int ldg, long long ldz,
                   float lr, float beta1, float beta2, float eps, float weight_decay, int step, float grad_scale, const float* hyper_dev,
                   e4t_stream stream);
int e4t_adamw_ema(float* p, const float* g, float* m, float* v, float* ema, long long n, float lr, float beta1, float beta2, float eps,
                  float weight_decay, int step, float grad_scale, float ema_w, const float* hyper_dev, e4t_stream stream);
int e4t_adamw_rank_ema(float* p, float* m, float* v, float* ema, const void* G, const void* Z, int n, int rows, int cols, int K, int ldg,
                       long long ldz, float lr, float beta1, float beta2, float eps, float weight_decay, int step, float grad_scale, float ema_w,
                       const float* hyper_dev, e4t_stream stream);
int e4t_ema_update(float* ema, const float* p, long long n, float ema_w, const float* w_dev, e4t_stream stream);
int e4t_adamw8(float* p, const float* g, void* qm, void* qv, float* absmax_m, float* absmax_v, float* ema, long long n, const float* code_m,
               const float* code_v, float lr, float beta1, float beta2, float eps, float weight_decay, int step, float grad_scale, float ema_w,
               const float* hyper_dev, e4t_stream stream);
int e4t_sumsq_partial(const float* g, long long n, float* partial, int nblocks, e4t_stream stream);

size_t e4t_tome_plan_ints(int T, int r);
int e4t_tome_match(const void* x, int ldx, int B, int h, int w, int d, int r, const int* choice, int* plan, e4t_stream stream);
int e4t_tome_merge(const void* x, int ldx, const int* plan, void* y, int ldy, int B, int T, int r, int d, int mean, e4t_stream stream);
int e4t_tome_unmerge(const void* y, int ldy, const int* plan, const void* residual, void* x_out, int ldx, int B, int T, int r, int d,
                     int scale_inv_count, e4t_stream stream);

typedef struct e4t_comm* e4t_comm_t;
#define E4T_COMM_F32 0
#define E4T_COMM_BF16 1
#define E4T_COMM_SUM 0
#define E4T_COMM_AVG 1
#define E4T_COMM_MIN 2
#define E4T_COMM_MAX 3
int e4t_comm_unique_id(void* id128);
int e4t_comm_init(e4t_comm_t* comm, const void* id128, int rank, int world);
int e4t_comm_allreduce(e4t_comm_t comm, void* buf, long long count, int dtype, int op, e4t_stream stream);
int e4t_comm_allgather(e4t_comm_t comm, const void* send, void* recv , long long count, int dtype, e4t_stream stream);
int e4t_comm_wait(e4t_comm_t comm, e4t_stream stream);
int e4t_comm_info(e4t_comm_t comm, int* rank, int* world, e4t_stream* comm_stream);
int e4t_comm_destroy(e4t_comm_t comm);

int e4t_probe_mfma_layout(float* out_rows , float* out_cols , e4t_stream stream);

#ifdef __cplusplus
}
#endif
#endif
```

Baseline: 168.6 images/s.

## Add specialized short-KV attention kernels staging all keys in LDS

Adds dedicated forward and backward attention kernels for short key lengths (up to 96), such as SD cross-attention over 77 text tokens. Each block stages the whole K/V sequence into LDS once and splits the work over query chunks, with a planner that picks chunking and an optional partial dK/dV reduction. The generic flash-attention loop tiles keys and pays per-tile overhead, which is wasteful when S is tiny. The cost is a new code path, extra workspace for the split reductions, and shared helpers moved into a common header.

Measured after the change: 169.2 images/s (median of 6 runs). No clear change (+0.4%).

```diff
diff --git a/e4t-diffusion_amd/csrc/attention.hip b/e4t-diffusion_amd/csrc/attention.hip
--- a/e4t-diffusion_amd/csrc/attention.hip
+++ b/e4t-diffusion_amd/csrc/attention.hip
@@ -1,27 +1,9 @@
-#include "common.h"
+#include "attention_common.h"
 #include "../../include/e4t_hip.h"
 #include <math.h>
 #include <type_traits>
 
 namespace {
-
-struct AttnArgs {
-  const bf16_t *Q, *K, *V, *dO;
-  const bf16_t* O;
-  bf16_t *Out, *dQ, *dK, *dV;
-  float* L;
-  float* Delta;
-  float* LD;
-  int T, S, H;
-  int ldq, ldk, ldv, ldo;
-  long long bq, bk, bv, bo;
-  float scale2;
-  float scale;
-  int causal;
-  int xcd_raster;
-  float* part;
-  int tsplit, tchunk;
-};
 
 struct Blk { int x, h, b; };
 __device__ __forceinline__ Blk xcd_block(int on) {
@@ -37,59 +19,6 @@
 }
 
 template <int DH>
-struct Cfg {
-  static constexpr int DK = (DH + 15) / 16 * 16;
-  static constexpr int DV = (DH + 31) / 32 * 32;
-  static constexpr int NKS = DK / 16;
-  static constexpr int NDT = DV / 32;
-  static constexpr int LDE = DH <= 128 ? 128 : 256;
-  static constexpr int NCH = DH / 8;
-  static constexpr int NIT = (32 * NCH + 255) / 256;
-};
-
-union Frag {
-  bf16x8 v;
-  uint4 q;
-  uint2 h[2];
-  uint32_t w[4];
-};
-
-__device__ __forceinline__ float xhalf_max(float v) {
-  float a = v, b = v;
-  asm volatile("s_nop 1\n\tv_permlane32_swap_b32 %0, %1\n\ts_nop 1\n\tv_max_f32 %0, %0, %1" : "+v"(a), "+v"(b));
-  return a;
-}
-__device__ __forceinline__ float xhalf_sum(float v) {
-  float a = v, b = v;
-  asm volatile("s_nop 1\n\tv_permlane32_swap_b32 %0, %1\n\ts_nop 1\n\tv_add_f32 %0, %0, %1" : "+v"(a), "+v"(b));
-  return a;
-}
-
-__device__ __forceinline__ f32x16 mfma32(bf16x8 a, bf16x8 b, f32x16 c) { return __builtin_amdgcn_mfma_f32_32x32x16_bf16(a, b, c, 0, 0, 0); }
-
-__device__ __forceinline__ float fast_exp2(float x) { return __builtin_amdgcn_exp2f(x); }
-
-typedef float f32x2 __attribute__((ext_vector_type(2)));
-constexpr bool PK_REG = true;
-constexpr bool PK_DMA = false;
-template <bool PK>
-__device__ __forceinline__ f32x2 pk_fma(f32x2 a, f32x2 b, f32x2 c) {
-  if constexpr (PK) return __builtin_elementwise_fma(a, b, c);
-  else return f32x2{__builtin_fmaf(a.x, b.x, c.x), __builtin_fmaf(a.y, b.y, c.y)};
-}
-template <bool PK>
-__device__ __forceinline__ f32x2 pk_mul(f32x2 a, f32x2 b) {
-  if constexpr (PK) return a * b;
-  else return f32x2{a.x * b.x, a.y * b.y};
-}
-
-
-template <int LDE>
-__device__ __forceinline__ int img_off(int r, int L) {
-  return r * LDE + (((((L >> 2) ^ (r & 3)) << 2) | ((L & 3) ^ ((r >> 2) & 3))) << 3);
-}
-
-template <int DH>
 struct TileRegs {
   using C = Cfg<DH>;
   uint4 v[C::NIT][2];
@@ -131,80 +60,6 @@
   if (PADC > 0)
     for (int i = threadIdx.x; i < 64 * PADC; i += 256)
       *(uint4*)(lds + img_off<Cfg<DH>::LDE>(i / PADC, Cfg<DH>::NCH + i % PADC)) = make_uint4(0, 0, 0, 0);
-}
-
-template <int DH>
-__device__ __forceinline__ void load_row_frags(const bf16_t* g, int ld, int row, int R, int hi, bf16x8* f) {
-#pragma unroll
-  for (int ks = 0; ks < Cfg<DH>::NKS; ++ks) {
-    Frag t;
-    t.q = make_uint4(0, 0, 0, 0);
-    const int d0 = ks * 16 + hi * 8;
-    if (row < R && d0 < DH) t.q = *(const uint4*)(g + (long long)row * ld + d0);
-    f[ks] = t.v;
-  }
-}
-
-template <int DH>
-struct FragOff {
-  using C = Cfg<DH>;
-  int row[C::NKS], tr_lo[C::NDT], tr_hi[C::NDT];
-  __device__ __forceinline__ FragOff() {
-    const int lane = threadIdx.x & 63, li = lane & 31, hi = lane >> 5, il = lane & 15, d16 = (lane >> 4) & 1;
-#pragma unroll
-    for (int ks = 0; ks < C::NKS; ++ks) row[ks] = img_off<C::LDE>(li, ks * 2 + hi);
-#pragma unroll
-    for (int dt = 0; dt < C::NDT; ++dt) {
-      const int L = dt * 4 + 2 * d16 + ((il & 3) >> 1), r = 4 * hi + (il >> 2);
-      tr_lo[dt] = img_off<C::LDE>(r, L) + 4 * (il & 1);
-      tr_hi[dt] = img_off<C::LDE>(r + 8, L) + 4 * (il & 1);
-    }
-  }
-};
-template <int DH>
-__device__ __forceinline__ bf16x8 load_row_frag(const bf16_t* img, const FragOff<DH>& f, int sub, int ks) {
-  return *(const bf16x8*)(img + sub * 32 * Cfg<DH>::LDE + f.row[ks]);
-}
-template <int DH>
-__device__ __forceinline__ bf16x8 load_T_frag(const bf16_t* img, const FragOff<DH>& f, int dt, int sub, int k2) {
-  const bf16_t* b = img + (sub * 32 + k2 * 16) * Cfg<DH>::LDE;
-  return tr_frag(b + f.tr_lo[dt], b + f.tr_hi[dt]);
-}
-__device__ __forceinline__ bf16x8 pack_acc(const float* p, int k2) {
-  Frag t;
-#pragma unroll
-  for (int j = 0; j < 4; ++j) t.w[j] = pack2bf(p[8 * k2 + 2 * j], p[8 * k2 + 2 * j + 1]);
-  return t.v;
-}
-__device__ __forceinline__ int acc_row(int r, int hi) { return (r & 3) + 8 * (r >> 2) + 4 * hi; }
-
-template <int DH>
-__device__ __forceinline__ void store_T_acc(const f32x16* acc, float mul, bf16_t* g, int ld, int row, int R, int hi) {
-  if (row >= R) return;
-#pragma unroll
-  for (int dt = 0; dt < Cfg<DH>::NDT; ++dt)
-#pragma unroll
-    for (int rg = 0; rg < 4; ++rg) {
-      const int d = dt * 32 + 8 * rg + 4 * hi;
-      if (d < DH) {
-        float f[4];
-#pragma unroll
-        for (int j = 0; j < 4; ++j) f[j] = acc[dt][rg * 4 + j] * mul;
-        *(uint2*)(g + (long long)row * ld + d) = pack4(f);
-      }
-    }
-}
-
-template <int DH>
-__device__ __forceinline__ void store_T_acc_f32(const f32x16* acc, float* g, int row, int R, int hi) {
-  if (row >= R) return;
-#pragma unroll
-  for (int dt = 0; dt < Cfg<DH>::NDT; ++dt)
-#pragma unroll
-    for (int rg = 0; rg < 4; ++rg) {
-      const int d = dt * 32 + 8 * rg + 4 * hi;
-      if (d < DH) *(float4*)(g + (size_t)row * DH + d) = make_float4(acc[dt][rg * 4], acc[dt][rg * 4 + 1], acc[dt][rg * 4 + 2], acc[dt][rg * 4 + 3]);
-    }
 }
 
 template <int DH>
@@ -579,24 +434,6 @@
 }
 
 template <int DH>
-__device__ __forceinline__ float row_delta(const bf16_t* o_base, int ldo, int row, int R, int hi, const bf16x8* dof) {
-  bf16x8 of[Cfg<DH>::NKS];
-  load_row_frags<DH>(o_base, ldo, row, R, hi, of);
-  float s = 0.f;
-#pragma unroll
-  for (int ks = 0; ks < Cfg<DH>::NKS; ++ks) {
-    Frag a, g;
-    a.v = of[ks]; g.v = dof[ks];
-    float x[8], y[8];
-    unpack8(a.q, x);
-    unpack8(g.q, y);
-#pragma unroll
-    for (int k = 0; k < 8; ++k) s = fmaf(x[k], y[k], s);
-  }
-  return s + __shfl_xor(s, 32, 64);
-}
-
-template <int DH>
 __global__ __launch_bounds__(256, (DH <= 64 ? 3 : DH <= 80 ? 2 : 1)) void attn_bwd_dq_kernel(AttnArgs p) {
   using C = Cfg<DH>;
   __shared__ __attribute__((aligned(16))) bf16_t Ks[64 * C::LDE];
@@ -1055,28 +892,6 @@
   asm volatile("" : "+v"(krow));
   store_T_acc<DH>(dvt, 1.f, p.dV + b * p.bv + h * DH, p.ldv, krow, p.S, hi);
   store_T_acc<DH>(dkt, p.scale, p.dK + b * p.bk + h * DH, p.ldk, krow, p.S, hi);
-}
-
-template <int DH>
-__global__ __launch_bounds__(256) void attn_dkv_reduce_kernel(AttnArgs p, int Bn) {
-  constexpr int D4 = DH / 4;
-  const long long per = (long long)p.S * D4, total = (long long)Bn * p.H * 2 * per;
-  const size_t slab = (size_t)Bn * p.H * 2 * p.S * DH;
-  for (long long i = (long long)blockIdx.x * 256 + threadIdx.x; i < total; i += (long long)gridDim.x * 256) {
-    const long long bh2 = i / per;
-    const int rem = (int)(i - bh2 * per), key = rem / D4, d = (rem - key * D4) * 4;
-    const int which = (int)(bh2 & 1), h = (int)((bh2 >> 1) % p.H), b = (int)((bh2 >> 1) / p.H);
-    const float* src = p.part + (size_t)bh2 * p.S * DH + (size_t)key * DH + d;
-    float4 a = *(const float4*)src;
-    for (int t = 1; t < p.tsplit; ++t) {
-      const float4 v = *(const float4*)(src + (size_t)t * slab);
-      a.x += v.x; a.y += v.y; a.z += v.z; a.w += v.w;
-    }
-    const float mul = which ? p.scale : 1.f;
-    const float f[4] = {a.x * mul, a.y * mul, a.z * mul, a.w * mul};
-    bf16_t* dst = which ? p.dK + b * p.bk + (long long)key * p.ldk + h * DH + d : p.dV + b * p.bv + (long long)key * p.ldv + h * DH + d;
-    *(uint2*)dst = pack4(f);
-  }
 }
 
 struct AttnKernel { void (*fn)(AttnArgs); const char* text; int rows; };
diff --git a/e4t-diffusion_amd/csrc/attention_common.h b/e4t-diffusion_amd/csrc/attention_common.h
--- /dev/null
+++ b/e4t-diffusion_amd/csrc/attention_common.h
@@ -0,0 +1,191 @@
+#pragma once
+#include "common.h"
+#include <math.h>
+
+namespace {
+
+struct AttnArgs {
+  const bf16_t *Q, *K, *V, *dO;
+  const bf16_t* O;
+  bf16_t *Out, *dQ, *dK, *dV;
+  float* L;
+  float* Delta;
+  float* LD;
+  int T, S, H;
+  int ldq, ldk, ldv, ldo;
+  long long bq, bk, bv, bo;
+  float scale2;
+  float scale;
+  int causal;
+  int xcd_raster;
+  float* part;
+  int tsplit, tchunk;
+};
+
+template <int DH>
+struct Cfg {
+  static constexpr int DK = (DH + 15) / 16 * 16;
+  static constexpr int DV = (DH + 31) / 32 * 32;
+  static constexpr int NKS = DK / 16;
+  static constexpr int NDT = DV / 32;
+  static constexpr int LDE = DH <= 128 ? 128 : 256;
+  static constexpr int NCH = DH / 8;
+  static constexpr int NIT = (32 * NCH + 255) / 256;
+};
+
+union Frag {
+  bf16x8 v;
+  uint4 q;
+  uint2 h[2];
+  uint32_t w[4];
+};
+
+__device__ __forceinline__ float xhalf_max(float v) {
+  float a = v, b = v;
+  asm volatile("s_nop 1\n\tv_permlane32_swap_b32 %0, %1\n\ts_nop 1\n\tv_max_f32 %0, %0, %1" : "+v"(a), "+v"(b));
+  return a;
+}
+__device__ __forceinline__ float xhalf_sum(float v) {
+  float a = v, b = v;
+  asm volatile("s_nop 1\n\tv_permlane32_swap_b32 %0, %1\n\ts_nop 1\n\tv_add_f32 %0, %0, %1" : "+v"(a), "+v"(b));
+  return a;
+}
+
+__device__ __forceinline__ f32x16 mfma32(bf16x8 a, bf16x8 b, f32x16 c) { return __builtin_amdgcn_mfma_f32_32x32x16_bf16(a, b, c, 0, 0, 0); }
+
+__device__ __forceinline__ float fast_exp2(float x) { return __builtin_amdgcn_exp2f(x); }
+
+typedef float f32x2 __attribute__((ext_vector_type(2)));
+constexpr bool PK_REG = true;
+constexpr bool PK_DMA = false;
+template <bool PK>
+__device__ __forceinline__ f32x2 pk_fma(f32x2 a, f32x2 b, f32x2 c) {
+  if constexpr (PK) return __builtin_elementwise_fma(a, b, c);
+  else return f32x2{__builtin_fmaf(a.x, b.x, c.x), __builtin_fmaf(a.y, b.y, c.y)};
+}
+template <bool PK>
+__device__ __forceinline__ f32x2 pk_mul(f32x2 a, f32x2 b) {
+  if constexpr (PK) return a * b;
+  else return f32x2{a.x * b.x, a.y * b.y};
+}
+
+template <int LDE>
+__device__ __forceinline__ int img_off(int r, int L) {
+  return r * LDE + (((((L >> 2) ^ (r & 3)) << 2) | ((L & 3) ^ ((r >> 2) & 3))) << 3);
+}
+
+template <int DH>
+__device__ __forceinline__ void load_row_frags(const bf16_t* g, int ld, int row, int R, int hi, bf16x8* f) {
+#pragma unroll
+  for (int ks = 0; ks < Cfg<DH>::NKS; ++ks) {
+    Frag t;
+    t.q = make_uint4(0, 0, 0, 0);
+    const int d0 = ks * 16 + hi * 8;
+    if (row < R && d0 < DH) t.q = *(const uint4*)(g + (long long)row * ld + d0);
+    f[ks] = t.v;
+  }
+}
+
+template <int DH>
+struct FragOff {
+  using C = Cfg<DH>;
+  int row[C::NKS], tr_lo[C::NDT], tr_hi[C::NDT];
+  __device__ __forceinline__ FragOff() {
+    const int lane = threadIdx.x & 63, li = lane & 31, hi = lane >> 5, il = lane & 15, d16 = (lane >> 4) & 1;
+#pragma unroll
+    for (int ks = 0; ks < C::NKS; ++ks) row[ks] = img_off<C::LDE>(li, ks * 2 + hi);
+#pragma unroll
+    for (int dt = 0; dt < C::NDT; ++dt) {
+      const int L = dt * 4 + 2 * d16 + ((il & 3) >> 1), r = 4 * hi + (il >> 2);
+      tr_lo[dt] = img_off<C::LDE>(r, L) + 4 * (il & 1);
+      tr_hi[dt] = img_off<C::LDE>(r + 8, L) + 4 * (il & 1);
+    }
+  }
+};
+template <int DH>
+__device__ __forceinline__ bf16x8 load_row_frag(const bf16_t* img, const FragOff<DH>& f, int sub, int ks) {
+  return *(const bf16x8*)(img + sub * 32 * Cfg<DH>::LDE + f.row[ks]);
+}
+template <int DH>
+__device__ __forceinline__ bf16x8 load_T_frag(const bf16_t* img, const FragOff<DH>& f, int dt, int sub, int k2) {
+  const bf16_t* b = img + (sub * 32 + k2 * 16) * Cfg<DH>::LDE;
+  return tr_frag(b + f.tr_lo[dt], b + f.tr_hi[dt]);
+}
+__device__ __forceinline__ bf16x8 pack_acc(const float* p, int k2) {
+  Frag t;
+#pragma unroll
+  for (int j = 0; j < 4; ++j) t.w[j] = pack2bf(p[8 * k2 + 2 * j], p[8 * k2 + 2 * j + 1]);
+  return t.v;
+}
+__device__ __forceinline__ int acc_row(int r, int hi) { return (r & 3) + 8 * (r >> 2) + 4 * hi; }
+
+template <int DH>
+__device__ __forceinline__ void store_T_acc(const f32x16* acc, float mul, bf16_t* g, int ld, int row, int R, int hi) {
+  if (row >= R) return;
+#pragma unroll
+  for (int dt = 0; dt < Cfg<DH>::NDT; ++dt)
+#pragma unroll
+    for (int rg = 0; rg < 4; ++rg) {
+      const int d = dt * 32 + 8 * rg + 4 * hi;
+      if (d < DH) {
+        float f[4];
+#pragma unroll
+        for (int j = 0; j < 4; ++j) f[j] = acc[dt][rg * 4 + j] * mul;
+        *(uint2*)(g + (long long)row * ld + d) = pack4(f);
+      }
+    }
+}
+
+template <int DH>
+__device__ __forceinline__ void store_T_acc_f32(const f32x16* acc, float* g, int row, int R, int hi) {
+  if (row >= R) return;
+#pragma unroll
+  for (int dt = 0; dt < Cfg<DH>::NDT; ++dt)
+#pragma unroll
+    for (int rg = 0; rg < 4; ++rg) {
+      const int d = dt * 32 + 8 * rg + 4 * hi;
+      if (d < DH) *(float4*)(g + (size_t)row * DH + d) = make_float4(acc[dt][rg * 4], acc[dt][rg * 4 + 1], acc[dt][rg * 4 + 2], acc[dt][rg * 4 + 3]);
+    }
+}
+
+template <int DH>
+__device__ __forceinline__ float row_delta(const bf16_t* o_base, int ldo, int row, int R, int hi, const bf16x8* dof) {
+  bf16x8 of[Cfg<DH>::NKS];
+  load_row_frags<DH>(o_base, ldo, row, R, hi, of);
+  float s = 0.f;
+#pragma unroll
+  for (int ks = 0; ks < Cfg<DH>::NKS; ++ks) {
+    Frag a, g;
+    a.v = of[ks]; g.v = dof[ks];
+    float x[8], y[8];
+    unpack8(a.q, x);
+    unpack8(g.q, y);
+#pragma unroll
+    for (int k = 0; k < 8; ++k) s = fmaf(x[k], y[k], s);
+  }
+  return s + __shfl_xor(s, 32, 64);
+}
+
+template <int DH>
+__global__ __launch_bounds__(256) void attn_dkv_reduce_kernel(AttnArgs p, int Bn) {
+  constexpr int D4 = DH / 4;
+  const long long per = (long long)p.S * D4, total = (long long)Bn * p.H * 2 * per;
+  const size_t slab = (size_t)Bn * p.H * 2 * p.S * DH;
+  for (long long i = (long long)blockIdx.x * 256 + threadIdx.x; i < total; i += (long long)gridDim.x * 256) {
+    const long long bh2 = i / per;
+    const int rem = (int)(i - bh2 * per), key = rem / D4, d = (rem - key * D4) * 4;
+    const int which = (int)(bh2 & 1), h = (int)((bh2 >> 1) % p.H), b = (int)((bh2 >> 1) / p.H);
+    const float* src = p.part + (size_t)bh2 * p.S * DH + (size_t)key * DH + d;
+    float4 a = *(const float4*)src;
+    for (int t = 1; t < p.tsplit; ++t) {
+      const float4 v = *(const float4*)(src + (size_t)t * slab);
+      a.x += v.x; a.y += v.y; a.z += v.z; a.w += v.w;
+    }
+    const float mul = which ? p.scale : 1.f;
+    const float f[4] = {a.x * mul, a.y * mul, a.z * mul, a.w * mul};
+    bf16_t* dst = which ? p.dK + b * p.bk + (long long)key * p.ldk + h * DH + d : p.dV + b * p.bv + (long long)key * p.ldv + h * DH + d;
+    *(uint2*)dst = pack4(f);
+  }
+}
+
+}
diff --git a/e4t-diffusion_amd/csrc/attention_short.hip b/e4t-diffusion_amd/csrc/attention_short.hip
--- /dev/null
+++ b/e4t-diffusion_amd/csrc/attention_short.hip
@@ -0,0 +1,438 @@
+#include "attention_common.h"
+#include "../../include/e4t_hip.h"
+
+namespace {
+
+constexpr int SHORT_MAX_S = 96, SHORT_KB = SHORT_MAX_S / 32;
+
+template <int DH, int ROWS, int NT, int FLIP>
+__device__ __forceinline__ void stage_rows(bf16_t* img, __amdgpu_buffer_rsrc_t rs, int ld, int row0, int nrows) {
+  using C = Cfg<DH>;
+  constexpr int SL = C::DV / 8;
+  for (int i = threadIdx.x; i < ROWS * SL; i += NT) {
+    const int r = i / SL, L = i - r * SL;
+    const unsigned vo = (L < C::NCH && row0 + r < nrows) ? (unsigned)(((row0 + r) * ld + L * 8) * 2) : 0x80000000u;
+    *(uint4*)(img + (img_off<C::LDE>(r, L) ^ FLIP)) = buf_load16(rs, vo, 0);
+  }
+}
+
+template <int DH>
+constexpr int PAIR_FLIP = Cfg<DH>::DV <= 64 ? 64 : 0;
+template <int DH>
+struct FragOffPair : FragOff<DH> {
+  __device__ __forceinline__ FragOffPair() {
+#pragma unroll
+    for (int ks = 0; ks < Cfg<DH>::NKS; ++ks) this->row[ks] ^= PAIR_FLIP<DH>;
+#pragma unroll
+    for (int dt = 0; dt < Cfg<DH>::NDT; ++dt) { this->tr_lo[dt] ^= PAIR_FLIP<DH>; this->tr_hi[dt] ^= PAIR_FLIP<DH>; }
+  }
+};
+
+template <int DH>
+__global__ __launch_bounds__(256, (DH <= 64 ? 4 : 2)) void attn_short_fwd_kernel(AttnArgs p, int qchunk) {
+  using C = Cfg<DH>;
+  constexpr int IMG = SHORT_MAX_S * C::LDE, FLIP = PAIR_FLIP<DH>;
+  __shared__ __attribute__((aligned(16))) bf16_t lds[FLIP ? IMG : 2 * IMG];
+  bf16_t* const Ks = lds;
+  bf16_t* const Vs = FLIP ? lds : lds + IMG;
+  const FragOff<DH> fo;
+  const FragOffPair<DH> fov;
+  const int b = blockIdx.z, h = blockIdx.y;
+  const int lane = threadIdx.x & 63, wave = threadIdx.x >> 6;
+  const int li = lane & 31, hi = lane >> 5;
+  const int q_begin = blockIdx.x * qchunk, q_end = min(p.T, q_begin + qchunk);
+  const bf16_t* Qb = p.Q + b * p.bq + h * DH;
+  const bf16_t* Kb = p.K + b * p.bk + h * DH;
+  const bf16_t* Vb = p.V + b * p.bv + h * DH;
+  bf16_t* Ob = p.Out + b * p.bo + h * DH;
+  float* Lb = p.L ? p.L + ((long long)b * p.H + h) * p.T : nullptr;
+
+  bf16x8 qf[C::NKS];
+  load_row_frags<DH>(Qb, p.ldq, q_begin + wave * 32 + li, p.T, hi, qf);
+  stage_rows<DH, SHORT_MAX_S, 256, 0>(Ks, make_rsrc(Kb, (unsigned)(((long long)(p.S - 1) * p.ldk + DH) * 2)), p.ldk, 0, p.S);
+  stage_rows<DH, SHORT_MAX_S, 256, FLIP>(Vs, make_rsrc(Vb, (unsigned)(((long long)(p.S - 1) * p.ldv + DH) * 2)), p.ldv, 0, p.S);
+  __syncthreads();
+
+  for (int q0 = q_begin + wave * 32; q0 < q_end; q0 += 128) {
+    const int q = q0 + li;
+    bf16x8 qn[C::NKS];
+    load_row_frags<DH>(Qb, p.ldq, q0 + 128 < q_end ? q + 128 : p.T, p.T, hi, qn);
+
+    f32x16 s[SHORT_KB];
+#pragma unroll
+    for (int kb = 0; kb < SHORT_KB; ++kb) {
+#pragma unroll
+      for (int r = 0; r < 16; ++r) s[kb][r] = 0.f;
+#pragma unroll
+      for (int ks = 0; ks < C::NKS; ++ks) s[kb] = mfma32(load_row_frag<DH>(Ks, fo, kb, ks), qf[ks], s[kb]);
+      if ((kb + 1) * 32 > p.S) {
+#pragma unroll
+        for (int r = 0; r < 16; ++r) s[kb][r] = kb * 32 + acc_row(r, hi) < p.S ? s[kb][r] : -INFINITY;
+      }
+    }
+    float mx = -INFINITY;
+#pragma unroll
+    for (int kb = 0; kb < SHORT_KB; ++kb)
+#pragma unroll
+      for (int r = 0; r < 16; ++r) mx = fmaxf(mx, s[kb][r]);
+    const float m = xhalf_max(mx) * p.scale2;
+
+    f32x16 o[C::NDT];
+#pragma unroll
+    for (int dt = 0; dt < C::NDT; ++dt)
+#pragma unroll
+      for (int r = 0; r < 16; ++r) o[dt][r] = 0.f;
+    float l = 0.f;
+#pragma unroll
+    for (int kb = 0; kb < SHORT_KB; ++kb) {
+      float pr[16];
+#pragma unroll
+      for (int r = 0; r < 16; r += 2) {
+        const f32x2 t = pk_fma<PK_REG>(f32x2{s[kb][r], s[kb][r + 1]}, f32x2{p.scale2, p.scale2}, f32x2{-m, -m});
+        pr[r] = fast_exp2(t.x); pr[r + 1] = fast_exp2(t.y);
+        l += pr[r] + pr[r + 1];
+      }
+      const bf16x8 pf0 = pack_acc(pr, 0), pf1 = pack_acc(pr, 1);
+#pragma unroll
+      for (int dt = 0; dt < C::NDT; ++dt) {
+        o[dt] = mfma32(load_T_frag<DH>(Vs, fov, dt, kb, 0), pf0, o[dt]);
+        o[dt] = mfma32(load_T_frag<DH>(Vs, fov, dt, kb, 1), pf1, o[dt]);
+      }
+    }
+    l = xhalf_sum(l);
+    store_T_acc<DH>(o, 1.f / l, Ob, p.ldo, q, p.T, hi);
+    if (Lb && hi == 0 && q < p.T) Lb[q] = m + log2f(l);
+#pragma unroll
+    for (int ks = 0; ks < C::NKS; ++ks) qf[ks] = qn[ks];
+  }
+}
+
+constexpr int BWD_QT = 32;
+
+template <int DH>
+__global__ __launch_bounds__(256, (DH <= 64 ? 3 : 2)) void attn_short_bwd_kernel(AttnArgs p) {
+  using C = Cfg<DH>;
+  constexpr int FLIP = PAIR_FLIP<DH>, NIMG = FLIP ? 1 : 2;
+  constexpr int IMG = SHORT_MAX_S * C::LDE, TIMG = BWD_QT * C::LDE;
+  constexpr int NIT = (BWD_QT * C::NCH + 255) / 256;
+  __shared__ __attribute__((aligned(16))) bf16_t lds[NIMG * (IMG + TIMG) + 4 * BWD_QT];
+  bf16_t* const Qs = lds;
+  bf16_t* const dOs = FLIP ? Qs : Qs + TIMG;
+  float* const Ls = (float*)(lds + NIMG * TIMG);
+  float* const Dls = Ls + BWD_QT;
+  bf16_t* const Ks = lds + NIMG * TIMG + 4 * BWD_QT;
+  bf16_t* const Vs = FLIP ? Ks : Ks + IMG;
+  const FragOff<DH> fo;
+  const FragOffPair<DH> fov;
+  const int b = blockIdx.z, h = blockIdx.y, chunk = blockIdx.x;
+  const int lane = threadIdx.x & 63, wave = __builtin_amdgcn_readfirstlane(threadIdx.x >> 6);
+  const int role = wave;
+  const int li = lane & 31, hi = lane >> 5;
+  const int q_begin = chunk * p.tchunk, q_end = min(p.T, q_begin + p.tchunk);
+  const bf16_t* Qb = p.Q + b * p.bq + h * DH;
+  const bf16_t* dOb = p.dO + b * p.bo + h * DH;
+  const bf16_t* Ob = p.O + b * p.bo + h * DH;
+  const float* Lb = p.L + ((long long)b * p.H + h) * p.T;
+  const __amdgpu_buffer_rsrc_t rsQ = make_rsrc(Qb, (unsigned)(((long long)(p.T - 1) * p.ldq + DH) * 2));
+  const __amdgpu_buffer_rsrc_t rsdO = make_rsrc(dOb, (unsigned)(((long long)(p.T - 1) * p.ldo + DH) * 2));
+
+  uint4 tq[NIT], tg[NIT];
+  auto tile_load = [&](int q0) {
+#pragma unroll
+    for (int it = 0; it < NIT; ++it) {
+      const int i = threadIdx.x + it * 256, r = i / C::NCH, c = i - r * C::NCH;
+      const bool on = i < BWD_QT * C::NCH && q0 + r < p.T;
+      tq[it] = buf_load16(rsQ, on ? (unsigned)(((q0 + r) * p.ldq + c * 8) * 2) : 0x80000000u, 0);
+      tg[it] = buf_load16(rsdO, on ? (unsigned)(((q0 + r) * p.ldo + c * 8) * 2) : 0x80000000u, 0);
+    }
+  };
+  auto tile_store = [&]() {
+#pragma unroll
+    for (int it = 0; it < NIT; ++it) {
+      const int i = threadIdx.x + it * 256, r = i / C::NCH, c = i - r * C::NCH;
+      if (i < BWD_QT * C::NCH) {
+        *(uint4*)(Qs + img_off<C::LDE>(r, c)) = tq[it];
+        *(uint4*)(dOs + (img_off<C::LDE>(r, c) ^ FLIP)) = tg[it];
+      }
+    }
+  };
+
+  tile_load(q_begin);
+  stage_rows<DH, SHORT_MAX_S, 256, 0>(Ks, make_rsrc(p.K + b * p.bk + h * DH, (unsigned)(((long long)(p.S - 1) * p.ldk + DH) * 2)), p.ldk, 0, p.S);
+  stage_rows<DH, SHORT_MAX_S, 256, FLIP>(Vs, make_rsrc(p.V + b * p.bv + h * DH, (unsigned)(((long long)(p.S - 1) * p.ldv + DH) * 2)), p.ldv, 0, p.S);
+  {
+    constexpr int PADC = (C::DV - DH) / 8;
+    if (PADC > 0)
+      for (int i = threadIdx.x; i < 2 * BWD_QT * PADC; i += 256) {
+        const int img = i / (BWD_QT * PADC), j = i - img * (BWD_QT * PADC);
+        *(uint4*)((img ? dOs : Qs) + (img_off<C::LDE>(j / PADC, C::NCH + j % PADC) ^ (img ? FLIP : 0))) = make_uint4(0, 0, 0, 0);
+      }
+  }
+  __syncthreads();
+
+  if (role == 0) {
+    bf16x8 of[C::NKS];
+    float Lq = 0.f;
+    auto stats_load = [&](int q0) {
+      const int q = q0 + li;
+      load_row_frags<DH>(Ob, p.ldo, q, p.T, hi, of);
+      Lq = q < p.T ? Lb[q] : 0.f;
+    };
+    stats_load(q_begin);
+    for (int q0 = q_begin; q0 < q_end; q0 += BWD_QT) {
+      __syncthreads();
+      tile_store();
+      __syncthreads();
+      if (q0 + BWD_QT < q_end) tile_load(q0 + BWD_QT);
+      bf16x8 qf[C::NKS], dof[C::NKS];
+      float Dq = 0.f, Lcur = 0.f;
+      const int q = q0 + li;
+#pragma unroll
+      for (int ks = 0; ks < C::NKS; ++ks) {
+        qf[ks] = load_row_frag<DH>(Qs, fo, 0, ks);
+        dof[ks] = load_row_frag<DH>(dOs, fov, 0, ks);
+      }
+      float sacc = 0.f;
+#pragma unroll
+      for (int ks = 0; ks < C::NKS; ++ks) {
+        Frag a, g;
+        a.v = of[ks]; g.v = dof[ks];
+        float x[8], y[8];
+        unpack8(a.q, x);
+        unpack8(g.q, y);
+#pragma unroll
+        for (int k = 0; k < 8; ++k) sacc = fmaf(x[k], y[k], sacc);
+      }
+      Dq = sacc + __shfl_xor(sacc, 32, 64);
+      Lcur = Lq;
+      if (hi == 0) {
+        Ls[li] = q < p.T ? Lcur : INFINITY;
+        Dls[li] = Dq;
+      }
+      __syncthreads();
+      if (q0 + BWD_QT < q_end) stats_load(q0 + BWD_QT);
+      f32x16 acc[C::NDT];
+#pragma unroll
+      for (int dt = 0; dt < C::NDT; ++dt)
+#pragma unroll
+        for (int r = 0; r < 16; ++r) acc[dt][r] = 0.f;
+#pragma unroll
+      for (int jb = 0; jb < SHORT_KB; ++jb) {
+        if (jb * 32 >= p.S) break;
+        f32x16 s, dp;
+#pragma unroll
+        for (int r = 0; r < 16; ++r) { s[r] = 0.f; dp[r] = 0.f; }
+#pragma unroll
+        for (int ks = 0; ks < C::NKS; ++ks) {
+          s = mfma32(load_row_frag<DH>(Ks, fo, jb, ks), qf[ks], s);
+          dp = mfma32(load_row_frag<DH>(Vs, fov, jb, ks), dof[ks], dp);
+        }
+        float ds[16];
+        if ((jb + 1) * 32 > p.S) {
+#pragma unroll
+          for (int r = 0; r < 16; ++r) {
+            const float pv = jb * 32 + acc_row(r, hi) < p.S ? fast_exp2(s[r] * p.scale2 - Lcur) : 0.f;
+            ds[r] = pv * (dp[r] - Dq);
+          }
+        } else {
+#pragma unroll
+          for (int r = 0; r < 16; r += 2) {
+            const f32x2 t = pk_fma<PK_REG>(f32x2{s[r], s[r + 1]}, f32x2{p.scale2, p.scale2}, f32x2{-Lcur, -Lcur});
+            const f32x2 d = pk_fma<PK_REG>(f32x2{Dq, Dq}, f32x2{-1.f, -1.f}, f32x2{dp[r], dp[r + 1]});
+            const f32x2 o2 = pk_mul<PK_REG>(f32x2{fast_exp2(t.x), fast_exp2(t.y)}, d);
+            ds[r] = o2.x; ds[r + 1] = o2.y;
+          }
+        }
+        const bf16x8 f0 = pack_acc(ds, 0), f1 = pack_acc(ds, 1);
+#pragma unroll
+        for (int dt = 0; dt < C::NDT; ++dt) {
+          acc[dt] = mfma32(load_T_frag<DH>(Ks, fo, dt, jb, 0), f0, acc[dt]);
+          acc[dt] = mfma32(load_T_frag<DH>(Ks, fo, dt, jb, 1), f1, acc[dt]);
+        }
+      }
+      store_T_acc<DH>(acc, p.scale, p.dQ + b * p.bq + h * DH, p.ldq, q, p.T, hi);
+    }
+    return;
+  }
+
+  const int kb = role - 1;
+  if (kb * 32 >= p.S) {
+    for (int q0 = q_begin; q0 < q_end; q0 += BWD_QT) {
+      __syncthreads();
+      tile_store();
+      __syncthreads();
+      if (q0 + BWD_QT < q_end) tile_load(q0 + BWD_QT);
+      __syncthreads();
+    }
+    return;
+  }
+  f32x16 dvt[C::NDT], dkt[C::NDT];
+#pragma unroll
+  for (int dt = 0; dt < C::NDT; ++dt)
+#pragma unroll
+    for (int r = 0; r < 16; ++r) { dvt[dt][r] = 0.f; dkt[dt][r] = 0.f; }
+  for (int q0 = q_begin; q0 < q_end; q0 += BWD_QT) {
+    __syncthreads();
+    tile_store();
+    __syncthreads();
+    if (q0 + BWD_QT < q_end) tile_load(q0 + BWD_QT);
+    f32x16 s, dp;
+#pragma unroll
+    for (int r = 0; r < 16; ++r) { s[r] = 0.f; dp[r] = 0.f; }
+#pragma unroll
+    for (int ks = 0; ks < C::NKS; ++ks) {
+      s = mfma32(load_row_frag<DH>(Qs, fo, 0, ks), load_row_frag<DH>(Ks, fo, kb, ks), s);
+      dp = mfma32(load_row_frag<DH>(dOs, fov, 0, ks), load_row_frag<DH>(Vs, fov, kb, ks), dp);
+    }
+    __syncthreads();
+    float pr[16], ds[16];
+#pragma unroll
+    for (int g = 0; g < 4; ++g) {
+      const float4 l4 = *(const float4*)(Ls + 8 * g + 4 * hi);
+      const float4 d4 = *(const float4*)(Dls + 8 * g + 4 * hi);
+      const float lq[4] = {l4.x, l4.y, l4.z, l4.w}, dq[4] = {d4.x, d4.y, d4.z, d4.w};
+#pragma unroll
+      for (int j = 0; j < 4; j += 2) {
+        const int r = 4 * g + j;
+        const f32x2 t = pk_fma<PK_REG>(f32x2{s[r], s[r + 1]}, f32x2{p.scale2, p.scale2}, f32x2{-lq[j], -lq[j + 1]});
+        const f32x2 d = pk_fma<PK_REG>(f32x2{dq[j], dq[j + 1]}, f32x2{-1.f, -1.f}, f32x2{dp[r], dp[r + 1]});
+        const f32x2 e2 = f32x2{fast_exp2(t.x), fast_exp2(t.y)};
+        const f32x2 o2 = pk_mul<PK_REG>(e2, d);
+        pr[r] = e2.x; pr[r + 1] = e2.y; ds[r] = o2.x; ds[r + 1] = o2.y;
+      }
+    }
+    const bf16x8 pf0 = pack_acc(pr, 0), pf1 = pack_acc(pr, 1);
+    const bf16x8 sf0 = pack_acc(ds, 0), sf1 = pack_acc(ds, 1);
+#pragma unroll
+    for (int dt = 0; dt < C::NDT; ++dt) {
+      dvt[dt] = mfma32(load_T_frag<DH>(dOs, fov, dt, 0, 0), pf0, dvt[dt]);
+      dvt[dt] = mfma32(load_T_frag<DH>(dOs, fov, dt, 0, 1), pf1, dvt[dt]);
+      dkt[dt] = mfma32(load_T_frag<DH>(Qs, fo, dt, 0, 0), sf0, dkt[dt]);
+      dkt[dt] = mfma32(load_T_frag<DH>(Qs, fo, dt, 0, 1), sf1, dkt[dt]);
+    }
+  }
+  int tid = threadIdx.x;
+  asm volatile("" : "+v"(tid));
+  const int key = kb * 32 + (tid & 31), hi2 = (tid >> 5) & 1;
+  if (p.tsplit > 1) {
+    float* base = p.part + ((((size_t)chunk * gridDim.z + b) * p.H + h) * 2) * (size_t)p.S * DH;
+    store_T_acc_f32<DH>(dvt, base, key, p.S, hi2);
+    store_T_acc_f32<DH>(dkt, base + (size_t)p.S * DH, key, p.S, hi2);
+    return;
+  }
+  store_T_acc<DH>(dvt, 1.f, p.dV + b * p.bv + h * DH, p.ldv, key, p.S, hi2);
+  store_T_acc<DH>(dkt, p.scale, p.dK + b * p.bk + h * DH, p.ldk, key, p.S, hi2);
+}
+
+struct ShortKernels {
+  int dh;
+  void (*fwd)(AttnArgs, int);
+  const char* fwd_text;
+  void (*bwd)(AttnArgs);
+  const char* bwd_text;
+  void (*reduce)(AttnArgs, int);
+  const char* reduce_text;
+};
+#define SHORT_KERNELS(DH) {DH, &attn_short_fwd_kernel<DH>, "attn_short_fwd_kernel<" #DH ">", &attn_short_bwd_kernel<DH>, "attn_short_bwd_kernel<" #DH ">", \
+                           &attn_dkv_reduce_kernel<DH>, "attn_dkv_reduce_kernel<" #DH ">"}
+const ShortKernels kShort[] = {SHORT_KERNELS(40), SHORT_KERNELS(80)};
+#undef SHORT_KERNELS
+
+struct ShortPlan {
+  const ShortKernels* k;
+  int fwd_qchunk, fwd_chunks, bwd_qchunk, bwd_chunks;
+  size_t ws_floats;
+};
+constexpr long long LIM32 = 0x7fffffffLL;
+
+bool short_plan(int Bn, int H, int T, int S, int DH, int causal, ShortPlan* pl) {
+  if (causal || Bn < 1 || H < 1 || T < 1 || S < 1 || S > SHORT_MAX_S) return false;
+  const ShortKernels* k = nullptr;
+  for (const ShortKernels& e : kShort)
+    if (e.dh == DH) k = &e;
+  if (!k) return false;
+  const long long ld = (long long)H * DH;
+  if (((long long)(T - 1) * ld + DH) * 2 > LIM32 || ((long long)(S - 1) * 2 * ld + DH) * 2 > LIM32) return false;
+  pl->k = k;
+  pl->fwd_qchunk = T >= 2048 ? 512 : T >= 1024 ? 256 : 128;
+  pl->fwd_chunks = cdiv(T, pl->fwd_qchunk);
+  pl->bwd_qchunk = T > 2048 ? 704 : 256;
+  pl->bwd_chunks = cdiv(T, pl->bwd_qchunk);
+  const long long ws = pl->bwd_chunks > 1 ? (long long)pl->bwd_chunks * Bn * H * 2 * S * DH : 0;
+  if (ws * 4 > LIM32) return false;
+  pl->ws_floats = (size_t)ws;
+  return true;
+}
+
+int short_check(const char* who, int Bn, int H, int T, int S, int DH, int causal, int ldq, int ldk, int ldv, int ldo, ShortPlan* pl) {
+  E4T_REQUIRE(short_plan(Bn, H, T, S, DH, causal, pl), "%s: B=%d H=%d T=%d S=%d dh=%d causal=%d is not served by the short-context kernels "
+              "(non-causal, 1 <= S <= %d, dh 40/80, 32-bit extents)", who, Bn, H, T, S, DH, causal, SHORT_MAX_S);
+  E4T_REQUIRE(ldq > 0 && ldk > 0 && ldv > 0 && ldo > 0 && ldq % 8 == 0 && ldk % 8 == 0 && ldv % 8 == 0 && ldo % 8 == 0, "%s: row strides must be positive multiples of 8", who);
+  E4T_REQUIRE(((long long)(T - 1) * ldq + DH) * 2 <= LIM32 && ((long long)(T - 1) * ldo + DH) * 2 <= LIM32 && ((long long)(S - 1) * ldk + DH) * 2 <= LIM32 &&
+              ((long long)(S - 1) * ldv + DH) * 2 <= LIM32, "%s: a (batch, head) extent exceeds 32-bit byte offsets", who);
+  return 0;
+}
+
+AttnArgs short_args(const void* Q, const void* K, const void* V, int H, int T, int S, int ldq, int ldk, int ldv, int ldo, long long bq, long long bk,
+                    long long bv, long long bo, float scale) {
+  AttnArgs p;
+  memset(&p, 0, sizeof(p));
+  p.Q = (const bf16_t*)Q; p.K = (const bf16_t*)K; p.V = (const bf16_t*)V;
+  p.T = T; p.S = S; p.H = H; p.ldq = ldq; p.ldk = ldk; p.ldv = ldv; p.ldo = ldo; p.bq = bq; p.bk = bk; p.bv = bv; p.bo = bo;
+  p.scale = scale; p.scale2 = scale * 1.4426950408889634f;
+  return p;
+}
+
+}
+
+extern "C" int e4t_attention_short_plan(int Bn, int H, int T, int S, int DH, int causal, e4t_attention_short_plan_t* out) {
+  ShortPlan pl;
+  if (!out || !short_plan(Bn, H, T, S, DH, causal, &pl)) return 0;
+  out->fwd = pl.k->fwd_text; out->bwd = pl.k->bwd_text; out->reduce = pl.bwd_chunks > 1 ? pl.k->reduce_text : nullptr;
+  out->fwd_qchunk = pl.fwd_qchunk; out->fwd_chunks = pl.fwd_chunks; out->bwd_qchunk = pl.bwd_qchunk; out->bwd_chunks = pl.bwd_chunks;
+  out->workspace_floats = pl.ws_floats;
+  return 1;
+}
+
+extern "C" int e4t_attention_short_fwd(const void* Q, const void* K, const void* V, void* O, float* lse, int Bn, int H, int T, int S, int DH, int ldq,
+                                       int ldk, int ldv, int ldo, long long bq, long long bk, long long bv, long long bo, float scale, int causal,
+                                       e4t_stream stream) {
+  ShortPlan pl;
+  if (int e = short_check("attention_short_fwd", Bn, H, T, S, DH, causal, ldq, ldk, ldv, ldo, &pl)) return e;
+  E4T_REQUIRE(Q && K && V && O, "attention_short_fwd: null operand");
+  AttnArgs p = short_args(Q, K, V, H, T, S, ldq, ldk, ldv, ldo, bq, bk, bv, bo, scale);
+  p.Out = (bf16_t*)O; p.L = lse;
+  E4T_LOG_LAUNCH("%s|B%d H%d T%d S%d causal%d|%.0f|%.0f", pl.k->fwd_text, Bn, H, T, S, 0, 2.0 * Bn * H * DH * (2.0 * T + 2.0 * S) + 4.0 * Bn * H * T,
+                 4.0 * Bn * H * (double)T * S * DH);
+  hipLaunchKernelGGL(pl.k->fwd, dim3(pl.fwd_chunks, H, Bn), dim3(256), 0, (hipStream_t)stream, p, pl.fwd_qchunk);
+  E4T_CHECK_LAUNCH(pl.k->fwd_text);
+  return 0;
+}
+
+extern "C" int e4t_attention_short_bwd(const void* Q, const void* K, const void* V, const void* O, const void* dO, const float* lse, float* ws,
+                                       size_t ws_floats, void* dQ, void* dK, void* dV, int Bn, int H, int T, int S, int DH, int ldq, int ldk, int ldv,
+                                       int ldo, long long bq, long long bk, long long bv, long long bo, float scale, int causal, e4t_stream stream) {
+  ShortPlan pl;
+  if (int e = short_check("attention_short_bwd", Bn, H, T, S, DH, causal, ldq, ldk, ldv, ldo, &pl)) return e;
+  E4T_REQUIRE(Q && K && V && O && dO && lse && dQ && dK && dV, "attention_short_bwd: null operand");
+  E4T_REQUIRE(ws_floats >= pl.ws_floats && (pl.ws_floats == 0 || ws), "attention_short_bwd: workspace of %zu floats, needs %zu", ws_floats, pl.ws_floats);
+  E4T_REQUIRE(((uintptr_t)ws & 15) == 0, "attention_short_bwd: workspace must be 16-byte aligned");
+  AttnArgs p = short_args(Q, K, V, H, T, S, ldq, ldk, ldv, ldo, bq, bk, bv, bo, scale);
+  p.O = (const bf16_t*)O; p.dO = (const bf16_t*)dO; p.L = (float*)lse;
+  p.dQ = (bf16_t*)dQ; p.dK = (bf16_t*)dK; p.dV = (bf16_t*)dV;
+  p.part = ws; p.tsplit = pl.bwd_chunks; p.tchunk = pl.bwd_qchunk;
+  const double el = (double)Bn * H * DH;
+  E4T_LOG_LAUNCH("%s|B%d H%d T%d S%d causal%d|%.0f|%.0f", pl.k->bwd_text, Bn, H, T, S, 0, 2.0 * el * (4.0 * T + 4.0 * S) + 4.0 * Bn * H * T,
+                 10.0 * Bn * H * (double)T * S * DH);
+  hipLaunchKernelGGL(pl.k->bwd, dim3(pl.bwd_chunks, H, Bn), dim3(256), 0, (hipStream_t)stream, p);
+  E4T_CHECK_LAUNCH(pl.k->bwd_text);
+  if (pl.bwd_chunks > 1) {
+    E4T_LOG_LAUNCH("%s|B%d H%d T%d S%d causal%d|%.0f|%.0f", pl.k->reduce_text, Bn, H, T, S, 0, 4.0 * pl.ws_floats + 2.0 * el * 2.0 * S, (double)pl.ws_floats);
+    const long long items = (long long)Bn * H * 2 * S * (DH / 4);
+    int rb = (int)((items + 255) / 256);
+    if (rb > 2048) rb = 2048;
+    hipLaunchKernelGGL(pl.k->reduce, dim3(rb), dim3(256), 0, (hipStream_t)stream, p, Bn);
+    E4T_CHECK_LAUNCH(pl.k->reduce_text);
+  }
+  return 0;
+}
diff --git a/e4t-diffusion_amd/e4t/_C.py b/e4t-diffusion_amd/e4t/_C.py
--- a/e4t-diffusion_amd/e4t/_C.py
+++ b/e4t-diffusion_amd/e4t/_C.py
@@ -44,6 +44,11 @@
     _fields_ = [("fwd", C.c_char_p), ("dq", C.c_char_p), ("dkv", C.c_char_p), ("tsplit", i32), ("tchunk", i32), ("dkv_occ", i32), ("workspace_floats", sz)]
 
 
+class AttentionShortPlan(C.Structure):
+    _fields_ = [("fwd", C.c_char_p), ("bwd", C.c_char_p), ("reduce", C.c_char_p), ("fwd_qchunk", i32), ("fwd_chunks", i32),
+                ("bwd_qchunk", i32), ("bwd_chunks", i32), ("workspace_floats", sz)]
+
+
 class WODesc(C.Structure):
     _fields_ = (
         [(n, vp) for n in ("v", "w1", "b1", "w2", "b2", "wc", "bc", "wr", "br", "W", "vecs", "partial", "weff", "weffT", "dweff")]
@@ -71,6 +76,9 @@
     "e4t_attention_bwd_workspace_floats": (sz, [i32] * 5),
     "e4t_attention_bwd_ws": (i32, [vp] * 7 + [sz] + [vp] * 3 + [i32] * 9 + [i64] * 4 + [f32, i32, vp]),
     "e4t_attention_plan": (i32, [i32] * 6 + [sz, C.POINTER(AttentionPlan)]),
+    "e4t_attention_short_plan": (i32, [i32] * 6 + [C.POINTER(AttentionShortPlan)]),
+    "e4t_attention_short_fwd": (i32, [vp, vp, vp, vp, vp, i32, i32, i32, i32, i32, i32, i32, i32, i32, i64, i64, i64, i64, f32, i32, vp]),
+    "e4t_attention_short_bwd": (i32, [vp] * 7 + [sz] + [vp] * 3 + [i32] * 9 + [i64] * 4 + [f32, i32, vp]),
     "e4t_groupnorm_num_chunks": (i32, [i32, i32]),
     "e4t_groupnorm_workspace_bytes": (sz, [i32, i32, i32, i32, i32]),
     "e4t_groupnorm_stats": (i32, [vp, i32, vp, i32, i32, i32, i32, f32, vp, vp, sz, vp]),
diff --git a/e4t-diffusion_amd/e4t/functional.py b/e4t-diffusion_amd/e4t/functional.py
--- a/e4t-diffusion_amd/e4t/functional.py
+++ b/e4t-diffusion_amd/e4t/functional.py
@@ -466,6 +466,11 @@
     return LayerNormSkipFn.apply(x, gamma, beta, eps)
 
 
+def _attention_short(be, q, k, v, B, H, T, S, DH, causal):
+    ok = getattr(be, "attention_short_ok", None)
+    return ok is not None and ok(q, k, v, B, H, T, S, DH, causal=causal)
+
+
 class AttentionFn(torch.autograd.Function):
 
     @staticmethod
@@ -475,7 +480,9 @@
             q, k, v = qkv[:, :d], qkv[:, d:2 * d], qkv[:, 2 * d:]
         else:
             q, k, v = qkv, kv[:, :d], kv[:, d:]
-        o, lse = ops.backend().attention_fwd(q, k, v, B, H, T, S, DH, scale, causal=causal)
+        be = ops.backend()
+        fwd = be.attention_short_fwd if _attention_short(be, q, k, v, B, H, T, S, DH, causal) else be.attention_fwd
+        o, lse = fwd(q, k, v, B, H, T, S, DH, scale, causal=causal)
         ctx.save_for_backward(qkv, kv, o, lse)
         ctx.cfg = (B, H, T, S, DH, scale, causal)
         return o
@@ -493,7 +500,9 @@
         else:
             q, k, v = qkv, kv[:, :d], kv[:, d:]
             dq, dk, dv = dqkv, dkv[:, :d], dkv[:, d:]
-        ops.backend().attention_bwd(q, k, v, o, do.contiguous(), lse, dq, dk, dv, B, H, T, S, DH, scale, causal=causal)
+        be = ops.backend()
+        bwd = be.attention_short_bwd if _attention_short(be, q, k, v, B, H, T, S, DH, causal) else be.attention_bwd
+        bwd(q, k, v, o, do.contiguous(), lse, dq, dk, dv, B, H, T, S, DH, scale, causal=causal)
         return dqkv, dkv, None, None, None, None, None, None, None
 
 
diff --git a/e4t-diffusion_amd/e4t/ops.py b/e4t-diffusion_amd/e4t/ops.py
--- a/e4t-diffusion_amd/e4t/ops.py
+++ b/e4t-diffusion_amd/e4t/ops.py
@@ -144,6 +144,7 @@
     def __init__(self):
         self.lib = _C.load()
         self._ws = {}
+        self._short_plans = {}
         self.prof = None
 
     def _timed(self, key, flops, fn, nbytes=0.0):
@@ -366,6 +367,46 @@
             _ptr(dv), B, H, T, S, DH, ldq, ldk, ldv, ldo, T * ldq, S * ldk, S * ldv, T * ldo,
             float(scale), int(causal), st), "e4t_attention_bwd_ws"), 2.0 * B * H * DH * (4 * T + 4 * S) + 8.0 * B * H * T)
 
+    def attention_short_plan(self, B, H, T, S, DH, causal=False):
+        key = (B, H, T, S, DH, bool(causal))
+        plans = self._short_plans
+        if key not in plans:
+            pl = _C.AttentionShortPlan()
+            plans[key] = pl if self.lib.e4t_attention_short_plan(B, H, T, S, DH, int(causal), C.byref(pl)) == 1 else None
+        return plans[key]
+
+    def attention_short_ok(self, q, k, v, B, H, T, S, DH, causal=False):
+        if self.attention_short_plan(B, H, T, S, DH, causal) is None:
+            return False
+        return all(t.dim() == 2 and t.stride(1) == 1 and t.stride(0) % 8 == 0 and rows * t.stride(0) * 2 < 2 ** 31
+                   for t, rows in ((q, T), (k, S), (v, S)))
+
+    def attention_short_fwd(self, q, k, v, B, H, T, S, DH, scale, out=None, need_lse=True, causal=False):
+        for t in (q, k, v):
+            _rowmajor(t, "attention operand")
+        if out is None:
+            out = torch.empty((B * T, H * DH), dtype=bf16, device=q.device)
+        lse = torch.empty((B, H, T), dtype=f32, device=q.device) if need_lse else None
+        ldq, ldk, ldv, ldo = q.stride(0), k.stride(0), v.stride(0), out.stride(0)
+        st = _stream()
+        self._timed(f"attn_fwd{DH}", 4.0 * B * H * T * S * DH, lambda: _C.check(self.lib.e4t_attention_short_fwd(
+            _ptr(q), _ptr(k), _ptr(v), _ptr(out), _ptr(lse), B, H, T, S, DH, ldq, ldk, ldv, ldo,
+            T * ldq, S * ldk, S * ldv, T * ldo, float(scale), int(causal), st), "e4t_attention_short_fwd"),
+            2.0 * B * H * DH * (2 * T + 2 * S) + 4.0 * B * H * T)
+        return out, lse
+
+    def attention_short_bwd(self, q, k, v, o, do, lse, dq, dk, dv, B, H, T, S, DH, scale, causal=False):
+        ldq, ldk, ldv, ldo = q.stride(0), k.stride(0), v.stride(0), o.stride(0)
+        assert dq.stride(0) == ldq and dk.stride(0) == ldk and dv.stride(0) == ldv and do.stride(0) == ldo
+        pl = self.attention_short_plan(B, H, T, S, DH, causal)
+        nws = pl.workspace_floats if pl is not None else 0
+        ws = torch.empty(nws, dtype=f32, device=q.device) if nws else None
+        st = _stream()
+        self._timed(f"attn_bwd{DH}", 10.0 * B * H * T * S * DH, lambda: _C.check(self.lib.e4t_attention_short_bwd(
+            _ptr(q), _ptr(k), _ptr(v), _ptr(o), _ptr(do), _ptr(lse), _ptr(ws), nws, _ptr(dq), _ptr(dk),
+            _ptr(dv), B, H, T, S, DH, ldq, ldk, ldv, ldo, T * ldq, S * ldk, S * ldv, T * ldo,
+            float(scale), int(causal), st), "e4t_attention_short_bwd"), 2.0 * B * H * DH * (4 * T + 4 * S) + 4.0 * B * H * T)
+
     def groupnorm_fwd(self, x1, x2, gamma, beta, B, HW, G, eps, silu):
         C1, C2 = x1.shape[-1], (x2.shape[-1] if x2 is not None else 0)
         Cn = C1 + C2
diff --git a/include/e4t_hip.h b/include/e4t_hip.h
--- a/include/e4t_hip.h
+++ b/include/e4t_hip.h
@@ -120,6 +120,23 @@
   size_t workspace_floats;
 } e4t_attention_plan_t;
 int e4t_attention_plan(int B, int H, int T, int S, int DH, int causal, size_t ws_floats, e4t_attention_plan_t* out);
+
+typedef struct {
+  const char* fwd;
+  const char* bwd;
+  const char* reduce;
+  int fwd_qchunk, fwd_chunks;
+  int bwd_qchunk, bwd_chunks;
+  size_t workspace_floats;
+} e4t_attention_short_plan_t;
+int e4t_attention_short_plan(int B, int H, int T, int S, int DH, int causal, e4t_attention_short_plan_t* out);
+int e4t_attention_short_fwd(const void* Q, const void* K, const void* V, void* O, float* lse, int B, int H, int T, int S, int DH,
+                            int ldq, int ldk, int ldv, int ldo, long long bq, long long bk, long long bv, long long bo,
+                            float scale, int causal, e4t_stream stream);
+int e4t_attention_short_bwd(const void* Q, const void* K, const void* V, const void* O, const void* dO, const float* lse,
+                            float* ws, size_t ws_floats, void* dQ, void* dK, void* dV, int B, int H, int T, int S, int DH, int ldq,
+                            int ldk, int ldv, int ldo, long long bq, long long bk, long long bv, long long bo, float scale,
+                            int causal, e4t_stream stream);
 
 int e4t_groupnorm_num_chunks(int B, int HW);
 size_t e4t_groupnorm_workspace_bytes(int B, int HW, int C, int G, int with_param_grads);
```
